# CPCLAB-UNIPI/MPC-code

Hardware: AMD Instinct MI355X
Metric: closed-loop MPC steps/sec over batch, LMPC-CSTR N=50 (higher is better)
Workload: dtype f64

## Files before the change

### __graft_entry__.py

```python
import os
import sys

ROOT = os.path.dirname(os.path.abspath(__file__))
if ROOT not in sys.path:
    sys.path.insert(0, ROOT)

WV_DIRECTION_EXTRA_SETS = ((1, 1, 1, 1, 1, 0, 0), (4, 1, 1, 1, 4, 0, 0), (4, 2, 2, 2, 4, 0, 0), (8, 2, 2, 2, 8, 0, 0))
WV_VGPR_FORM_SETS = ((1, 1, 1, 1, 1, 0, 0), (2, 1, 1, 1, 2, 0, 0), (2, 1, 1, 1, 2, 0, 1), (3, 2, 3, 3, 3, 0, 0), (4, 1, 1, 1, 4, 0, 0), (4, 2, 2, 2, 4, 0, 0))


def build() -> None:
    import mpc_code_amd
    from concurrent.futures import ThreadPoolExecutor
    from mpc_code_amd import capi, nlcodegen
    sys.path.insert(0, os.path.join(ROOT, "oracle"))
    import oracle_c
    import enmpc_oracle_c
    import nmpc_oracle_c
    jobs = [lambda: capi.build_library(verbose=True), oracle_c.build, enmpc_oracle_c.build, nmpc_oracle_c.build]
    for dims in ((3, 2, 3, 3, 3, 1, 0), (5, 2, 2, 2, 5, 0, 0), (3, 2, 3, 3, 3, 0, 0, 1, 1), (3, 2, 3, 3, 3, 0, 2, 1, 1), (6, 2, 8, 0, 6, 0, 0, 1, 1)):
        jobs.append(lambda dims=dims: capi.build_library(dims=dims))
    for dims in WV_DIRECTION_EXTRA_SETS:
        jobs.append(lambda dims=dims: capi.build_library(dims=dims))
    for dims in WV_VGPR_FORM_SETS:
        jobs.append(lambda dims=dims: capi.build_library(dims=dims, extra_flags=(capi.WV_GENERIC_TILES_FLAG,)))
    for ex, dims in (("cstr_nlplant_lmpc.py", (3, 2, 2, 2, 3, 1, 0)), ("cstr_xp_nlplant_lmpc.py", (4, 2, 2, 2, 3, 1, 1))):
        jobs.append(lambda ex=ex, dims=dims: capi.build_library(dims=dims, plant_header=nlcodegen.emit_plant_header(mpc_code_amd.load_problem(mpc_code_amd.example_path(ex)))))
    for ex in ("cstr_nmpc.py", "quadtank_nmpc_dis.py", "reactor_nmpc.py", "cstr_nmpc_rows.py"):
        jobs.append(lambda ex=ex: nlcodegen.build_nmpc_library(mpc_code_amd.load_problem(mpc_code_amd.example_path(ex))))
    from mpc_code_amd import econcodegen
    jobs.append(lambda: econcodegen.build_enmpc_library(mpc_code_amd.load_problem(mpc_code_amd.example_path("reactor_enmpc.py"))))
    jobs.append(lambda: econcodegen.build_enmpc_library(mpc_code_amd.load_problem(mpc_code_amd.example_path("reactor_enmpc_ekf.py"))))
    jobs.append(lambda: econcodegen.build_enmpc_library(mpc_code_amd.load_problem(mpc_code_amd.example_path("reactor_enmpc.py"), overrides={"wmin": [-1.0] * 4, "wmax": [1.0] * 4})))
    jobs.append(lambda: econcodegen.build_enmpc_library(mpc_code_amd.load_problem(mpc_code_amd.example_path("reactor_enmpc_rows.py"))))
    jobs.append(lambda: econcodegen.build_enmpc_library(mpc_code_amd.load_problem(mpc_code_amd.example_path("reactor_enmpc.py")), extra_flags=["-DEC_SWEEP_SERIAL"]))
    import warnings
    sys.path.insert(0, os.path.join(ROOT, "tests"))
    from enmpc_cases import FUZZ_SEEDS, draw

    def fuzz_model(seed):
        with warnings.catch_warnings():
            warnings.simplefilter("ignore")
            return mpc_code_amd.load_problem(mpc_code_amd.example_path("reactor_enmpc.py"), overrides=draw(seed)[0])
    for seed in FUZZ_SEEDS:
        jobs.append(lambda seed=seed: econcodegen.build_enmpc_library(fuzz_model(seed)))
    import nmpc_family
    for member in nmpc_family.MEMBERS:
        jobs.append(lambda member=member: nlcodegen.build_nmpc_library(nmpc_family.load_product(member)))
    import nmpc_lin_family
    for member in nmpc_lin_family.MEMBERS:
        jobs.append(lambda member=member: nlcodegen.build_nmpc_library(nmpc_lin_family.load_product(member)))
    jobs.append(lambda: nlcodegen.build_nmpc_library(mpc_code_amd.load_problem(mpc_code_amd.example_path("reactor_nmpc_lin.py"))))
    with ThreadPoolExecutor(max_workers=min(len(jobs), max(1, (os.cpu_count() or 2) - 1))) as pool:
        built = [f.result() for f in [pool.submit(j) for j in jobs]]
    lib = built[0]
    handle = capi.load_library(lib)
    missing = [s for s in capi.EXPORTS if not hasattr(handle, s)]
    if missing:
        raise RuntimeError(f"libmpc_amd.so lacks {missing}")
    for b in built:
        print("built", b)
    print(handle.mpc_build_info().decode())
    assert mpc_code_amd.load_problem(mpc_code_amd.example_path("cstr_lmpc.py")).nw == 253


def smoke() -> None:
    import numpy as np
    import mpc_code_amd as m
    from mpc_code_amd import capi
    sys.path.insert(0, os.path.join(ROOT, "oracle"))
    import oracle_c
    prob = m.load_problem(m.example_path("cstr_lmpc.py"))
    rng = np.random.default_rng(20250614)
    x0 = rng.uniform([-0.5, -8.0, -5.0], [0.5, 8.0, 5.0], size=(128, 3))
    nsteps = 8
    solver = capi.Solver(prob, device=0)
    solver.loop_alloc(len(x0), nsteps, capi.LOG_ALL)
    solver.loop_set_state(x0, x0)
    solver.loop_set_schedule(prob.schedules(nsteps))
    solver.loop_run(0, nsteps)
    solver.loop_sync()
    U = solver.loop_get_log("U"); st = solver.loop_get_log("STATUS_DYN")
    ref = oracle_c.OracleC(prob).closed_loop(nsteps, x0, x0)
    assert np.array_equal(st, ref["STATUS_DYN"]), "solver status differs from the oracle"
    err = float(np.abs(U - ref["U"]).max())
    assert err < 1e-6, f"u* differs from the oracle by {err}"
    ms, n = solver.last_kernel_ms()
    print(f"smoke ok: {len(x0)} instances x {nsteps} steps, max|u - u_oracle| = {err:.2e}, {ms:.2f} ms in {n} launches")
    solver.close()
    from mpc_code_amd import nmpc
    g = np.load(os.path.join(ROOT, "tests", "golden", "nmpc_cstr.npz"))
    nl = m.load_problem(m.example_path("cstr_nmpc.py"))
    r = nmpc.run_nmpc_closed_loop(nl, g["rti_x0"], g["rti_x0"], nsteps=3, max_sqp=1)
    e = float(np.max(np.abs(r["U"] - g["rti_U"][:3]) / (1.0 + np.abs(g["rti_U"][:3]))))
    assert np.array_equal(r["STATUS_DYN"], g["rti_STATUS_DYN"][:3]) and e < 1e-6, f"non-linear path differs from its oracle vectors by {e}"
    print(f"smoke ok: non-linear path, max rel |u - u_oracle| = {e:.2e}")
    from mpc_code_amd import enmpc
    g = np.load(os.path.join(ROOT, "tests", "golden", "enmpc_reactor.npz"))
    ec = m.load_problem(m.example_path("reactor_enmpc.py"))
    r = enmpc.run_enmpc_closed_loop(ec, g["ship_x0"], nsteps=3)
    e = float(np.abs(r["U"] - g["ship_U"][:3]).max())
    assert np.array_equal(r["STATUS_DYN"], g["ship_STATUS_DYN"][:3]) and np.array_equal(r["ITERS_DYN"], g["ship_ITERS_DYN"][:3]) and e < 1e-7, f"economic path differs from its oracle vectors by {e}"
    print(f"smoke ok: economic path, max |u - u_oracle| = {e:.2e}")


# ... 5 lines not shown
```

### mpc-code_amd/csrc/mpc_amd.hip

```cpp
#include "../../include/mpc_amd.h"
#include "mpc_device.hpp"
#include "mpc_lane_step.hpp"
#include "mpc_tp.hpp"
#include "mpc_wave.hpp"
#include "mpc_soft.hpp"

#include <hip/hip_runtime.h>
#include "mpc_comm.hpp"

#include <cmath>
#include <cstdint>
#include <cstdio>
#include <cstring>
#include <string>
#include <vector>

using namespace mpc;

#ifndef MPC_PART2
extern "C" const char *mpc_last_error(void) { return g_err; }
#endif

#define MPC_DIM9_(M, NX, NU, NY, ND, NXP, DU, NG, NGS, NHS, ...) M(NX, NU, NY, ND, NXP, DU, NG, NGS, NHS)
#define MPC_DIM9(M, ...) MPC_DIM9_(M, __VA_ARGS__, 0, 0, 0)
// ... 413 lines not shown
                    MPC_UNROLL for (int j = 0; j < NX; j++) v += P.Cm[i][j] * xs[j];
                    MPC_UNROLL for (int j = 0; j < ND; j++) v += P.Cd[i][j] * dh[j];
                    (a.YS + (size_t)((size_t)k * NY + i) * Bs)[bq] = v;
                }
            }
            if (a.st_dyn) { (a.st_ss + (size_t)k * Bs)[bq] = st_ss; (a.it_ss + (size_t)k * Bs)[bq] = it_ss; }
            OcpInst<NS, NU> q;
            build_inst<NX, NU, NY, ND, DU, NG>(P, xh, xs, us, dh, u, q);
            double delta = delta_est;
            MPC_UNROLL for (int i = 0; i < NX; i++) delta = dmax(delta, fabs(xs[i] - xs_prev[i]));
            MPC_UNROLL for (int i = 0; i < NU; i++) delta = dmax(delta, fabs(us[i] - us_prev[i]));
            const bool warm = a.ws_valid[bq] != 0 && delta <= kWsDelta && !P.no_warm;
            double *qd = sh.q + lane * Cfg::QN;
            MPC_UNROLL for (int i = 0; i < NS; i++) { qd[i] = q.z0[i]; qd[NS + i] = q.zr[i]; qd[2 * NS + i] = q.c[i]; qd[3 * NS + i] = q.zlo_m[i]; qd[4 * NS + i] = q.zhi_m[i]; }
            MPC_UNROLL for (int i = 0; i < NU; i++) { qd[5 * NS + i] = q.ur[i]; qd[5 * NS + NU + i] = q.us[i]; }
            qd[5 * NS + 2 * NU] = delta;
            sh.iflag[lane] = kTpValid | (q.ok0 ? kTpOk0 : 0) | (warm ? kTpWarm : 0);
            MPC_UNROLL for (int i = 0; i < NX; i++) { (a.xhat + (size_t)(i) * Bs)[bq] = xh[i]; (a.xs + (size_t)(i) * Bs)[bq] = xs[i]; }
            MPC_UNROLL for (int i = 0; i < ND; i++) (a.dhat + (size_t)(i) * Bs)[bq] = dh[i];
            MPC_UNROLL for (int i = 0; i < NU; i++) (a.us + (size_t)(i) * Bs)[bq] = us[i];
        } else if (wl) sh.iflag[lane] = 0;
        int st_dyn, it_dyn;
        MPC_TSTAMP(0);
        tp_solve<NS, NU, DU, NC, MASKED, NW, IPW>(P, sh, wsg, P.max_iter, st_dyn, it_dyn);
        if (valid && P.term_cons && st_dyn != kInfeasible) {
            const double *fin_rows = wsg + (size_t)lane * Cfg::ROWS_ST * 64, *qd = sh.q + lane * Cfg::QN;
            double v = 0.0;
            MPC_UNROLL for (int i = 0; i < NX; i++) v = dmax(v, fabs(fin_rows[(Cfg::ST_Z + i) * 64 + P.N - 1] - qd[NS + i]) * frcp(dmax(1.0, fabs(qd[NS + i]))));
            if (!(v <= P.term_tol)) st_dyn = kInfeasible;
        }
        if (valid) {
            double x[NXP], xh[NX], u[NU];
            MPC_UNROLL for (int i = 0; i < NXP; i++) x[i] = (a.x + (size_t)(i) * Bs)[bq];
            MPC_UNROLL for (int i = 0; i < NU; i++) u[i] = (a.u + (size_t)(i) * Bs)[bq];
            if (st_dyn != kInfeasible) {
                const double *fin_rows = wsg + (size_t)lane * Cfg::ROWS_ST * 64;
                MPC_UNROLL for (int i = 0; i < NU; i++) u[i] = (DU && P.in_is_du) ? fin_rows[(Cfg::ST_Z + (DU ? NX + i : 0)) * 64] : fin_rows[(Cfg::ST_U + i) * 64];
                MPC_UNROLL for (int i = 0; i < NX; i++) xh[i] = fin_rows[(Cfg::ST_Z + i) * 64];
            } else {
                double xo[NX], dh[ND > 0 ? ND : 1];
                MPC_UNROLL for (int i = 0; i < NX; i++) xo[i] = (a.xhat + (size_t)(i) * Bs)[bq];
                MPC_UNROLL for (int i = 0; i < ND; i++) dh[i] = (a.dhat + (size_t)(i) * Bs)[bq];
                MPC_UNROLL for (int i = 0; i < NX; i++) {
                    double v = P.fxc[i];
                    MPC_UNROLL for (int j = 0; j < NX; j++) v += P.Am[i][j] * xo[j];
                    MPC_UNROLL for (int j = 0; j < NU; j++) v += P.Bm[i][j] * u[j];
                    MPC_UNROLL for (int j = 0; j < ND; j++) v += P.Bd[i][j] * dh[j];
                    xh[i] = v;
                }
            }
            if (a.U) { MPC_UNROLL for (int i = 0; i < NU; i++) (a.U + (size_t)((size_t)k * NU + i) * Bs)[bq] = u[i]; }
            if (a.st_dyn) { (a.st_dyn + (size_t)k * Bs)[bq] = st_dyn; (a.it_dyn + (size_t)k * Bs)[bq] = it_dyn; }
            double xn[NXP];
            plant_next<NXP, NU>(P, x, u, a.pxp + k * NXP, a.t0 + k * a.h, a.h, xn);
            if (a.wn) { MPC_UNROLL for (int i = 0; i < NXP; i++) xn[i] += (a.wn + (size_t)((size_t)k * NXP + i) * Bs)[bq]; }
            MPC_UNROLL for (int i = 0; i < NXP; i++) (a.x + (size_t)(i) * Bs)[bq] = xn[i];
            MPC_UNROLL for (int i = 0; i < NX; i++) (a.xhat + (size_t)(i) * Bs)[bq] = xh[i];
            MPC_UNROLL for (int i = 0; i < NU; i++) (a.u + (size_t)(i) * Bs)[bq] = u[i];
            a.ws_valid[bq] = st_dyn == kSolved ? 1 : 0;
        }
        __syncthreads();
        MPC_STAMP_RESET
    }
    if (valid) {
        a.tw_valid[b] = sh.keepflag[lane];
        MPC_UNROLL for (int f = 0; f < NTW; f++) (a.tw + (size_t)f * Bs)[(unsigned)b] = twk[f];
    }
}

template <int NS, int NU, int NC, int NX, int NI, class Cfg>
__device__ __forceinline__ bool wv_term_aim(int N, double *q, int *iflag, int *aimv, int *itacc, const WvIterA<NS, NU, NC> (&X)[NI], const WvInst (&S)[NI])
{
    const int lane = threadIdx.x;
    if (lane == N - 1) {
        MPC_UNROLL for (int j = 0; j < NI; j++) {
            double c[NX], v = 0.0;
            MPC_UNROLL for (int i = 0; i < NX; i++) { const double zr = q[j * Cfg::QN + NS + i]; c[i] = a_get(X[j].z[i]) - zr; v = dmax(v, fabs(c[i]) * frcp(dmax(1.0, fabs(zr)))); }
            const int f = iflag[j];
            const bool again = (f & kWvValid) && (f & kWvOk0) && S[j].status != kInfeasible && v > 1e-11 && v <= 1e-4;
            if (again) { MPC_UNROLL for (int i = 0; i < NX; i++) q[j * Cfg::QN + Cfg::QZN + i] -= c[i]; q[j * Cfg::QN + 5 * NS + 2 * NU] = v; }
            aimv[j] = again ? 1 : 0;
        }
    }
    __syncthreads();
    int any = 0;
    MPC_UNROLL for (int j = 0; j < NI; j++) any |= aimv[j];
    any = __builtin_amdgcn_readfirstlane(any);
    if (any && lane < NI) {
        int st = S[0].status, it = S[0].iters;
        MPC_UNROLL for (int j = 1; j < NI; j++) { if (lane == j) { st = S[j].status; it = S[j].iters; } }
        const int f = iflag[lane];
        if ((f & kWvValid) && (f & kWvOk0) && st != kInfeasible) { iflag[lane] = kWvValid | kWvOk0 | kWvWarm | kWvNoShift; itacc[lane] += it; }
    }
    __syncthreads();
    return any != 0;
}

template <int NX, int NU, int NY, int ND, int NXP, bool DU, int NG, int NC, bool MASKED, int NI, int NGS = 0, int NHS = 0>
struct WvKernelCfg {
    static constexpr int NS = NX + (DU ? NU : 0) + NG, NE = NX + ND, NDD = ND > 0 ? ND : 1;
    using Cfg = WvCfg<NS, NU, NC, NI>;
    using RT = Row16Tab<NX, NU, NY, ND, NGS, NHS>;
    static constexpr int NTW = 2 * (NU - NHS) + 3 * (NX + NU + NY + NGS);
    static constexpr int K_X = 0, K_XH = NXP, K_DH = K_XH + NX, K_U = K_DH + NDD, K_XS = K_U + NU, K_US = K_XS + NX, K_P = K_US + NU,
                         K_TW = K_P + NE * NE, KEEP = K_TW + NTW;
    static constexpr int t_region(int N)
    {
        const int t = Cfg::t_doubles(N), x = Cfg::GUARD + (RT::fits ? 4 * RT::XCH : 0);
        return t > x ? t : x;
    }
    static constexpr size_t lds_bytes(int N) { return sizeof(double) * ((size_t)t_region(N) + NI * Cfg::QN + NI * Cfg::OUT + NI * KEEP + (RT::fits ? RT::DOUBLES : 0)) + sizeof(int) * 24; }
    static constexpr int ni() { return NI; }
};

template <bool NOISE, int NX, int NU, int NY, int ND, int NXP, bool DU, int NG, int NC, bool MASKED, int NI, int NGS, int NHS>
__device__ __forceinline__ void loop_wv_body(const DevProblem *__restrict__ Pp, const LoopArgs &a)
{
    using KC = WvKernelCfg<NX, NU, NY, ND, NXP, DU, NG, NC, MASKED, NI, NGS, NHS>;
    using Cfg = typename KC::Cfg;
    constexpr int NS = KC::NS, NE = KC::NE, NDD = KC::NDD, NTW = KC::NTW, KEEP = KC::KEEP;
    extern __shared__ double wv_smem[];
    const DevProblem &P0 = *Pp;
    const int LD = Cfg::ld(P0.N);
    double *const T = wv_smem + Cfg::GUARD, *const q = wv_smem + KC::t_region(P0.N), *const outv = q + NI * Cfg::QN, *const keep = outv + NI * Cfg::OUT;
    int *const iflag = (int *)(keep + NI * KEEP), *const twv = iflag + 4, *const wsv = twv + 4, *const aimv = wsv + 4, *const itacc = aimv + 4;
    using RT = typename KC::RT;
    double *const tab = (double *)(wsv + 16);
    const ConstProblem &P = *(const ConstProblem *)Pp;
    const size_t Bs = a.Bs;
    const int lane = threadIdx.x;
    const int il = lane < NI ? lane : 0;
    const int b = blockIdx.x * NI + il;
    const bool valid = lane < NI && b < a.B;
    double *const kp = keep + il * KEEP;
    if (valid) {
        MPC_UNROLL for (int i = 0; i < NXP; i++) kp[KC::K_X + i] = (a.x + (size_t)i * Bs)[b];
        MPC_UNROLL for (int i = 0; i < NX; i++) { kp[KC::K_XH + i] = (a.xhat + (size_t)i * Bs)[b]; kp[KC::K_XS + i] = (a.xs + (size_t)i * Bs)[b]; }
        MPC_UNROLL for (int i = 0; i < ND; i++) kp[KC::K_DH + i] = (a.dhat + (size_t)i * Bs)[b];
        MPC_UNROLL for (int i = 0; i < NU; i++) { kp[KC::K_U + i] = (a.u + (size_t)i * Bs)[b]; kp[KC::K_US + i] = (a.us + (size_t)i * Bs)[b]; }
        if (P.estimator == MPC_EST_KALMAN) { for (int i = 0; i < NE * NE; i++) kp[KC::K_P + i] = (a.Pk + (size_t)i * Bs)[b]; }
        for (int f = 0; f < NTW; f++) kp[KC::K_TW + f] = (a.tw + (size_t)f * Bs)[b];
        twv[lane] = a.tw_valid[b]; wsv[lane] = a.ws_valid[b];
    } else if (lane < NI) { twv[lane] = 0; wsv[lane] = 0; }
    for (int i = lane; i < NI * LD; i += 64) T[Cfg::RZ * NI * LD + i] = 0.0;
    if (lane < Cfg::GUARD) wv_smem[lane] = 0.0;
    if (RT::fits) row16_fill_tables<NX, NU, NY, ND, NGS, NHS>(P, tab, lane);
    __syncthreads();
    WvIterA<NS, NU, NC> X[NI];
    WvInst S[NI];
    MPC_UNROLL for (int j = 0; j < NI; j++) {
        const double *rows = a.ws + ((size_t)(blockIdx.x * NI + j) * Cfg::ROWS_WS) * 64;
        const bool w = __builtin_amdgcn_readfirstlane(wsv[j]) != 0;
        WvIter<NS, NU, NC> X0;
        MPC_UNROLL for (int i = 0; i < NU; i++) X0.u[i] = w ? rows[i * 64 + lane] : 0.0;
        MPC_UNROLL for (int i = 0; i < NC; i++) { X0.ll[i] = w ? rows[(NU + i) * 64 + lane] : 0.0; X0.lh[i] = w ? rows[(NU + NC + i) * 64 + lane] : 0.0; X0.sl[i] = 1.0; X0.sh[i] = 1.0; }
        MPC_UNROLL for (int i = 0; i < NS; i++) X0.z[i] = 0.0;
        X[j].put(X0);
    }
    MPC_STAMP_INIT
    int redo = 0;
    for (int k = 0; k < a.nsteps; k++) {
        unsigned bq = (unsigned)b;
        asm volatile("" : "+v"(bq));
        if (redo == 0) {
        if constexpr (RT::fits) {
            const int b16 = lane >> 4, r16 = lane & 15, b16c = b16 < NI ? b16 : 0;
            const unsigned bi = (unsigned)(blockIdx.x * NI + b16c);
            const bool inst16 = b16 < NI && (int)bi < a.B;
            double *const kq = keep + b16c * KEEP;
            if (inst16) {
                if (a.XP && r16 < NXP) (a.XP + (size_t)((size_t)k * NXP + r16) * Bs)[bi] = kq[KC::K_X + r16];
                if (a.XHAT && r16 < NX) (a.XHAT + (size_t)((size_t)k * NX + r16) * Bs)[bi] = kq[KC::K_XH + r16];
            }
            double xi_old = 0.0, xi_new = 0.0;
            if (P.estimator != MPC_EST_NONE)
                kalman_row16<NX, NY, ND, NXP, NU>(P, r16, b16 < NI, kq, KC::K_X, KC::K_XH, KC::K_P, a.pyp + k * NY, (NOISE && a.vn) ? a.vn + (size_t)k * NY * Bs + bi : nullptr, Bs, tab, T + b16c * RT::XCH, xi_old, xi_new);
            if (inst16 && a.DHAT && r16 >= NX && r16 < NE) (a.DHAT + (size_t)((size_t)k * ND + (r16 - NX)) * Bs)[bi] = xi_new;
            double delta = row16_max(r16 < NE ? fabs(xi_new - xi_old) : 0.0);
            __syncthreads();
            if (Cfg::RZ * NI * LD < 4 * RT::XCH) { for (int i = lane; i < NI * LD; i += 64) T[Cfg::RZ * NI * LD + i] = 0.0; }
            double dh[NDD], usv[NU];
            MPC_UNROLL for (int i = 0; i < ND; i++) dh[i] = kq[KC::K_DH + i];
            MPC_UNROLL for (int i = 0; i < NU; i++) usv[i] = kq[KC::K_US + i];
            int it_ss; double vrow;
            int st_ss;
            if constexpr (NOISE) {
                double uspv[NU], yspv[NY];
                MPC_UNROLL for (int i = 0; i < NU; i++) uspv[i] = a.usp[k * NU + i];
                MPC_UNROLL for (int i = 0; i < NY; i++) yspv[i] = a.ysp[k * NY + i];
                if (a.usp_b) { MPC_UNROLL for (int i = 0; i < NU; i++) uspv[i] = (a.usp_b + (size_t)((size_t)k * NU + i) * Bs)[bi]; }
                if (a.ysp_b) { MPC_UNROLL for (int i = 0; i < NY; i++) yspv[i] = (a.ysp_b + (size_t)((size_t)k * NY + i) * Bs)[bi]; }
                st_ss = target_row16<NX, NU, NY, ND, NGS, NHS>(P, r16, tab, uspv, yspv, dh, usv, kq + KC::K_TW, twv + b16c, inst16, vrow, it_ss);
            } else
                st_ss = target_row16<NX, NU, NY, ND, NGS, NHS>(P, r16, tab, a.usp + k * NU, a.ysp + k * NY, dh, usv, kq + KC::K_TW, twv + b16c, inst16, vrow, it_ss);
            const bool trow = r16 < NX + NU && b16 < NI;
            const double prev = trow ? kq[KC::K_XS + r16] : 0.0;
            const double tnew = (st_ss != kInfeasible && trow) ? vrow : prev;
            delta = dmax(delta, row16_max(fabs(tnew - prev)));
            if (trow) kq[KC::K_XS + r16] = tnew;
            if (inst16) {
                if (a.XS && r16 < NX) (a.XS + (size_t)((size_t)k * NX + r16) * Bs)[bi] = tnew;
                if (a.US && r16 >= NX && trow) (a.US + (size_t)((size_t)k * NU + (r16 - NX)) * Bs)[bi] = tnew;
                if (a.st_dyn && r16 == 0) { (a.st_ss + (size_t)k * Bs)[bi] = st_ss; (a.it_ss + (size_t)k * Bs)[bi] = it_ss; }
            }
            if (r16 == 0 && b16 < NI) outv[b16c * Cfg::OUT] = delta;
            __syncthreads();
        }
        if (valid) {
            double xh[NX], dh[NDD], u[NU], xs[NX], us[NU], delta = 0.0;
            MPC_UNROLL for (int i = 0; i < NX; i++) { xh[i] = kp[KC::K_XH + i]; xs[i] = kp[KC::K_XS + i]; }
            MPC_UNROLL for (int i = 0; i < ND; i++) dh[i] = kp[KC::K_DH + i];
            MPC_UNROLL for (int i = 0; i < NU; i++) { u[i] = kp[KC::K_U + i]; us[i] = kp[KC::K_US + i]; }
            if constexpr (RT::fits) delta = outv[lane * Cfg::OUT];
            else {
                double x[NXP];
                double xh_pred[NX], dh_prev[NDD], xs_prev[NX], us_prev[NU];
                MPC_UNROLL for (int i = 0; i < NXP; i++) x[i] = kp[KC::K_X + i];
                MPC_UNROLL for (int i = 0; i < NX; i++) { xh[i] = kp[KC::K_XH + i]; xs[i] = kp[KC::K_XS + i]; xh_pred[i] = xh[i]; xs_prev[i] = xs[i]; }
                MPC_UNROLL for (int i = 0; i < ND; i++) { dh[i] = kp[KC::K_DH + i]; dh_prev[i] = dh[i]; }
                MPC_UNROLL for (int i = 0; i < NU; i++) { u[i] = kp[KC::K_U + i]; us[i] = kp[KC::K_US + i]; us_prev[i] = us[i]; }
                if (a.XP) { MPC_UNROLL for (int i = 0; i < NXP; i++) (a.XP + (size_t)((size_t)k * NXP + i) * Bs)[bq] = x[i]; }
                if (a.XHAT) { MPC_UNROLL for (int i = 0; i < NX; i++) (a.XHAT + (size_t)((size_t)k * NX + i) * Bs)[bq] = xh[i]; }
                if (P.estimator != MPC_EST_NONE) {
                    double xi[NE], innov[NY];
                    MPC_UNROLL for (int i = 0; i < NX; i++) xi[i] = xh[i];
                    MPC_UNROLL for (int i = 0; i < ND; i++) xi[NX + i] = dh[i];
                    MPC_UNROLL for (int i = 0; i < NY; i++) {
                        double yh = P.fyc[i], yy = a.pyp[k * NY + i];
                        if (NOISE && a.vn) yy += (a.vn + (size_t)((size_t)k * NY + i) * Bs)[bq];
                        MPC_UNROLL for (int j = 0; j < NE; j++) yh += P.Ca[i][j] * xi[j];
                        MPC_UNROLL for (int j = 0; j < NXP; j++) yy += P.Cp[i][j] * x[j];
                        innov[i] = yy - yh;
                    }
                    if (P.estimator == MPC_EST_KALMAN) {
                        double Pk[NE][NE];
                        MPC_UNROLL for (int i = 0; i < NE; i++) { MPC_UNROLL for (int j = 0; j < NE; j++) Pk[i][j] = kp[KC::K_P + i * NE + j]; }
                        kalman_lane<NE, NY>(P, xi, Pk, innov);
                        MPC_UNROLL for (int i = 0; i < NE; i++) { MPC_UNROLL for (int j = 0; j < NE; j++) kp[KC::K_P + i * NE + j] = Pk[i][j]; }
                    } else {
                        MPC_UNROLL for (int i = 0; i < NE; i++) { double s = 0.0; MPC_UNROLL for (int l = 0; l < NY; l++) s += P.Kfix[i][l] * innov[l]; xi[i] += s; }
                    }
                    MPC_UNROLL for (int i = 0; i < NX; i++) xh[i] = xi[i];
                    MPC_UNROLL for (int i = 0; i < ND; i++) { double d = xi[NX + i]; if (P.has_dsat) d = dmin(dmax(d, P.dmin[i]), P.dmax[i]); dh[i] = d; }
                }
                if (a.DHAT) { MPC_UNROLL for (int i = 0; i < ND; i++) (a.DHAT + (size_t)((size_t)k * ND + i) * Bs)[bq] = dh[i]; }
                MPC_UNROLL for (int i = 0; i < NX; i++) delta = dmax(delta, fabs(xh[i] - xh_pred[i]));
                MPC_UNROLL for (int i = 0; i < ND; i++) delta = dmax(delta, fabs(dh[i] - dh_prev[i]));
                double usp[NU], ysp[NY], xs_n[NX], us_n[NU], ys_n[NY];
                MPC_UNROLL for (int i = 0; i < NU; i++) usp[i] = a.usp[k * NU + i];
                MPC_UNROLL for (int i = 0; i < NY; i++) ysp[i] = a.ysp[k * NY + i];
                if (NOISE && a.usp_b) { MPC_UNROLL for (int i = 0; i < NU; i++) usp[i] = (a.usp_b + (size_t)((size_t)k * NU + i) * Bs)[bq]; }
                if (NOISE && a.ysp_b) { MPC_UNROLL for (int i = 0; i < NY; i++) ysp[i] = (a.ysp_b + (size_t)((size_t)k * NY + i) * Bs)[bq]; }
                int it_ss;
                const int st_ss = target_lane<NX, NU, NY, ND, NGS, NHS>(P, usp, ysp, dh, us, xs_n, us_n, ys_n, it_ss, kp + KC::K_TW, 1, twv + lane);
                if (st_ss != kInfeasible) {
                    MPC_UNROLL for (int i = 0; i < NX; i++) xs[i] = xs_n[i];
                    MPC_UNROLL for (int i = 0; i < NU; i++) us[i] = us_n[i];
                }
                if (a.XS) { MPC_UNROLL for (int i = 0; i < NX; i++) (a.XS + (size_t)((size_t)k * NX + i) * Bs)[bq] = xs[i]; }
                if (a.US) { MPC_UNROLL for (int i = 0; i < NU; i++) (a.US + (size_t)((size_t)k * NU + i) * Bs)[bq] = us[i]; }
                if (a.st_dyn) { (a.st_ss + (size_t)k * Bs)[bq] = st_ss; (a.it_ss + (size_t)k * Bs)[bq] = it_ss; }
                MPC_UNROLL for (int i = 0; i < NX; i++) delta = dmax(delta, fabs(xs[i] - xs_prev[i]));
                MPC_UNROLL for (int i = 0; i < NU; i++) delta = dmax(delta, fabs(us[i] - us_prev[i]));
            }
            if (a.YS) {
                MPC_UNROLL for (int i = 0; i < NY; i++) {
                    double v = P.fyc[i];
                    MPC_UNROLL for (int j = 0; j < NX; j++) v += P.Cm[i][j] * xs[j];
                    MPC_UNROLL for (int j = 0; j < ND; j++) v += P.Cd[i][j] * dh[j];
                    (a.YS + (size_t)((size_t)k * NY + i) * Bs)[bq] = v;
                }
            }
            OcpInst<NS, NU> qi;
            build_inst<NX, NU, NY, ND, DU, NG>(P, xh, xs, us, dh, u, qi);
            const bool warm = wsv[lane] != 0 && delta <= kWsDelta && !P.no_warm;
            double *qd = q + lane * Cfg::QN;
            MPC_UNROLL for (int i = 0; i < NS; i++) { qd[i] = qi.z0[i]; qd[NS + i] = qi.zr[i]; qd[2 * NS + i] = qi.c[i]; qd[3 * NS + i] = qi.zlo_m[i]; qd[4 * NS + i] = qi.zhi_m[i]; qd[Cfg::QZN + i] = qi.zrN[i]; }
            MPC_UNROLL for (int i = 0; i < NU; i++) { qd[5 * NS + i] = qi.ur[i]; qd[5 * NS + NU + i] = qi.us[i]; }
            qd[5 * NS + 2 * NU] = delta;
            iflag[lane] = kWvValid | (qi.ok0 ? kWvOk0 : 0) | (warm ? kWvWarm : 0);
            itacc[lane] = 0;
            MPC_UNROLL for (int i = 0; i < NX; i++) { kp[KC::K_XH + i] = xh[i]; kp[KC::K_XS + i] = xs[i]; }
            MPC_UNROLL for (int i = 0; i < ND; i++) kp[KC::K_DH + i] = dh[i];
            MPC_UNROLL for (int i = 0; i < NU; i++) kp[KC::K_US + i] = us[i];
        } else if (lane < NI) iflag[lane] = 0;
        __syncthreads();
        }
        MPC_TSTAMP(0);
        wv_solve<NS, NU, DU, NC, MASKED, NI>(P, T, q, iflag, X, S, P.max_iter);
        MPC_STAMP_RESET
        if (lane == 0) {
            MPC_UNROLL for (int j = 0; j < NI; j++) {
                MPC_UNROLL for (int i = 0; i < NU; i++) outv[j * Cfg::OUT + i] = a_get(X[j].u[i]);
                MPC_UNROLL for (int i = 0; i < NS; i++) outv[j * Cfg::OUT + NU + i] = a_get(X[j].z[i]);
            }
        }
        if (P.term_cons && lane == P.N - 1) {
            MPC_UNROLL for (int j = 0; j < NI; j++) {
                double v = 0.0, c[NX];
                MPC_UNROLL for (int i = 0; i < NX; i++) { const double zr = q[j * Cfg::QN + NS + i]; c[i] = a_get(X[j].z[i]) - zr; v = dmax(v, fabs(c[i]) * frcp(dmax(1.0, fabs(zr)))); }
                outv[j * Cfg::OUT + NU + NS] = v;
                const int f = iflag[j];
                const bool again = redo < 2 && (f & kWvValid) && (f & kWvOk0) && S[j].status != kInfeasible && v > 1e-11 && v <= 1e-4;
                if (again) { MPC_UNROLL for (int i = 0; i < NX; i++) q[j * Cfg::QN + Cfg::QZN + i] -= c[i]; q[j * Cfg::QN + 5 * NS + 2 * NU] = v; }
                aimv[j] = again ? 1 : 0;
            }
        }
        __syncthreads();
        if (P.term_cons && redo < 2) {
            int any = 0;
            MPC_UNROLL for (int j = 0; j < NI; j++) any |= aimv[j];
            if (__builtin_amdgcn_readfirstlane(any)) {
                if (lane < NI) {
                    int st = S[0].status, it = S[0].iters;
                    MPC_UNROLL for (int j = 1; j < NI; j++) { if (lane == j) { st = S[j].status; it = S[j].iters; } }
                    const int f = iflag[lane];
                    if ((f & kWvValid) && (f & kWvOk0) && st != kInfeasible) { iflag[lane] = kWvValid | kWvOk0 | kWvWarm | kWvNoShift; itacc[lane] += it; }
                }
                __syncthreads();
                redo++; k--;
                continue;
            }
        }
        redo = 0;
        if (valid) {
            int st_dyn = S[0].status, it_dyn = S[0].iters;
            MPC_UNROLL for (int j = 1; j < NI; j++) { if (lane == j) { st_dyn = S[j].status; it_dyn = S[j].iters; } }
            if (P.term_cons) it_dyn += itacc[lane];
            if (P.term_cons && st_dyn != kInfeasible && !(outv[lane * Cfg::OUT + NU + NS] <= P.term_tol)) st_dyn = kInfeasible;
            double x[NXP], xh[NX], u[NU];
            MPC_UNROLL for (int i = 0; i < NXP; i++) x[i] = kp[KC::K_X + i];
            MPC_UNROLL for (int i = 0; i < NU; i++) u[i] = kp[KC::K_U + i];
            if (st_dyn != kInfeasible) {
                MPC_UNROLL for (int i = 0; i < NU; i++) u[i] = (DU && P.in_is_du) ? outv[lane * Cfg::OUT + NU + (DU ? NX + i : 0)] : outv[lane * Cfg::OUT + i];
                MPC_UNROLL for (int i = 0; i < NX; i++) xh[i] = outv[lane * Cfg::OUT + NU + i];
            } else {
                double xo[NX], dh[NDD];
                MPC_UNROLL for (int i = 0; i < NX; i++) xo[i] = kp[KC::K_XH + i];
                MPC_UNROLL for (int i = 0; i < ND; i++) dh[i] = kp[KC::K_DH + i];
                MPC_UNROLL for (int i = 0; i < NX; i++) {
                    double v = P.fxc[i];
                    MPC_UNROLL for (int j = 0; j < NX; j++) v += P.Am[i][j] * xo[j];
                    MPC_UNROLL for (int j = 0; j < NU; j++) v += P.Bm[i][j] * u[j];
                    MPC_UNROLL for (int j = 0; j < ND; j++) v += P.Bd[i][j] * dh[j];
                    xh[i] = v;
                }
            }
            if (a.U) { MPC_UNROLL for (int i = 0; i < NU; i++) (a.U + (size_t)((size_t)k * NU + i) * Bs)[bq] = u[i]; }
            if (a.st_dyn) { (a.st_dyn + (size_t)k * Bs)[bq] = st_dyn; (a.it_dyn + (size_t)k * Bs)[bq] = it_dyn; }
            {
                double xn[NXP];
                plant_next<NXP, NU>(P, x, u, a.pxp + k * NXP, a.t0 + k * a.h, a.h, xn);
                if (NOISE && a.wn) { MPC_UNROLL for (int i = 0; i < NXP; i++) xn[i] += (a.wn + (size_t)((size_t)k * NXP + i) * Bs)[bq]; }
                MPC_UNROLL for (int i = 0; i < NXP; i++) kp[KC::K_X + i] = xn[i];
            }
            MPC_UNROLL for (int i = 0; i < NX; i++) kp[KC::K_XH + i] = xh[i];
            MPC_UNROLL for (int i = 0; i < NU; i++) kp[KC::K_U + i] = u[i];
            wsv[lane] = st_dyn == kSolved ? 1 : 0;
        }
        __syncthreads();
        MPC_TSTAMP(7);
    }
    if (valid) {
        MPC_UNROLL for (int i = 0; i < NXP; i++) (a.x + (size_t)i * Bs)[b] = kp[KC::K_X + i];
        MPC_UNROLL for (int i = 0; i < NX; i++) { (a.xhat + (size_t)i * Bs)[b] = kp[KC::K_XH + i]; (a.xs + (size_t)i * Bs)[b] = kp[KC::K_XS + i]; }
        MPC_UNROLL for (int i = 0; i < ND; i++) (a.dhat + (size_t)i * Bs)[b] = kp[KC::K_DH + i];
        MPC_UNROLL for (int i = 0; i < NU; i++) { (a.u + (size_t)i * Bs)[b] = kp[KC::K_U + i]; (a.us + (size_t)i * Bs)[b] = kp[KC::K_US + i]; }
        if (P.estimator == MPC_EST_KALMAN) { for (int i = 0; i < NE * NE; i++) (a.Pk + (size_t)i * Bs)[b] = kp[KC::K_P + i]; }
        for (int f = 0; f < NTW; f++) (a.tw + (size_t)f * Bs)[b] = kp[KC::K_TW + f];
        a.tw_valid[b] = twv[lane]; a.ws_valid[b] = wsv[lane];
    }
    MPC_UNROLL for (int j = 0; j < NI; j++) {
        double *rows = a.ws + ((size_t)(blockIdx.x * NI + j) * Cfg::ROWS_WS) * 64;
        MPC_UNROLL for (int i = 0; i < NU; i++) rows[i * 64 + lane] = a_get(X[j].u[i]);
        MPC_UNROLL for (int i = 0; i < NC; i++) { rows[(NU + i) * 64 + lane] = a_get(X[j].ll[i]); rows[(NU + NC + i) * 64 + lane] = a_get(X[j].lh[i]); }
    }
}

template <int NX, int NU, int NY, int ND, int NXP, bool DU, int NG, int NC, bool MASKED, int NI, int NGS = 0, int NHS = 0>
__global__ __launch_bounds__(64, 1) void loop_kernel_wv(const DevProblem *__restrict__ Pp, LoopArgs a)
{
    loop_wv_body<false, NX, NU, NY, ND, NXP, DU, NG, NC, MASKED, NI, NGS, NHS>(Pp, a);
}

template <int NX, int NU, int NY, int ND, int NXP, bool DU, int NG, int NC, bool MASKED, int NI, int NGS = 0, int NHS = 0>
__global__ __launch_bounds__(64, 1) void loop_noisy_wv_kernel(const DevProblem *__restrict__ Pp, LoopArgs a)
{
    loop_wv_body<true, NX, NU, NY, ND, NXP, DU, NG, NC, MASKED, NI, NGS, NHS>(Pp, a);
}

struct OcpWvArgs {
    OcpArgs o;
    const double *u_guess;
    double *traj;
    double *prev;
    int32_t *valid;
    int warm_on;
};

template <int NX, int NU, int NY, int ND, bool DU, int NG, int NC, bool MASKED, int NI>
__global__ __launch_bounds__(64, 1) void ocp_kernel_wv(const DevProblem *__restrict__ Pp, OcpWvArgs w)
{
    constexpr int NS = NX + (DU ? NU : 0) + NG, NDD = ND > 0 ? ND : 1;
    using Cfg = WvCfg<NS, NU, NC, NI>;
    const OcpArgs &a = w.o;
    extern __shared__ double wv_smem[];
    const ConstProblem &P = *(const ConstProblem *)Pp;
    const int N = Pp->N, LD = Cfg::ld(N);
    double *const T = wv_smem + Cfg::GUARD, *const q = wv_smem + Cfg::t_doubles(N), *const outv = q + NI * Cfg::QN;
    int *const iflag = (int *)(outv + NI * Cfg::OUT), *const aimv = iflag + 4, *const itacc = aimv + 4;
    const size_t Bs = a.Bs;
    const int lane = threadIdx.x;
    const int il = lane < NI ? lane : 0;
    const int b = blockIdx.x * NI + il;
    const bool valid = lane < NI && b < a.B;
    for (int i = lane; i < NI * LD; i += 64) T[Cfg::RZ * NI * LD + i] = 0.0;
    if (lane < Cfg::GUARD) wv_smem[lane] = 0.0;
    if (valid) {
        double xh[NX], xs[NX], us[NU], up[NU], dh[NDD];
        MPC_UNROLL for (int i = 0; i < NX; i++) { xh[i] = a.xhat[i * Bs + b]; xs[i] = a.xs[i * Bs + b]; }
        MPC_UNROLL for (int i = 0; i < NU; i++) { us[i] = a.us[i * Bs + b]; up[i] = a.u_prev[i * Bs + b]; }
        MPC_UNROLL for (int i = 0; i < ND; i++) dh[i] = a.dhat[i * Bs + b];
        OcpInst<NS, NU> qi;
        build_inst<NX, NU, NY, ND, DU, NG>(P, xh, xs, us, dh, up, qi);
        double delta = 0.0;
        MPC_UNROLL for (int i = 0; i < NX; i++) delta = dmax(delta, dmax(fabs(xh[i] - w.prev[i * Bs + b]), fabs(xs[i] - w.prev[(NX + ND + i) * Bs + b])));
        MPC_UNROLL for (int i = 0; i < ND; i++) delta = dmax(delta, fabs(dh[i] - w.prev[(NX + i) * Bs + b]));
        MPC_UNROLL for (int i = 0; i < NU; i++) delta = dmax(delta, fabs(us[i] - w.prev[(2 * NX + ND + i) * Bs + b]));
        const bool warm = w.warm_on && w.valid[b] != 0 && delta <= kWsDelta && !P.no_warm;
        double *qd = q + lane * Cfg::QN;
        MPC_UNROLL for (int i = 0; i < NS; i++) { qd[i] = qi.z0[i]; qd[NS + i] = qi.zr[i]; qd[2 * NS + i] = qi.c[i]; qd[3 * NS + i] = qi.zlo_m[i]; qd[4 * NS + i] = qi.zhi_m[i]; qd[Cfg::QZN + i] = qi.zrN[i]; }
        MPC_UNROLL for (int i = 0; i < NU; i++) { qd[5 * NS + i] = qi.ur[i]; qd[5 * NS + NU + i] = qi.us[i]; }
        qd[5 * NS + 2 * NU] = delta;
        iflag[lane] = kWvValid | (qi.ok0 ? kWvOk0 : 0) | (warm ? kWvWarm : 0) | ((warm && w.u_guess) ? kWvKeepU : 0);
        itacc[lane] = 0;
        MPC_UNROLL for (int i = 0; i < ND; i++) w.prev[(NX + i) * Bs + b] = dh[i];
        MPC_UNROLL for (int i = 0; i < NX; i++) w.prev[(NX + ND + i) * Bs + b] = xs[i];
        MPC_UNROLL for (int i = 0; i < NU; i++) w.prev[(2 * NX + ND + i) * Bs + b] = us[i];
    } else if (lane < NI) iflag[lane] = 0;
    __syncthreads();
    WvIterA<NS, NU, NC> X[NI];
    WvInst S[NI];
    MPC_UNROLL for (int j = 0; j < NI; j++) {
        const size_t bj = (size_t)blockIdx.x * NI + j;
        const double *rows = a.ws + (bj * Cfg::ROWS_WS) * 64;
        const int fl = __builtin_amdgcn_readfirstlane(iflag[j]);
        const bool wm = (fl & kWvWarm) != 0, ku = (fl & kWvKeepU) != 0;
        WvIter<NS, NU, NC> X0;
        MPC_UNROLL for (int i = 0; i < NU; i++) X0.u[i] = wm ? (ku ? w.u_guess[(bj * NU + i) * 64 + lane] : rows[i * 64 + lane]) : 0.0;
        MPC_UNROLL for (int i = 0; i < NC; i++) { X0.ll[i] = wm ? rows[(NU + i) * 64 + lane] : 0.0; X0.lh[i] = wm ? rows[(NU + NC + i) * 64 + lane] : 0.0; X0.sl[i] = 1.0; X0.sh[i] = 1.0; }
        MPC_UNROLL for (int i = 0; i < NS; i++) X0.z[i] = 0.0;
        X[j].put(X0);
    }
    for (int pass = 0;; pass++) {
        wv_solve<NS, NU, DU, NC, MASKED, NI, ConstProblem, false, false, true>(P, T, q, iflag, X, S, P.max_iter);
        if (!P.term_cons || pass == 2 || !wv_term_aim<NS, NU, NC, NX, NI, Cfg>(N, q, iflag, aimv, itacc, X, S)) break;
    }
    MPC_UNROLL for (int j = 0; j < NI; j++) {
        const size_t bj = (size_t)blockIdx.x * NI + j;
        double *rows = a.ws + (bj * Cfg::ROWS_WS) * 64;
        WvIter<NS, NU, NC> Xf; X[j].get(Xf);
        MPC_UNROLL for (int i = 0; i < NU; i++) rows[i * 64 + lane] = Xf.u[i];
        MPC_UNROLL for (int i = 0; i < NC; i++) { rows[(NU + i) * 64 + lane] = Xf.ll[i]; rows[(NU + NC + i) * 64 + lane] = Xf.lh[i]; }
        if (w.traj) {
            MPC_UNROLL for (int i = 0; i < NU; i++) w.traj[(bj * (NU + NS) + i) * 64 + lane] = Xf.u[i];
            MPC_UNROLL for (int i = 0; i < NS; i++) w.traj[(bj * (NU + NS) + NU + i) * 64 + lane] = Xf.z[i];
        }
        if (lane == 0) {
            MPC_UNROLL for (int i = 0; i < NU; i++) outv[j * Cfg::OUT + i] = Xf.u[i];
            MPC_UNROLL for (int i = 0; i < NS; i++) outv[j * Cfg::OUT + NU + i] = Xf.z[i];
        }
        if (P.term_cons && lane == P.N - 1) {
            double v = 0.0;
            MPC_UNROLL for (int i = 0; i < NX; i++) { const double zr = q[j * Cfg::QN + NS + i]; v = dmax(v, fabs(Xf.z[i] - zr) * frcp(dmax(1.0, fabs(zr)))); }
            outv[j * Cfg::OUT + NU + NS] = v;
        }
    }
    __syncthreads();
    if (valid) {
        int st = S[0].status, it = S[0].iters; double r0 = S[0].res_s, r1 = S[0].res_p, r2 = S[0].mu;
        MPC_UNROLL for (int j = 1; j < NI; j++) { if (lane == j) { st = S[j].status; it = S[j].iters; r0 = S[j].res_s; r1 = S[j].res_p; r2 = S[j].mu; } }
        if (P.term_cons) it += itacc[lane];
        if (P.term_cons && st != kInfeasible && !(outv[lane * Cfg::OUT + NU + NS] <= P.term_tol)) st = kInfeasible;
        a.status[b] = st; a.iters[b] = it;
        a.res[0 * Bs + b] = r0; a.res[1 * Bs + b] = r1; a.res[2 * Bs + b] = r2;
        w.valid[b] = st == kSolved ? 1 : 0;
        if (st != kInfeasible) {
            MPC_UNROLL for (int i = 0; i < NU; i++) a.u_out[i * Bs + b] = (DU && P.in_is_du) ? outv[lane * Cfg::OUT + NU + (DU ? NX + i : 0)] : outv[lane * Cfg::OUT + i];
            MPC_UNROLL for (int i = 0; i < NX; i++) { const double v = outv[lane * Cfg::OUT + NU + i]; a.xnext_out[i * Bs + b] = v; w.prev[i * Bs + b] = v; }
        }
    }
}

#ifndef MPC_PART2
__global__ void pack_u_kernel(const double *__restrict__ u, double *__restrict__ dst, int B, size_t Bs, int nu)
{
    const int b = blockIdx.x * blockDim.x + threadIdx.x;
    if (b >= B) return;
    for (int i = 0; i < nu; i++) dst[(size_t)b * nu + i] = u[i * Bs + b];
}
#endif

struct Launchers {
    void (*ocp)(const DevProblem *, OcpArgs, hipStream_t);
    void (*ocp_pxy)(const DevProblem *, OcpPxyArgs, hipStream_t);
    void (*ocp_soft)(const DevProblem *, OcpSoftArgs, hipStream_t);
    int soft_fields;
    void (*loop_soft)(const DevProblem *, LoopArgs, hipStream_t);
    void (*loop_pxy)(const DevProblem *, LoopArgs, hipStream_t);
    int pxy_ws_rows, pxy_nc, pxy_lin;
    void (*target)(const DevProblem *, TargetArgs, hipStream_t);
    void (*kf)(const DevProblem *, KfArgs, hipStream_t);
    void (*loop)(const DevProblem *, LoopArgs, hipStream_t);
    int (*loop_tp)(const DevProblem *, LoopArgs, hipStream_t);
    int (*loop_wv)(const DevProblem *, LoopArgs, hipStream_t);
    int (*ocp_wv)(const DevProblem *, OcpWvArgs, int, hipStream_t);
    int wv_ns;
    size_t wv_ws_per_inst, wv_lds;
    int ws_rows, nc, tp_ni;
    int tp_max_batch;
    size_t tp_ws_per_inst, tp_ws_per_group, tp_lds;
};

static constexpr int kTpMaxBatch = 16384;

enum { kBoundsAllFinite = 1, kBoundsInputsOnly = 2, kBoundsGeneric = 0 };

template <int NX, int NU, int NY, int ND, int NXP, bool DU, int NG, int NC, bool MASKED, int NI, int NGS, int NHS>
static int launch_loop_wv(const DevProblem *p, LoopArgs a, hipStream_t s, int dev)
{
    using KC = WvKernelCfg<NX, NU, NY, ND, NXP, DU, NG, NC, MASKED, NI, NGS, NHS>;
    const bool noisy = a.vn || a.wn || a.ysp_b || a.usp_b;
    auto kern = noisy ? loop_noisy_wv_kernel<NX, NU, NY, ND, NXP, DU, NG, NC, MASKED, NI, NGS, NHS> : loop_kernel_wv<NX, NU, NY, ND, NXP, DU, NG, NC, MASKED, NI, NGS, NHS>;
    static bool attr_set[2][64] = {};
    if (!attr_set[noisy][dev]) {
        if (hipFuncSetAttribute(reinterpret_cast<const void *>(kern), hipFuncAttributeMaxDynamicSharedMemorySize, (int)KC::lds_bytes(64)) != hipSuccess) return -1;
        attr_set[noisy][dev] = true;
    }
    hipLaunchKernelGGL(kern, dim3((a.B + NI - 1) / NI), dim3(64), KC::lds_bytes(a.N), s, p, a);
    return 0;
}

template <int NX, int NU, int NY, int ND, int NXP, bool DU, int NG, int NC, bool MASKED, int NGS, int NHS>
static Launchers make_launchers_mode()
{
    Launchers l;
    l.ocp = [](const DevProblem *p, OcpArgs a, hipStream_t s) { hipLaunchKernelGGL((ocp_kernel<NX, NU, NY, ND, DU, NG, NC, MASKED>), dim3((a.B + 63) / 64), dim3(64), 0, s, p, a); };
    {
        constexpr int NSZ = NX + (DU ? NU : 0) + NG;
        l.ocp_pxy = [](const DevProblem *p, OcpPxyArgs a, hipStream_t s) { hipLaunchKernelGGL((ocp_kernel_pxy<NX, NU, NY, ND, DU, NG>), dim3((a.o.B + 63) / 64), dim3(64), 0, s, p, a); };
        if constexpr (NGS == 0 && NHS == 0)
            l.loop_pxy = [](const DevProblem *p, LoopArgs a, hipStream_t s) { hipLaunchKernelGGL((loop_kernel_pxy<NX, NU, NY, ND, NXP, DU, NG>), dim3((a.B + 63) / 64), dim3(64), 0, s, p, a); };
        else
            l.loop_pxy = nullptr;
        l.pxy_ws_rows = 2 * BlkLayout<NSZ, NU, NSZ + NU>::SLOTS; l.pxy_nc = NSZ + NU; l.pxy_lin = NSZ * (NSZ + NU + 1) + 2 * NSZ;
        l.ocp_soft = [](const DevProblem *p, OcpSoftArgs a, hipStream_t s) { hipLaunchKernelGGL((ocp_kernel_soft<NX, NU, NY, ND, DU, NG>), dim3((a.o.B + 63) / 64), dim3(64), 0, s, p, a); };
        l.soft_fields = SoftLayout<NSZ, NU, NY>::FIELDS;
        l.loop_soft = [](const DevProblem *p, LoopArgs a, hipStream_t s) { hipLaunchKernelGGL((loop_kernel_soft<NX, NU, NY, ND, NXP, DU, NG, NGS, NHS>), dim3((a.B + 63) / 64), dim3(64), 0, s, p, a); };
    }
    l.target = [](const DevProblem *p, TargetArgs a, hipStream_t s) { hipLaunchKernelGGL((target_kernel<NX, NU, NY, ND, NGS, NHS>), dim3((a.B + 63) / 64), dim3(64), 0, s, p, a); };
    l.kf = [](const DevProblem *p, KfArgs a, hipStream_t s) { hipLaunchKernelGGL((kf_kernel<NX, NY, ND>), dim3((a.B + 63) / 64), dim3(64), 0, s, p, a); };
// ... 1202 lines not shown
```

### mpc-code_amd/csrc/mpc_device.hpp

```cpp
#pragma once
#include <hip/hip_runtime.h>
#include <math.h>
#include <stdint.h>

namespace mpc {

constexpr double kMu0 = 1.0;
constexpr double kSMin = 1.0;
constexpr double kTau = 0.995;
constexpr double kTolStat = 1e-9;
constexpr double kTolStatAcc = 1e-6;
constexpr int kStallMax = 2;
constexpr double kTolFeas = 1e-9;
constexpr double kTolC = 1e-9;
constexpr double kTolMu = 1e-14;
constexpr double kMuFloor = 1e-15;
constexpr double kSFloor = 1e-11;
constexpr double kBoundRelax = 1e-8;
constexpr double kInfeasZ = 1e10;
constexpr double kWsDelta = 0.3;
constexpr double kWsKappa = 1e-2;
constexpr double kWsSMinLo = 1e-9, kWsSMinHi = 1e-6;
constexpr double kWsMuFactor = 1e4;

constexpr int kMaxN = 8, kMaxM = 4, kMaxY = 8, kMaxD = 8, kMaxV = kMaxN + kMaxM, kMaxC = kMaxN + kMaxM + kMaxY,
              kMaxE = kMaxN + kMaxD, kMaxGS = 4;

enum : int { kSolved = 0, kMaxIter = 1, kInfeasible = 2 };

struct DevProblem {
    int nx, nu, ny, nd, nxp, N, du_form, duss_form, y_bounded, estimator, max_iter, has_dsat;
    int term_cons; double term_tol, term_gcap, term_floor;
    int no_warm;
    int in_is_du, zr_us;
    double A[kMaxN][kMaxN], B[kMaxN][kMaxM], Q[kMaxN][kMaxN], M[kMaxN][kMaxM], R[kMaxM][kMaxM], Pf[kMaxN][kMaxN];
    double ulo[kMaxM], uhi[kMaxM], zlo_m[kMaxN], zhi_m[kMaxN], zlo_e[kMaxN], zhi_e[kMaxN];
    double Am[kMaxN][kMaxN], Bm[kMaxN][kMaxM], Cm[kMaxY][kMaxN], Bd[kMaxN][kMaxD], Cd[kMaxY][kMaxD], fxc[kMaxN], fyc[kMaxY];
    double Ap[kMaxN][kMaxN], Bp[kMaxN][kMaxM], Cp[kMaxY][kMaxN];
    double ymin[kMaxY], ymax[kMaxY], dmin[kMaxD], dmax[kMaxD];
    int ymap_idx[kMaxY]; double ymap_scale[kMaxY];
    int ng, yg_row[kMaxY];
    double Ep[kMaxV][kMaxN], Zn[kMaxV][kMaxM], CZx[kMaxY][kMaxM], Hr[kMaxM][kMaxM], W[kMaxC][kMaxM], tlo[kMaxC], thi[kMaxC];
    double Qss[kMaxY][kMaxY], Rss[kMaxM][kMaxM];
    double Aa[kMaxE][kMaxE], Ca[kMaxY][kMaxE], Qkf[kMaxE][kMaxE], Rkf[kMaxY][kMaxY], Kfix[kMaxE][kMaxY];
    double Apow[6][kMaxN][kMaxN];
    int soft;
    double Ws[2 * kMaxY][2 * kMaxY];
    int ng_ss, nh_ss;
    double Eh[kMaxV][kMaxM];
    double Hd_ss[kMaxM][kMaxD], h0_ss[kMaxM];
    double Gv_ss[kMaxGS][kMaxV], Gd_ss[kMaxGS][kMaxD], g0_ss[kMaxGS];
    double Wg[kMaxGS][kMaxM];
};

typedef __attribute__((address_space(4))) DevProblem ConstProblem;

#define MPC_UNROLL _Pragma("unroll")
#ifdef MPC_STAMPS
__device__ unsigned long long mpc_stamp_buf[4096 * 8];
#define MPC_STAMP(slot) do { const unsigned long long t_ = __builtin_amdgcn_s_memtime(); __builtin_amdgcn_s_waitcnt(0xC07F); \
    if (threadIdx.x == 0) mpc_stamp_buf[blockIdx.x * 8 + (slot)] += t_ - stamp_prev_; stamp_prev_ = t_; } while (0)
#define MPC_STAMP_INIT unsigned long long stamp_prev_ = __builtin_amdgcn_s_memtime();
#define MPC_STAMP_RESET stamp_prev_ = __builtin_amdgcn_s_memtime();
#else
#define MPC_STAMP(slot) do { } while (0)
#define MPC_STAMP_INIT
#define MPC_STAMP_RESET
#endif

__device__ __forceinline__ double dmax(double a, double b) { return __builtin_fmax(a, b); }
__device__ __forceinline__ double dmin(double a, double b) { return __builtin_fmin(a, b); }
__device__ __forceinline__ bool fin(double a) { return fabs(a) < 1.0e300; }
__device__ __forceinline__ double comp_measure(double s, double l)
{
    return dmin(dmin(s, l) * (1.0 / kTolC), s * l * (1.0 / kTolMu));
}

__device__ __forceinline__ double frcp(double x)
{
    double r = __builtin_amdgcn_rcp(x);
    double e = __builtin_fma(-x, r, 1.0);
    r = __builtin_fma(e, r, r);
    e = __builtin_fma(-x, r, 1.0);
    r = __builtin_fma(e, r, r);
    return r;
}
__device__ __forceinline__ double frcp_approx(double x) { return __builtin_amdgcn_rcp(x); }

__device__ __forceinline__ double vreg(double x)
{
    asm volatile("" : "+v"(x));
    return x;
}

template <int NS, int NU, int NC>
struct BlkLayout {
    static constexpr int NV = NS + NU;
    static constexpr int S = 0, L = NC, P = 2 * NC, IS = 3 * NC;
    static constexpr int U = 4 * NC, Z = U + (NU + 1) / 2, DU = Z + (NS + 1) / 2, DZ = DU + (NU + 1) / 2,
                         KFF = DZ + (NS + 1) / 2, K = KFF + (NU + 1) / 2, LI = K + (NU * NS + 1) / 2,
                         SLOTS = LI + (NU * (NU + 1) / 2 + 1) / 2;
};

typedef double v2d __attribute__((ext_vector_type(2)));
typedef __attribute__((address_space(1))) v2d gv2d;
struct BlkPtr {
    gv2d *base; int lane;
    __device__ __forceinline__ gv2d &operator[](int i) const { return base[i + lane]; }
};
struct Ws {
    gv2d *slab;
    int N, slots, lane;
    __device__ __forceinline__ BlkPtr blk(int k) const { return BlkPtr{slab + (ptrdiff_t)k * slots * 64, lane}; }
};

template <int CNT>
__device__ __forceinline__ void ld_field(const BlkPtr blk, int slot0, double (&out)[CNT])
{
    MPC_UNROLL for (int j = 0; j < (CNT + 1) / 2; j++) {
        const v2d v = blk[(slot0 + j) * 64];
        out[2 * j] = v.x;
        if (2 * j + 1 < CNT) out[2 * j + 1 < CNT ? 2 * j + 1 : 0] = v.y;
    }
}
template <int CNT>
__device__ __forceinline__ void st_field(const BlkPtr blk, int slot0, const double (&in)[CNT])
{
    MPC_UNROLL for (int j = 0; j < (CNT + 1) / 2; j++) {
        v2d v;
        v.x = in[2 * j];
        v.y = (2 * j + 1 < CNT) ? in[2 * j + 1 < CNT ? 2 * j + 1 : 0] : 0.0;
        blk[(slot0 + j) * 64] = v;
    }
}

#include "mpc_sym.hpp"

template <int NS, int NU>
struct OcpInst {
    double z0[NS], zr[NS], ur[NU], c[NS], us[NU], zlo_m[NS], zhi_m[NS];
    double zrN[NS];
    bool ok0;
};

template <int NX, int NU, int NY, int ND, bool DU, int NG, class PT>
__device__ __forceinline__ void build_inst(const PT &P, const double (&xhat)[NX], const double (&xs)[NX],
                                           const double (&us)[NU], const double *dhat, const double (&u_prev)[NU],
                                           OcpInst<NX + (DU ? NU : 0) + NG, NU> &q)
{
    constexpr int NS = NX + (DU ? NU : 0) + NG, NB = NX + (DU ? NU : 0);
    MPC_UNROLL for (int i = 0; i < NX; i++) {
        double c = P.fxc[i];
        MPC_UNROLL for (int j = 0; j < ND; j++) c += P.Bd[i][j] * dhat[j];
        q.c[i] = c; q.z0[i] = xhat[i]; q.zr[i] = xs[i];
    }
    MPC_UNROLL for (int i = 0; i < NU; i++) { q.us[i] = us[i]; q.ur[i] = DU ? 0.0 : us[i]; }
    if (DU) {
        MPC_UNROLL for (int i = 0; i < NU; i++) { q.z0[NX + i] = u_prev[i]; q.zr[NX + i] = 0.0; q.c[NX + i] = 0.0; }
// ... 732 lines not shown
```

### mpc-code_amd/csrc/mpc_nmpc.hip

```cpp
#include "../../include/mpc_nmpc.h"
#include "../../include/mpc_amd.h"

#include <hip/hip_runtime.h>
#include <hip/hip_ext.h>

#include MPC_NL_MODEL_HEADER
#include "mpc_nmpc.hpp"
#include "mpc_wave.hpp"
#include "mpc_host.hpp"

#include <cmath>
#include <algorithm>
#include <cstdio>
#include <cstring>
#include <string>
#include <type_traits>
#include <vector>

using namespace mpc;
using M = NlModel;

extern "C" const char *nmpc_last_error(void) { return g_err; }

template <class T, class = void> struct NgOf { static constexpr int value = 0; };
// ... 340 lines not shown
        MPC_UNROLL for (int i = 0; i < NX; i++) { xh_pred[i] = xi[i]; xs_prev[i] = xs[i]; }
        MPC_UNROLL for (int i = 0; i < ND; i++) dh_prev[i] = xi[NX + i];
        MPC_UNROLL for (int i = 0; i < NU; i++) us_prev[i] = us[i];
        nl_log<NXP>(a.XP, k, Bs, b, x);
        nl_log<NX>(a.XHAT, k, Bs, b, xi);
        double y[NY];
        nl_measure(a, k, b, x, u, t, y);
        nl_correct(P, a.h, xi, Pk, y, u, t);
        double *const dh = xi + NX;
        nl_log<ND>(a.DHAT, k, Bs, b, dh);
        int st_ss = kMaxIter, sqp_ss = 0;
        {
            double xs_t[NX], us_t[NU];
            MPC_UNROLL for (int i = 0; i < NX; i++) xs_t[i] = xs[i];
            MPC_UNROLL for (int i = 0; i < NU; i++) us_t[i] = us[i];
            for (int it = 0; it < 30; it++) {
                double F[NX], A[NX][NX], B[NX][NU], G[NX][NDD], yv[NY], hx[NY][NX], hd[NY][NDD];
                rk4_model_sens<M, false>(xs_t, us_t, dh, t, a.h, F, A, B, G);
                M::h(xs_t, us_t, dh, t, yv); M::h_jac(xs_t, us_t, dh, t, hx, hd);
                TargetLocal<NX, NU, NY> T;
                T.duss_form = P.duss_form; T.max_iter = P.max_iter;
                MPC_UNROLL for (int i = 0; i < NX; i++) { double c = F[i]; MPC_UNROLL for (int j = 0; j < NX; j++) c -= A[i][j] * xs_t[j]; MPC_UNROLL for (int j = 0; j < NU; j++) c -= B[i][j] * us_t[j]; T.fxc[i] = c; T.Bd[i][0] = 0.0; }
                MPC_UNROLL for (int i = 0; i < NY; i++) { double e = yv[i]; MPC_UNROLL for (int j = 0; j < NX; j++) { e -= hx[i][j] * xs_t[j]; T.Cm[i][j] = hx[i][j]; } T.fyc[i] = e; T.Cd[i][0] = 0.0; }
                MPC_UNROLL for (int i = 0; i < NY; i++) { MPC_UNROLL for (int j = 0; j < NY; j++) T.Qss[i][j] = P.Qss[i][j]; }
                MPC_UNROLL for (int i = 0; i < NU; i++) { MPC_UNROLL for (int j = 0; j < NU; j++) T.Rss[i][j] = P.Rss[i][j]; }
                MPC_UNROLL for (int r = 0; r < NX + NU + NY; r++) { T.tlo[r] = P.tlo[r]; T.thi[r] = P.thi[r]; }
                if (!target_prepare<NX, NU, NY>(A, B, T)) { st_ss = kInfeasible; break; }
                double usp[NU], ysp[NY], xs_n[NX], us_n[NU], ys_n[NY];
                MPC_UNROLL for (int i = 0; i < NU; i++) usp[i] = a.usp[k * NU + i];
                MPC_UNROLL for (int i = 0; i < NY; i++) ysp[i] = a.ysp[k * NY + i];
                if (a.usp_b) { MPC_UNROLL for (int i = 0; i < NU; i++) usp[i] = a.usp_b[(k * NU + i) * (long)Bs + b]; }
                if (a.ysp_b) { MPC_UNROLL for (int i = 0; i < NY; i++) ysp[i] = a.ysp_b[(k * NY + i) * (long)Bs + b]; }
                int itq;
                const int sq = target_lane<NX, NU, NY, 0>(T, usp, ysp, nullptr, us_prev, xs_n, us_n, ys_n, itq);
                sqp_ss = it + 1;
                if (sq != kSolved) { st_ss = sq; break; }
                double step = 0.0;
                MPC_UNROLL for (int i = 0; i < NX; i++) { step = dmax(step, fabs(xs_n[i] - xs_t[i])); xs_t[i] = xs_n[i]; }
                MPC_UNROLL for (int i = 0; i < NU; i++) { step = dmax(step, fabs(us_n[i] - us_t[i])); us_t[i] = us_n[i]; }
                if (step < 1e-10) { st_ss = kSolved; break; }
            }
            if (st_ss != kInfeasible) {
                MPC_UNROLL for (int i = 0; i < NX; i++) xs[i] = xs_t[i];
                MPC_UNROLL for (int i = 0; i < NU; i++) us[i] = us_t[i];
            }
        }
        nl_log<NX>(a.XS, k, Bs, b, xs);
        nl_log<NU>(a.US, k, Bs, b, us);
        if (a.st_dyn) { a.st_ss[(size_t)k * Bs + b] = st_ss; a.sqp_ss[(size_t)k * Bs + b] = sqp_ss; }
        OcpInst<NS, NU> q;
        const double delta = nl_ocp_data(P, xi, xs, us, u, xh_pred, dh_prev, xs_prev, us_prev, q);
        MPC_UNROLL for (int i = 0; i < NX; i++) { a.xch[(XC_XH + i) * Bs + b] = xi[i]; a.xch[(XC_XSP + i) * Bs + b] = xs_prev[i]; a.xch[(XC_XH0 + i) * Bs + b] = xh_pred[i]; }
        MPC_UNROLL for (int i = 0; i < ND; i++) a.xch[(XC_DH + i) * Bs + b] = dh[i];
        MPC_UNROLL for (int i = 0; i < NS; i++) { a.xch[(XC_ZR + i) * Bs + b] = q.zr[i]; a.xch[(XC_ZLO + i) * Bs + b] = q.zlo_m[i]; a.xch[(XC_ZHI + i) * Bs + b] = q.zhi_m[i]; }
        MPC_UNROLL for (int i = 0; i < NU; i++) { a.xch[(XC_UR + i) * Bs + b] = q.ur[i]; a.xch[(XC_USQ + i) * Bs + b] = q.us[i]; a.xch[(XC_USP + i) * Bs + b] = us_prev[i]; a.xch[(XC_UP + i) * Bs + b] = u[i]; }
        a.xch[XC_DELTA * Bs + b] = delta;
        a.xci[XI_OK0 * Bs + b] = q.ok0 ? 1 : 0;
    }
    nl_state_store(a, b, with_P, x, xi, u, xs, us, Pk);
}

constexpr int WNI = 4;
constexpr bool kWaveFits = MPC_NL_WAVE_FITS != 0;
static_assert(kWaveFits == (NS <= 4 && NU <= 2 && !DUV), "generated header and kernel disagree on the wave-autonomous kernel");
constexpr int kRowsWsWv = NU + NS + 2 * NC;
#if MPC_NL_WAVE_FITS
using WCfg = WvCfg<NS, NU, NC, WNI>;
struct NwKeep {
    static constexpr int K_X = 0, K_XI = NXP, K_U = K_XI + NE, K_XS = K_U + NU, K_US = K_XS + NX, K_XSP = K_US + NU, K_USP = K_XSP + NX, K_P = K_USP + NU,
                         K_XI0 = K_P + NE * NE, KEEP = K_XI0 + NX;
};
static size_t nmpc_wv_lds_bytes(int N) { return sizeof(double) * ((size_t)WCfg::t_doubles_ltv(N) + WNI * WCfg::QN + WNI * WCfg::OUT + WNI * NwKeep::KEEP) + sizeof(int) * 32; }

template <bool SPLIT, bool PAIR, bool WN = false>
__global__ __launch_bounds__(64, 1) __attribute__((flatten)) void nmpc_loop_kernel_wv(const DevProblem *__restrict__ Pp, NlArgs a)
{
    using Cfg = WCfg;
    using KK = NwKeep;
    constexpr int NI = WNI, NJ = PAIR ? NI / 2 : NI;
    extern __shared__ double nw_smem[];
    const DevProblem &Pg = *Pp;
    const ConstProblem &P = *(const ConstProblem *)Pp;
    const int N = Pg.N, LD = Cfg::ld(N);
    double *const T = nw_smem + Cfg::GUARD, *const q = nw_smem + Cfg::t_doubles_ltv(N), *const outv = q + NI * Cfg::QN, *const keep = outv + NI * Cfg::OUT;
    int *const iflag = (int *)(keep + NI * KK::KEEP), *const act = iflag + 4, *const shf = act + 4, *const wsv = shf + 4, *const stv = wsv + 4, *const itv = stv + 4, *const sqv = itv + 4;
    const size_t Bs = a.Bs;
    const int lane = threadIdx.x, k = PAIR ? (lane & 31) : lane, hsel = PAIR ? (lane >> 5) : 0;
    auto ji = [&](int j) -> int { return PAIR ? 2 * j + hsel : j; };
    const bool blk_on = k < N;
    const int il = lane < NI ? lane : 0;
    const int bix = blockIdx.x + a.b0 / NI;
    const int b = bix * NI + il;
    const bool valid = lane < NI && b < a.B;
    double *const kp = keep + il * KK::KEEP;
    if (valid && SPLIT) {
        MPC_UNROLL for (int i = 0; i < NX; i++) { kp[KK::K_XI + i] = a.xch[(XC_XH + i) * Bs + b]; kp[KK::K_XSP + i] = a.xch[(XC_XSP + i) * Bs + b]; kp[KK::K_XI0 + i] = a.xch[(XC_XH0 + i) * Bs + b]; }
        MPC_UNROLL for (int i = 0; i < ND; i++) kp[KK::K_XI + NX + i] = a.xch[(XC_DH + i) * Bs + b];
        MPC_UNROLL for (int i = 0; i < NU; i++) { kp[KK::K_U + i] = a.xch[(XC_UP + i) * Bs + b]; kp[KK::K_USP + i] = a.xch[(XC_USP + i) * Bs + b]; }
        wsv[lane] = a.ws_valid[b];
    } else if (valid) {
        MPC_UNROLL for (int i = 0; i < NXP; i++) kp[KK::K_X + i] = a.x[i * Bs + b];
        MPC_UNROLL for (int i = 0; i < NX; i++) { kp[KK::K_XI + i] = a.xhat[i * Bs + b]; kp[KK::K_XS + i] = a.xs[i * Bs + b]; }
        MPC_UNROLL for (int i = 0; i < ND; i++) kp[KK::K_XI + NX + i] = a.dhat[i * Bs + b];
        MPC_UNROLL for (int i = 0; i < NU; i++) { kp[KK::K_U + i] = a.u[i * Bs + b]; kp[KK::K_US + i] = a.us[i * Bs + b]; }
        for (int i = 0; i < NE * NE; i++) kp[KK::K_P + i] = a.Pk[i * Bs + b];
        wsv[lane] = a.ws_valid[b];
    } else if (lane < NI) wsv[lane] = 0;
    for (int i = lane; i < NI * LD; i += 64) T[Cfg::RZ * NI * LD + i] = 0.0;
    if (lane < Cfg::GUARD) nw_smem[lane] = 0.0;
    __syncthreads();
    WvIterA<NS, NU, NC> X[NJ];
    WvInst S[NJ];
    MPC_UNROLL for (int j = 0; j < NJ; j++) {
        const double *rows = a.ws + ((size_t)(bix * NI + ji(j)) * kRowsWsWv) * 64;
        const bool w = PAIR ? wsv[ji(j)] != 0 : __builtin_amdgcn_readfirstlane(wsv[j]) != 0;
        WvIter<NS, NU, NC> X0;
        MPC_UNROLL for (int i = 0; i < NU; i++) X0.u[i] = w ? rows[i * 64 + k] : 0.0;
        MPC_UNROLL for (int i = 0; i < NS; i++) X0.z[i] = w ? rows[(NU + i) * 64 + k] : 0.0;
        MPC_UNROLL for (int i = 0; i < NC; i++) { X0.ll[i] = w ? rows[(NU + NS + i) * 64 + k] : 0.0; X0.lh[i] = w ? rows[(NU + NS + NC + i) * 64 + k] : 0.0; X0.sl[i] = 1.0; X0.sh[i] = 1.0; }
        X[j].put(X0);
    }
    MPC_STAMP_INIT
    for (int ks = 0; ks < (SPLIT ? 1 : a.nsteps); ks++) {
        const double t = (a.k0 + ks) * a.h;
        MPC_STAMP_RESET
        if (valid && SPLIT) {
            double *qd = q + lane * Cfg::QN;
            MPC_UNROLL for (int i = 0; i < NS; i++) { qd[i] = i < NX ? a.xch[(XC_XH + (i < NX ? i : 0)) * Bs + b] : 0.0; qd[NS + i] = a.xch[(XC_ZR + i) * Bs + b]; qd[2 * NS + i] = 0.0; qd[3 * NS + i] = a.xch[(XC_ZLO + i) * Bs + b]; qd[4 * NS + i] = a.xch[(XC_ZHI + i) * Bs + b]; qd[Cfg::QZN + i] = qd[NS + i]; }
            MPC_UNROLL for (int i = 0; i < NU; i++) { qd[5 * NS + i] = a.xch[(XC_UR + i) * Bs + b]; qd[5 * NS + NU + i] = a.xch[(XC_USQ + i) * Bs + b]; }
            const double delta = a.xch[XC_DELTA * Bs + b];
            qd[5 * NS + 2 * NU] = delta;
            const bool ok0 = a.xci[XI_OK0 * Bs + b] != 0, have = wsv[lane] != 0, warm = have && delta <= kWsDelta;
            iflag[lane] = kWvValid | (ok0 ? kWvOk0 : 0) | (warm ? kWvWarm : 0);
            act[lane] = ok0 ? 1 : 0; shf[lane] = have ? 1 : 0;
            stv[lane] = ok0 ? kMaxIter : kInfeasible; itv[lane] = 0; sqv[lane] = 0;
        } else if (valid) {
            double x[NXP], xi[NE], u[NU], xs[NX], us[NU], Pk[NE][NE];
            MPC_UNROLL for (int i = 0; i < NXP; i++) x[i] = kp[KK::K_X + i];
            MPC_UNROLL for (int i = 0; i < NE; i++) xi[i] = kp[KK::K_XI + i];
            MPC_UNROLL for (int i = 0; i < NU; i++) { u[i] = kp[KK::K_U + i]; us[i] = kp[KK::K_US + i]; }
            MPC_UNROLL for (int i = 0; i < NX; i++) xs[i] = kp[KK::K_XS + i];
            MPC_UNROLL for (int i = 0; i < NE; i++) { MPC_UNROLL for (int jj = 0; jj < NE; jj++) Pk[i][jj] = kp[KK::K_P + i * NE + jj]; }
            double xh_pred[NX], dh_prev[NDD], xs_prev[NX], us_prev[NU];
            MPC_UNROLL for (int i = 0; i < NX; i++) { xh_pred[i] = xi[i]; xs_prev[i] = xs[i]; }
            MPC_UNROLL for (int i = 0; i < ND; i++) dh_prev[i] = xi[NX + i];
            MPC_UNROLL for (int i = 0; i < NU; i++) us_prev[i] = us[i];
            if (a.XP) { MPC_UNROLL for (int i = 0; i < NXP; i++) a.XP[((size_t)ks * NXP + i) * Bs + b] = x[i]; }
            if (a.XHAT) { MPC_UNROLL for (int i = 0; i < NX; i++) a.XHAT[((size_t)ks * NX + i) * Bs + b] = xi[i]; }
            double y[NY];
            M::hp(x, u, t, y);
            MPC_UNROLL for (int i = 0; i < NY; i++) y[i] += a.pyp[ks * NY + i];
            if (a.vn) { MPC_UNROLL for (int i = 0; i < NY; i++) y[i] += a.vn[((size_t)ks * NY + i) * Bs + b]; }
            if (Pg.estimator == MPC_EST_FIXED_GAIN) {
                double yh[NY];
                M::h(xi, u, xi + NX, t, yh);
                MPC_UNROLL for (int i = 0; i < NE; i++) { double sacc = 0.0; MPC_UNROLL for (int l = 0; l < NY; l++) sacc += Pg.Kfix[i][l] * (y[l] - yh[l]); xi[i] += sacc; }
            } else ekf_lane<M, true>(Pg, xi, Pk, y, u, t, a.h);
            if (Pg.has_dsat) { MPC_UNROLL for (int i = 0; i < ND; i++) xi[NX + i] = dmin(dmax(xi[NX + i], Pg.dmin[i]), Pg.dmax[i]); }
            double *const dh = xi + NX;
            if (a.DHAT) { MPC_UNROLL for (int i = 0; i < ND; i++) a.DHAT[((size_t)ks * ND + i) * Bs + b] = dh[i]; }
            int st_ss = kMaxIter, sqp_ss = 0;
            {
                double xs_t[NX], us_t[NU];
                MPC_UNROLL for (int i = 0; i < NX; i++) xs_t[i] = xs[i];
                MPC_UNROLL for (int i = 0; i < NU; i++) us_t[i] = us[i];
                for (int it = 0; it < 30; it++) {
                    double F[NX], A[NX][NX], B[NX][NU], G[NX][NDD], yv[NY], hx[NY][NX], hd[NY][NDD];
                    rk4_model_sens_inl<M, false>(xs_t, us_t, dh, t, a.h, F, A, B, G);
                    M::h(xs_t, us_t, dh, t, yv); M::h_jac(xs_t, us_t, dh, t, hx, hd);
                    TargetLocal<NX, NU, NY> TT;
                    TT.duss_form = Pg.duss_form; TT.max_iter = Pg.max_iter;
                    MPC_UNROLL for (int i = 0; i < NX; i++) { double c = F[i]; MPC_UNROLL for (int jj = 0; jj < NX; jj++) c -= A[i][jj] * xs_t[jj]; MPC_UNROLL for (int jj = 0; jj < NU; jj++) c -= B[i][jj] * us_t[jj]; TT.fxc[i] = c; TT.Bd[i][0] = 0.0; }
                    MPC_UNROLL for (int i = 0; i < NY; i++) { double e = yv[i]; MPC_UNROLL for (int jj = 0; jj < NX; jj++) { e -= hx[i][jj] * xs_t[jj]; TT.Cm[i][jj] = hx[i][jj]; } TT.fyc[i] = e; TT.Cd[i][0] = 0.0; }
                    MPC_UNROLL for (int i = 0; i < NY; i++) { MPC_UNROLL for (int jj = 0; jj < NY; jj++) TT.Qss[i][jj] = Pg.Qss[i][jj]; }
                    MPC_UNROLL for (int i = 0; i < NU; i++) { MPC_UNROLL for (int jj = 0; jj < NU; jj++) TT.Rss[i][jj] = Pg.Rss[i][jj]; }
                    MPC_UNROLL for (int r = 0; r < NX + NU + NY; r++) { TT.tlo[r] = Pg.tlo[r]; TT.thi[r] = Pg.thi[r]; }
                    if (!target_prepare<NX, NU, NY>(A, B, TT)) { st_ss = kInfeasible; break; }
                    double usp[NU], ysp[NY], xs_n[NX], us_n[NU], ys_n[NY];
                    MPC_UNROLL for (int i = 0; i < NU; i++) usp[i] = a.usp[ks * NU + i];
                    MPC_UNROLL for (int i = 0; i < NY; i++) ysp[i] = a.ysp[ks * NY + i];
                    if constexpr (WN) {
                        if (a.usp_b) { MPC_UNROLL for (int i = 0; i < NU; i++) usp[i] = a.usp_b[((size_t)ks * NU + i) * Bs + b]; }
                        if (a.ysp_b) { MPC_UNROLL for (int i = 0; i < NY; i++) ysp[i] = a.ysp_b[((size_t)ks * NY + i) * Bs + b]; }
                    }
                    int itq;
                    const int sq = target_lane<NX, NU, NY, 0>(TT, usp, ysp, nullptr, us_prev, xs_n, us_n, ys_n, itq);
                    sqp_ss = it + 1;
                    if (sq != kSolved) { st_ss = sq; break; }
                    double step = 0.0;
                    MPC_UNROLL for (int i = 0; i < NX; i++) { step = dmax(step, fabs(xs_n[i] - xs_t[i])); xs_t[i] = xs_n[i]; }
                    MPC_UNROLL for (int i = 0; i < NU; i++) { step = dmax(step, fabs(us_n[i] - us_t[i])); us_t[i] = us_n[i]; }
                    if (step < 1e-10) { st_ss = kSolved; break; }
// ... 735 lines not shown
```

### mpc-code_amd/csrc/mpc_tp.hpp

```cpp
#pragma once
#include "mpc_device.hpp"

#ifdef MPC_STAMPS
#define MPC_TSTAMP(slot) do { const unsigned long long t_ = __builtin_amdgcn_s_memtime(); __builtin_amdgcn_s_waitcnt(0xC07F); \
    if (threadIdx.x == 0 && threadIdx.y == 0) mpc_stamp_buf[(blockIdx.x & 4095) * 8 + (slot)] += t_ - stamp_prev_; stamp_prev_ = t_; } while (0)
#else
#define MPC_TSTAMP(slot) do { } while (0)
#endif
#ifdef MPC_STAMPS_FINE
#define MPC_TSTAMP_IT(slot) MPC_TSTAMP(3)
#define MPC_TSTAMP_FINE(slot) MPC_TSTAMP(slot)
#else
#define MPC_TSTAMP_IT(slot) MPC_TSTAMP(slot)
#define MPC_TSTAMP_FINE(slot) do { } while (0)
#endif

namespace mpc {

template <int NS, int NU, int NC, int NW, int IPW, int XKEEP = 0>
struct TpCfg {
    static constexpr int NI = NW * IPW;
    static constexpr int NV = NS + NU, NKF = NU * NS, NLI = NU * (NU + 1) / 2;
    static constexpr int RA = 0, RA_SZ = (NC > NKF + NLI ? NC : NKF + NLI);
    static constexpr int RG = RA_SZ, RK = RG + NV, ROWS = RK + NU;
    static constexpr int LD = 65;
    static constexpr int T_DOUBLES = ROWS * NI * LD;
    static constexpr int QN = 5 * NS + 2 * NU + 1;
    static constexpr int ST_SL = 0, ST_SH = NC, ST_LL = 2 * NC, ST_LH = 3 * NC, ST_DV = 4 * NC, ST_U = 5 * NC, ST_Z = 5 * NC + NU, ROWS_ST = 5 * NC + NV;
    static constexpr int KEEP_MAX = 2 * NU + 3 * (NS + NU + 8) + XKEEP;
    static constexpr size_t lds_bytes() { return sizeof(double) * (T_DOUBLES + NI * QN + NI * 4 + NI * KEEP_MAX) + sizeof(int) * (4 * NI + 4); }
};

template <int CTRL, int ROW_MASK>
__device__ __forceinline__ double dpp_move(double old, double v)
{
    constexpr bool every_lane_has_a_source = ROW_MASK == 0xF && ((CTRL >= 0 && CTRL <= 0xFF) || CTRL == 0x140 || CTRL == 0x141);
    union { double d; int i[2]; } a, o, r; a.d = v; o.d = old;
    if constexpr (every_lane_has_a_source) {
        r.i[0] = __builtin_amdgcn_update_dpp(a.i[0], a.i[0], CTRL, 0xF, 0xF, true);
        r.i[1] = __builtin_amdgcn_update_dpp(a.i[1], a.i[1], CTRL, 0xF, 0xF, true);
    } else {
        r.i[0] = __builtin_amdgcn_update_dpp(o.i[0], a.i[0], CTRL, ROW_MASK, 0xF, false);
        r.i[1] = __builtin_amdgcn_update_dpp(o.i[1], a.i[1], CTRL, ROW_MASK, 0xF, false);
    }
    return r.d;
}
__device__ __forceinline__ double wave_up1(double old, double v) { return dpp_move<0x138, 0xF>(old, v); }
__device__ __forceinline__ double wave_dn1(double old, double v) { return dpp_move<0x130, 0xF>(old, v); }
__device__ __forceinline__ double lane63(double v)
{
    union { double d; int i[2]; } x; x.d = v;
    x.i[0] = __builtin_amdgcn_readlane(x.i[0], 63); x.i[1] = __builtin_amdgcn_readlane(x.i[1], 63);
    return x.d;
}
__device__ __forceinline__ double wave_sum(double v)
{
    v += dpp_move<0xB1, 0xF>(0.0, v);
    v += dpp_move<0x4E, 0xF>(0.0, v);
    v += dpp_move<0x141, 0xF>(0.0, v);
    v += dpp_move<0x140, 0xF>(0.0, v);
    v += dpp_move<0x142, 0xA>(0.0, v);
    v += dpp_move<0x143, 0xC>(0.0, v);
    return lane63(v);
}
__device__ __forceinline__ double wave_max(double v)
{
    v = dmax(v, dpp_move<0xB1, 0xF>(v, v));
    v = dmax(v, dpp_move<0x4E, 0xF>(v, v));
    v = dmax(v, dpp_move<0x141, 0xF>(v, v));
    v = dmax(v, dpp_move<0x140, 0xF>(v, v));
    v = dmax(v, dpp_move<0x142, 0xA>(v, v));
    v = dmax(v, dpp_move<0x143, 0xC>(v, v));
    return lane63(v);
}
__device__ __forceinline__ double lane_of(double v, int l)
{
    union { double d; int i[2]; } x; x.d = v;
    x.i[0] = __builtin_amdgcn_readlane(x.i[0], l); x.i[1] = __builtin_amdgcn_readlane(x.i[1], l);
    return x.d;
}
__device__ __forceinline__ double half_sum(double v)
{
    v += dpp_move<0xB1, 0xF>(0.0, v);
    v += dpp_move<0x4E, 0xF>(0.0, v);
    v += dpp_move<0x141, 0xF>(0.0, v);
    v += dpp_move<0x140, 0xF>(0.0, v);
    v += dpp_move<0x142, 0xA>(0.0, v);
    const double lo = lane_of(v, 31), hi = lane_of(v, 63);
    return (threadIdx.x & 32) ? hi : lo;
}
__device__ __forceinline__ double half_max(double v)
{
    v = dmax(v, dpp_move<0xB1, 0xF>(v, v));
    v = dmax(v, dpp_move<0x4E, 0xF>(v, v));
    v = dmax(v, dpp_move<0x141, 0xF>(v, v));
    v = dmax(v, dpp_move<0x140, 0xF>(v, v));
    v = dmax(v, dpp_move<0x142, 0xA>(v, v));
    const double lo = lane_of(v, 31), hi = lane_of(v, 63);
    return (threadIdx.x & 32) ? hi : lo;
}
__device__ __forceinline__ double uni(double v)
{
    union { double d; int i[2]; } x; x.d = v;
    x.i[0] = __builtin_amdgcn_readfirstlane(x.i[0]); x.i[1] = __builtin_amdgcn_readfirstlane(x.i[1]);
    return x.d;
}

template <int NS, int NU, int NC, int NW, int IPW, int XKEEP = 0>
struct TpShared {
    using Cfg = TpCfg<NS, NU, NC, NW, IPW, XKEEP>;
    static constexpr int NI = Cfg::NI;
    double *T, *q, *red, *keep; int *flag, *iflag, *iters, *keepflag, *misc;
    __device__ explicit TpShared(double *base)
    {
        T = base; q = T + Cfg::T_DOUBLES; red = q + NI * Cfg::QN; keep = red + NI * 4;
        flag = (int *)(keep + NI * Cfg::KEEP_MAX); iflag = flag + NI; iters = iflag + NI; keepflag = iters + NI; misc = keepflag + NI;
    }
    __device__ __forceinline__ double &t(int row, int inst, int k) const
    {
        double *g = T + (((row >> 3) * 8 * NI + inst) * Cfg::LD + k);
        return g[(row & 7) * NI * Cfg::LD];
    }
};

enum : int { kTpOk0 = 1, kTpWarm = 2, kTpValid = 4 };

template <int NS, int NU, bool HASM, int NC, bool MASKED, int NW, int IPW, int XKEEP = 0>
__device__ void tp_solve(const DevProblem &P, const TpShared<NS, NU, NC, NW, IPW, XKEEP> &sh, double *__restrict__ wsg,
                         int max_iter, int &status_o, int &iters_o)
{
    using Cfg = TpCfg<NS, NU, NC, NW, IPW>;
    constexpr int NV = Cfg::NV, NKF = Cfg::NKF, NLI = Cfg::NLI, RA = Cfg::RA, RG = Cfg::RG, RK = Cfg::RK, NI = Cfg::NI;
    const int lane = threadIdx.x, w = __builtin_amdgcn_readfirstlane(threadIdx.y), N = P.N;
    const bool worker = w == 0;
    const bool wl = worker && lane < NI;
    MPC_STAMP_INIT
    __syncthreads();

    const int k = lane;
    const bool blk_on = k < N, last = k == N - 1;
    struct Inst {
        double qz0[NS], qzr[NS], qur[NU];
        double mu, mu_sum, sm, inv_ncon, gscale;
        int stall;
        bool on, warm;
    };
    struct Iter { double sl[NC], sh[NC], ll[NC], lh[NC], u[NU], z[NS], lo[NC], hi[NC]; bool fl[NC], fh[NC]; };
    auto bounds = [&](int wi, Iter &X) {
        const double *qd = sh.q + wi * Cfg::QN;
        MPC_UNROLL for (int i = 0; i < NC; i++) {
            const double zlm = i >= NU ? qd[3 * NS + (i >= NU ? i - NU : 0)] : 0.0, zhm = i >= NU ? qd[4 * NS + (i >= NU ? i - NU : 0)] : 0.0;
            const double lm = i < NU ? P.ulo[i < NU ? i : 0] : zlm, hm = i < NU ? P.uhi[i < NU ? i : 0] : zhm;
            const double le = i < NU ? P.ulo[i < NU ? i : 0] : P.zlo_e[i >= NU ? i - NU : 0], he = i < NU ? P.uhi[i < NU ? i : 0] : P.zhi_e[i >= NU ? i - NU : 0];
            const double lo = last ? le : lm, hi = last ? he : hm;
            X.fl[i] = MASKED ? fin(lo) : true; X.fh[i] = MASKED ? fin(hi) : true;
            X.lo[i] = X.fl[i] ? lo : 0.0; X.hi[i] = X.fh[i] ? hi : 0.0;
        }
    };
    Inst I[IPW];
    unsigned ku = (unsigned)k;
    unsigned lq = (unsigned)lane;
    auto fresh = [&]() { asm volatile("" : "+v"(ku), "+v"(lq)); };
    fresh();
    auto rowp = [&](int wi, int r) -> double * { return wsg + ((size_t)wi * Cfg::ROWS_ST + r) * 64; };
    auto load_iter = [&](int wi, Iter &X) {
        MPC_UNROLL for (int i = 0; i < NC; i++) { X.sl[i] = rowp(wi, Cfg::ST_SL + i)[ku]; X.sh[i] = rowp(wi, Cfg::ST_SH + i)[ku]; X.ll[i] = rowp(wi, Cfg::ST_LL + i)[ku]; X.lh[i] = rowp(wi, Cfg::ST_LH + i)[ku]; }
        MPC_UNROLL for (int i = 0; i < NU; i++) X.u[i] = rowp(wi, Cfg::ST_U + i)[ku];
        MPC_UNROLL for (int i = 0; i < NS; i++) X.z[i] = rowp(wi, Cfg::ST_Z + i)[ku];
        bounds(wi, X);
    };
    auto store_iter = [&](int wi, const Iter &X) {
        MPC_UNROLL for (int i = 0; i < NC; i++) { rowp(wi, Cfg::ST_SL + i)[ku] = X.sl[i]; rowp(wi, Cfg::ST_SH + i)[ku] = X.sh[i]; rowp(wi, Cfg::ST_LL + i)[ku] = X.ll[i]; rowp(wi, Cfg::ST_LH + i)[ku] = X.lh[i]; }
        MPC_UNROLL for (int i = 0; i < NU; i++) rowp(wi, Cfg::ST_U + i)[ku] = X.u[i];
        MPC_UNROLL for (int i = 0; i < NS; i++) rowp(wi, Cfg::ST_Z + i)[ku] = X.z[i];
    };
    double Qk[NS][NS], Rk[NU][NU], Mk[NS][NU];
    MPC_UNROLL for (int i = 0; i < NS; i++) {
        MPC_UNROLL for (int j = 0; j <= i; j++) { const double t = vreg(last ? P.Pf[i][j] : P.Q[i][j]); Qk[i][j] = t; Qk[j][i] = t; }
        MPC_UNROLL for (int j = 0; j < NU; j++) Mk[i][j] = HASM ? vreg(P.M[i][j]) : 0.0;
    }
// ... 485 lines not shown
```

### mpc-code_amd/csrc/mpc_wave.hpp

```cpp
#pragma once
#include "mpc_device.hpp"
#include "mpc_tp.hpp"

namespace mpc {

#ifdef MPC_WV_GENERIC_TILES
constexpr bool kWvGenericTiles = true;
#else
constexpr bool kWvGenericTiles = false;
#endif

template <int NS, int NU, int NC, int NI_>
struct WvCfg {
    static constexpr int NI = NI_;
    static constexpr int NV = NS + NU, NKF = NU * NS, NLI = NU * (NU + 1) / 2;
    static constexpr int RA = 0, RA_SZ = (NC > NKF + NLI ? NC : NKF + NLI);
    static constexpr int RG = RA_SZ, RK = RG + NV, RZ = RK + NU, ROWS = RZ + 1;
    __host__ __device__ static constexpr int ld(int N) { return (N + 1) | 1; }
    static constexpr int GUARD = 8;
    __host__ __device__ static constexpr int t_doubles(int N) { return GUARD + ROWS * NI * ld(N); }
    static constexpr int RL_A = ROWS, RL_B = RL_A + NS * NS, RL_C = RL_B + NS * NU, ROWS_LTV = RL_C + NS;
    __host__ __device__ static constexpr int t_doubles_ltv(int N) { return GUARD + ROWS_LTV * NI * ld(N); }
    static constexpr int QZN = 5 * NS + 2 * NU + 1;
    static constexpr int QN = QZN + NS;
    static constexpr int ROWS_WS = NU + 2 * NC;
    static constexpr int OUT = NU + NS + 1;
    __host__ __device__ static constexpr size_t lds_doubles(int keep_per_inst, int N) { return (size_t)t_doubles(N) + NI * QN + NI * OUT + NI * keep_per_inst; }
};

template <int V>
struct WvInt { static constexpr int value = V; };

template <int NS, int NU, int NC>
struct WvIter { double sl[NC], sh[NC], ll[NC], lh[NC], u[NU], z[NS]; };

struct AReg2 { int lo, hi; };
__device__ __forceinline__ void a_put(AReg2 &r, double v)
{
    union { double d; int i[2]; } u; u.d = v;
    asm("v_accvgpr_write_b32 %0, %1" : "=a"(r.lo) : "v"(u.i[0]));
    asm("v_accvgpr_write_b32 %0, %1" : "=a"(r.hi) : "v"(u.i[1]));
}
__device__ __forceinline__ double a_get(const AReg2 &r)
{
    union { double d; int i[2]; } u;
    asm("v_accvgpr_read_b32 %0, %1" : "=v"(u.i[0]) : "a"(r.lo));
    asm("v_accvgpr_read_b32 %0, %1" : "=v"(u.i[1]) : "a"(r.hi));
    return u.d;
}
template <int NS, int NU, int NC>
struct WvIterA {
    AReg2 sl[NC], sh[NC], ll[NC], lh[NC], u[NU], z[NS];
    __device__ __forceinline__ void get(WvIter<NS, NU, NC> &X) const
    {
        MPC_UNROLL for (int i = 0; i < NC; i++) { X.sl[i] = a_get(sl[i]); X.sh[i] = a_get(sh[i]); X.ll[i] = a_get(ll[i]); X.lh[i] = a_get(lh[i]); }
        MPC_UNROLL for (int i = 0; i < NU; i++) X.u[i] = a_get(u[i]);
        MPC_UNROLL for (int i = 0; i < NS; i++) X.z[i] = a_get(z[i]);
    }
    __device__ __forceinline__ void put(const WvIter<NS, NU, NC> &X)
    {
        MPC_UNROLL for (int i = 0; i < NC; i++) { a_put(sl[i], X.sl[i]); a_put(sh[i], X.sh[i]); a_put(ll[i], X.ll[i]); a_put(lh[i], X.lh[i]); }
        MPC_UNROLL for (int i = 0; i < NU; i++) a_put(u[i], X.u[i]);
        MPC_UNROLL for (int i = 0; i < NS; i++) a_put(z[i], X.z[i]);
    }
};

struct WvInst { double mu, mu_sum, sm, inv_ncon, gscale, res_s, res_p; int stall, iters, status; bool on, warm, keep_u; };

enum : int { kWvOk0 = 1, kWvWarm = 2, kWvValid = 4, kWvKeepU = 8, kWvNoShift = 16 };

__device__ __forceinline__ double row16_sum(double v)
{
    v += dpp_move<0xB1, 0xF>(0.0, v);
    v += dpp_move<0x4E, 0xF>(0.0, v);
    v += dpp_move<0x141, 0xF>(0.0, v);
    v += dpp_move<0x140, 0xF>(0.0, v);
    return v;
}
__device__ __forceinline__ double row16_max(double v)
{
    v = dmax(v, dpp_move<0xB1, 0xF>(v, v));
    v = dmax(v, dpp_move<0x4E, 0xF>(v, v));
    v = dmax(v, dpp_move<0x141, 0xF>(v, v));
    v = dmax(v, dpp_move<0x140, 0xF>(v, v));
    return v;
}

template <int NS, int NU, bool HASM, int NC, bool MASKED, int NI, class PT, bool LTV = false, bool PAIR = false, bool RES_P = false>
__device__ __forceinline__ void wv_solve(const PT &P, double *T, const double *q, const int *iflag,
                                         WvIterA<NS, NU, NC> (&X)[PAIR ? NI / 2 : NI], WvInst (&S)[PAIR ? NI / 2 : NI], int max_iter)
{
    static_assert(!LTV || (NS <= 4 && !HASM), "time-varying stage matrices: one 4 x 4 tile per state matrix, no cross term");
    using Cfg = WvCfg<NS, NU, NC, NI>;
    using Iter = WvIter<NS, NU, NC>;
    constexpr int NV = Cfg::NV, NKF = Cfg::NKF, NLI = Cfg::NLI, RA = Cfg::RA, RG = Cfg::RG, RK = Cfg::RK;
    static_assert(NS <= 8 && NU <= 2 && NI >= 1 && NI <= 4, "stage state <= 8 (2 x 2 tiles of 4 x 4), nu <= 2 (closed-form inverse of Lambda); at most four instances per product");
    static_assert(!PAIR || NI % 2 == 0, "pairs of instances");
    constexpr int NJ = PAIR ? NI / 2 : NI;
    const int lane = threadIdx.x, N = P.N, LD = Cfg::ld(N);
    const int k = PAIR ? (lane & 31) : lane;
    const int hsel = PAIR ? (lane >> 5) : 0;
    auto ji = [&](int j) -> int { return PAIR ? 2 * j + hsel : j; };
    const bool blk_on = k < N, last = k == N - 1;
    auto tk = [&](int row, int j) -> double & { return T[(row * NI + ji(j)) * LD + k]; };
    auto un = [](double v) -> double { return PAIR ? v : uni(v); };
    auto rsum = [](double v) -> double { return PAIR ? half_sum(v) : wave_sum(v); };
    auto rmax = [](double v) -> double { return PAIR ? half_max(v) : wave_max(v); };
    MPC_STAMP_INIT

    auto launder = [](const PT &Pin) -> const PT & { const PT *pp = &Pin; asm volatile("" : "+s"(pp)); return *pp; };
    struct Bnd { double lo[NC], hi[NC]; bool fl[NC], fh[NC]; };
    auto bounds = [&](const PT &Pl, int j, Bnd &Bd) {
        const double *qd = q + ji(j) * Cfg::QN;
        MPC_UNROLL for (int i = 0; i < NC; i++) {
            const double zlm = i >= NU ? qd[3 * NS + (i >= NU ? i - NU : 0)] : 0.0, zhm = i >= NU ? qd[4 * NS + (i >= NU ? i - NU : 0)] : 0.0;
            const double lm = i < NU ? Pl.ulo[i < NU ? i : 0] : zlm, hm = i < NU ? Pl.uhi[i < NU ? i : 0] : zhm;
            const double le = i < NU ? Pl.ulo[i < NU ? i : 0] : Pl.zlo_e[i >= NU ? i - NU : 0], he = i < NU ? Pl.uhi[i < NU ? i : 0] : Pl.zhi_e[i >= NU ? i - NU : 0];
            const double lo = last ? le : lm, hi = last ? he : hm;
            Bd.fl[i] = MASKED ? fin(lo) : true; Bd.fh[i] = MASKED ? fin(hi) : true;
            Bd.lo[i] = Bd.fl[i] ? lo : 0.0; Bd.hi[i] = Bd.fh[i] ? hi : 0.0;
        }
    };
    auto gradient = [&](const PT &Pl, int j, const Iter &Xj, double (&gu)[NU], double (&gz)[NS]) {
        const double *qd = q + ji(j) * Cfg::QN;
        double dz1[NS], du[NU];
        const double *qz = qd + (last ? Cfg::QZN : NS);
        MPC_UNROLL for (int i = 0; i < NS; i++) dz1[i] = Xj.z[i] - qz[i];
        MPC_UNROLL for (int i = 0; i < NU; i++) du[i] = Xj.u[i] - qd[5 * NS + i];
        MPC_UNROLL for (int i = 0; i < NS; i++) {
            double a = (NU + i < NC) ? Xj.lh[NU + i < NC ? NU + i : 0] - Xj.ll[NU + i < NC ? NU + i : 0] : 0.0;
            MPC_UNROLL for (int l = 0; l < NS; l++) a += (last ? Pl.Pf[i][l] : Pl.Q[i][l]) * dz1[l];
            gz[i] = a;
        }
        MPC_UNROLL for (int i = 0; i < NU; i++) {
            double a = Xj.lh[i] - Xj.ll[i];
            MPC_UNROLL for (int l = 0; l < NU; l++) a += Pl.R[i][l] * du[l];
            gu[i] = a;
        }
        if (HASM) {
            double un[NU], zp[NS];
            MPC_UNROLL for (int i = 0; i < NU; i++) un[i] = wave_dn1(du[i], du[i]);
            MPC_UNROLL for (int i = 0; i < NS; i++) { const double t = wave_up1(dz1[i], dz1[i]); zp[i] = k > 0 ? t : qd[i] - qd[NS + i]; }
            if (!last) { MPC_UNROLL for (int i = 0; i < NS; i++) { MPC_UNROLL for (int l = 0; l < NU; l++) gz[i] += Pl.M[i][l] * un[l]; } }
            MPC_UNROLL for (int i = 0; i < NU; i++) { MPC_UNROLL for (int l = 0; l < NS; l++) gu[i] += Pl.M[l][i] * zp[l]; }
        }
    };
    auto phase_a = [&](const PT &Pl, int j, WvInst &Sj, const Iter &Xj, int it) {
        Bnd Bd; bounds(Pl, j, Bd);
        double mu_p = 0.0, resp_p = 0.0, cres_p = 0.0, lmax_p = 0.0, hb[NC];
        MPC_UNROLL for (int i = 0; i < NC; i++) {
            const double v = i < NU ? Xj.u[i < NU ? i : 0] : Xj.z[i >= NU ? i - NU : 0];
            const double rh = Bd.fh[i] ? v + Xj.sh[i] - Bd.hi[i] : 0.0, rl = Bd.fl[i] ? v - Xj.sl[i] - Bd.lo[i] : 0.0;
            const double isl = frcp(Xj.sl[i]), ish = frcp(Xj.sh[i]);
            mu_p += Xj.sl[i] * Xj.ll[i] + Xj.sh[i] * Xj.lh[i];
            if (blk_on) tk(RA + i, j) = Xj.ll[i] * isl + Xj.lh[i] * ish;
            hb[i] = Xj.lh[i] * (rh * ish - 1.0) + Xj.ll[i] * (rl * isl + 1.0);
            resp_p = dmax(resp_p, dmax(fabs(rl), fabs(rh)));
            cres_p = dmax(cres_p, dmax(comp_measure(Xj.sl[i], Xj.ll[i]), comp_measure(Xj.sh[i], Xj.lh[i])));
            lmax_p = dmax(lmax_p, dmax(Xj.ll[i], Xj.lh[i]));
        }
        double gu[NU], gz[NS], pi[NS];
        gradient(Pl, j, Xj, gu, gz);
        if (blk_on) {
            MPC_UNROLL for (int i = 0; i < NU; i++) tk(RG + i, j) = gu[i] + hb[i];
            MPC_UNROLL for (int i = 0; i < NS; i++) tk(RG + NU + i, j) = gz[i] + (NU + i < NC ? hb[NU + i < NC ? NU + i : 0] : 0.0);
        }
        MPC_UNROLL for (int i = 0; i < NS; i++) pi[i] = blk_on ? gz[i] : 0.0;
        Sj.mu_sum = rsum(blk_on ? mu_p : 0.0);
        double resp_m = blk_on ? resp_p : 0.0, cres_m = blk_on ? cres_p : 0.0, lmax_m = blk_on ? lmax_p : 0.0;
        if constexpr (!PAIR) { resp_m = vreg(resp_m); cres_m = vreg(cres_m); lmax_m = vreg(lmax_m); }
        double res_p = 0.0, cres = 0.0, lmax = 0.0;
        bool ok_cp;
        if constexpr (PAIR) {
            res_p = rmax(resp_m); cres = rmax(cres_m); lmax = rmax(lmax_m);
            ok_cp = (cres <= 1.0) && (res_p <= kTolFeas);
        } else ok_cp = !__any((cres_m > 1.0 || resp_m > kTolFeas) ? 1 : 0);
        double rs_p = 0.0;
        if (LTV) {
            if (it == 0 || ok_cp) {
                double An[NS][NS], g0[NS];
                const int kn = k + 1 < N ? k + 1 : (N > 0 ? N - 1 : 0);
                const bool upd = k + 1 < N;
                MPC_UNROLL for (int i = 0; i < NS; i++) { g0[i] = pi[i]; MPC_UNROLL for (int l = 0; l < NS; l++) { const double v = T[((Cfg::RL_A + i * NS + l) * NI + ji(j)) * LD + kn]; An[i][l] = upd ? v : 0.0; } }
                for (int s = N - 2; s >= 0; s--) {
                    double t[NS];
                    MPC_UNROLL for (int i = 0; i < NS; i++) { const double v = wave_dn1(pi[i], pi[i]); t[i] = (PAIR && !upd) ? 0.0 : v; }
                    MPC_UNROLL for (int i = 0; i < NS; i++) { double a = g0[i]; MPC_UNROLL for (int l = 0; l < NS; l++) a += An[l][i] * t[l]; pi[i] = a; }
                }
                MPC_UNROLL for (int i = 0; i < NU; i++) {
                    double a = gu[i];
                    MPC_UNROLL for (int l = 0; l < NS; l++) a += (blk_on ? tk(Cfg::RL_B + l * NU + i, j) : 0.0) * pi[l];
                    rs_p = dmax(rs_p, fabs(a));
                }
            }
        } else if (it == 0 || ok_cp) {
            MPC_UNROLL for (int e = 0; e < 6; e++) {
                const int d = 1 << e;
                if (d < N) {
                    double t[NS];
                    MPC_UNROLL for (int i = 0; i < NS; i++) { const double v = e == 0 ? wave_dn1(pi[i], pi[i]) : __shfl_down(pi[i], d, 64); t[i] = (k + d < N) ? v : 0.0; }
                    MPC_UNROLL for (int i = 0; i < NS; i++) { double a = pi[i]; MPC_UNROLL for (int l = 0; l < NS; l++) a += Pl.Apow[e][l][i] * t[l]; pi[i] = a; }
                }
            }
            MPC_UNROLL for (int i = 0; i < NU; i++) { double a = gu[i]; MPC_UNROLL for (int l = 0; l < NS; l++) a += Pl.B[l][i] * pi[l]; rs_p = dmax(rs_p, fabs(a)); }
        }
        double res_s = Sj.res_s;
        if (it == 0 || ok_cp) res_s = rmax(blk_on ? rs_p : 0.0);
        Sj.mu = Sj.mu_sum * Sj.inv_ncon; Sj.res_s = res_s;
        if constexpr (PAIR) Sj.res_p = res_p;
        else if constexpr (RES_P) Sj.res_p = wave_max(resp_m);
        if (it == 0) Sj.gscale = dmax(1.0, P.term_cons ? dmin(res_s, P.term_gcap) : res_s);
        Sj.stall = ok_cp ? Sj.stall + 1 : 0;
        bool lm_big;
        if constexpr (PAIR) lm_big = lmax > kInfeasZ * Sj.gscale;
        else lm_big = __any(lmax_m > kInfeasZ * Sj.gscale ? 1 : 0) != 0;
        int verdict = -1;
        if (ok_cp && (res_s <= kTolStat * Sj.gscale + P.term_floor || (Sj.stall > kStallMax && res_s <= kTolStatAcc * Sj.gscale + P.term_floor))) verdict = kSolved;
        else if (lm_big || !(fabs(Sj.mu) < 1.0e300)) verdict = kInfeasible;
        else if (it == max_iter) verdict = kMaxIter;
        if (verdict >= 0) { Sj.on = false; Sj.status = verdict; Sj.iters = it; }
    };

    MPC_UNROLL for (int j = 0; j < NJ; j++) {
        WvInst &Sj = S[j];
        Iter Xj;
        const PT &Pl = P;
        const double *qd = q + ji(j) * Cfg::QN;
        const int myflag = PAIR ? iflag[ji(j)] : __builtin_amdgcn_readfirstlane(iflag[j]);
        Sj.on = (myflag & kWvValid) && (myflag & kWvOk0);
        Sj.warm = (myflag & kWvWarm) != 0;
        Sj.mu = 0.0; Sj.mu_sum = 0.0; Sj.sm = 0.0; Sj.gscale = 1.0; Sj.stall = 0; Sj.iters = 0; Sj.res_s = 0.0; Sj.res_p = 0.0;
        Sj.keep_u = (myflag & kWvKeepU) != 0;
        Sj.status = ((myflag & kWvValid) && !(myflag & kWvOk0)) ? kInfeasible : kMaxIter;
        double ncon = 0.0;
        MPC_UNROLL for (int i = 0; i < NC; i++) {
            const double zlm = i >= NU ? un(qd[3 * NS + (i >= NU ? i - NU : 0)]) : 0.0, zhm = i >= NU ? un(qd[4 * NS + (i >= NU ? i - NU : 0)]) : 0.0;
            const double lm = i < NU ? Pl.ulo[i < NU ? i : 0] : zlm, hm = i < NU ? Pl.uhi[i < NU ? i : 0] : zhm;
            const double le = i < NU ? Pl.ulo[i < NU ? i : 0] : Pl.zlo_e[i >= NU ? i - NU : 0], he = i < NU ? Pl.uhi[i < NU ? i : 0] : Pl.zhi_e[i >= NU ? i - NU : 0];
            const bool flm = MASKED ? fin(lm) : true, fhm = MASKED ? fin(hm) : true, fle = MASKED ? fin(le) : true, fhe = MASKED ? fin(he) : true;
            ncon += (double)(N - 1) * ((flm ? 1 : 0) + (fhm ? 1 : 0)) + (fle ? 1 : 0) + (fhe ? 1 : 0);
        }
        Sj.inv_ncon = 1.0 / dmax(ncon, 1.0);
// ... 19 lines not shown
                    if (f_lo && f_hi) push = 0.1 * (uhi - ulo);
                    else push = 0.1 * dmax(1.0, fabs(f_lo ? ulo : (f_hi ? uhi : 0.0)));
                    v = us;
                    if (f_lo) v = dmax(v, ulo + push);
                    if (f_hi) v = dmin(v, uhi - push);
                }
                Xj.u[i] = v;
            }
            MPC_UNROLL for (int i = 0; i < NC; i++) {
                if (Sj.warm) {
                    const double tl = wave_dn1(Xj.ll[i], Xj.ll[i]), th = wave_dn1(Xj.lh[i], Xj.lh[i]);
                    ll0[i] = rep ? Xj.ll[i] : tl; lh0[i] = rep ? Xj.lh[i] : th;
                } else { ll0[i] = 0.0; lh0[i] = 0.0; }
            }
            if (LTV) {
                double Ak[NS][NS], bk[NS], xk[NS];
                MPC_UNROLL for (int i = 0; i < NS; i++) {
                    double a = blk_on ? tk(Cfg::RL_C + i, j) : 0.0;
                    MPC_UNROLL for (int l = 0; l < NU; l++) a += (blk_on ? tk(Cfg::RL_B + i * NU + l, j) : 0.0) * Xj.u[l];
                    bk[i] = a;
                    MPC_UNROLL for (int l = 0; l < NS; l++) Ak[i][l] = blk_on ? tk(Cfg::RL_A + i * NS + l, j) : 0.0;
                }
                MPC_UNROLL for (int i = 0; i < NS; i++) { double a = bk[i]; MPC_UNROLL for (int l = 0; l < NS; l++) a += Ak[i][l] * qd[l]; xk[i] = k == 0 ? a : 0.0; }
                double x00[NS];
                MPC_UNROLL for (int i = 0; i < NS; i++) x00[i] = xk[i];
                if (k == 0 || !blk_on) { MPC_UNROLL for (int i = 0; i < NS; i++) { bk[i] = x00[i]; MPC_UNROLL for (int l = 0; l < NS; l++) Ak[i][l] = 0.0; } }
                for (int s = 1; s < N; s++) {
                    double t[NS];
                    MPC_UNROLL for (int i = 0; i < NS; i++) { const double v = wave_up1(xk[i], xk[i]); t[i] = (PAIR && (k == 0 || !blk_on)) ? 0.0 : v; }
                    MPC_UNROLL for (int i = 0; i < NS; i++) { double a = bk[i]; MPC_UNROLL for (int l = 0; l < NS; l++) a += Ak[i][l] * t[l]; xk[i] = a; }
                }
                MPC_UNROLL for (int i = 0; i < NS; i++) Xj.z[i] = xk[i];
            } else {
                double xk[NS];
                MPC_UNROLL for (int i = 0; i < NS; i++) {
                    double a = qd[2 * NS + i];
                    MPC_UNROLL for (int l = 0; l < NU; l++) a += Pl.B[i][l] * Xj.u[l];
                    if (k == 0) { MPC_UNROLL for (int l = 0; l < NS; l++) a += Pl.A[i][l] * qd[l]; }
                    xk[i] = blk_on ? a : 0.0;
                }
                MPC_UNROLL for (int e = 0; e < 6; e++) {
                    const int d = 1 << e;
                    if (d < N) {
                        double t[NS];
                        MPC_UNROLL for (int i = 0; i < NS; i++) { const double v = e == 0 ? wave_up1(xk[i], xk[i]) : __shfl_up(xk[i], d, 64); t[i] = k >= d ? v : 0.0; }
                        MPC_UNROLL for (int i = 0; i < NS; i++) { double a = xk[i]; MPC_UNROLL for (int l = 0; l < NS; l++) a += Pl.Apow[e][i][l] * t[l]; xk[i] = a; }
                    }
                }
                MPC_UNROLL for (int i = 0; i < NS; i++) Xj.z[i] = xk[i];
            }
            Bnd Bd; bounds(Pl, j, Bd);
            const double ws_delta = un(qd[5 * NS + 2 * NU]);
            const double ws_smin = dmin(dmax(kWsKappa * ws_delta, kWsSMinLo), kWsSMinHi), ws_mu = kWsMuFactor * ws_smin * ws_smin;
            const double smin = Sj.warm ? ws_smin : kSMin;
            MPC_UNROLL for (int i = 0; i < NC; i++) {
                const double v = i < NU ? Xj.u[i < NU ? i : 0] : Xj.z[i >= NU ? i - NU : 0];
                Xj.sl[i] = Bd.fl[i] ? dmax(v - Bd.lo[i], smin) : 1.0; Xj.sh[i] = Bd.fh[i] ? dmax(Bd.hi[i] - v, smin) : 1.0;
                const double isl = frcp(Xj.sl[i]), ish = frcp(Xj.sh[i]);
                const double llo = Sj.warm ? dmax(ll0[i], ws_mu * isl) : kMu0 * isl, lhi = Sj.warm ? dmax(lh0[i], ws_mu * ish) : kMu0 * ish;
                Xj.ll[i] = Bd.fl[i] ? llo : 0.0; Xj.lh[i] = Bd.fh[i] ? lhi : 0.0;
            }
            X[j].put(Xj);
            phase_a(Pl, j, Sj, Xj, 0);
        }
        __builtin_amdgcn_sched_barrier(0);
    }

    MPC_TSTAMP(1);
    auto mm = [](double a, double b, double c) { return __builtin_amdgcn_mfma_f64_4x4x4f64(a, b, c, 0, 0, 0); };
    constexpr int RZ = Cfg::RZ;
    constexpr int SB = (NS + 3) / 4;
    constexpr bool VF = SB == 1 && !HASM && !kWvGenericTiles;
#define MPC_MM "v_mfma_f64_4x4x4_4b_f64 "
#define MPC_WV_RD(dst, addr) "ds_read_b64 %[" #dst "], %[" #addr "] offset:%[off]\n\t"
#define MPC_WV_NORD(dst, addr) "s_nop 0\n\t"
    auto wv_lds_addr = [](const double *p) { return (unsigned)(unsigned long long)p; };
    struct TileCtx {
        int tr, tc; bool live;
        double *Tt, *trash;
        double Ar[SB][SB], Atr[SB][SB], Br[SB], Btr[SB];
        double *p_hu, *p_hz[SB], *p_kf, *p_k[SB], *p_kt[SB], *p_li;
        const double *p_a, *p_at, *p_b, *p_bt;
    };
    auto tile_ctx = [&](const PT &Pl) {
        int lo = threadIdx.x;
        asm volatile("" : "+v"(lo));
        TileCtx c;
        c.tr = lo >> 4; c.tc = lo & 3;
        const int tbq = (lo >> 2) & 3;
        c.live = tbq < NI;
        const int tb = c.live ? tbq : 0;
        const int tr = c.tr, tc = c.tc;
        c.Tt = T + tb * LD; c.trash = T - Cfg::GUARD;
        auto trow = [&](int row) -> double * { return c.Tt + (c.live ? row : RZ) * (NI * LD); };
        MPC_UNROLL for (int i = 0; i < SB; i++) {
            const int ri = 4 * i + tr, ci = 4 * i + tc;
            MPC_UNROLL for (int j = 0; j < SB; j++) {
                const int cj = 4 * j + tc, rj = 4 * j + tr;
                c.Ar[i][j] = (ri < NS && cj < NS) ? Pl.A[ri < NS ? ri : 0][cj < NS ? cj : 0] : 0.0;
                c.Atr[i][j] = (ri < NS && cj < NS) ? Pl.A[cj < NS ? cj : 0][ri < NS ? ri : 0] : 0.0;
                (void)rj;
            }
            c.Br[i] = (ri < NS && tc < NU) ? Pl.B[ri < NS ? ri : 0][tc < NU ? tc : 0] : 0.0;
            c.Btr[i] = (tr < NU && ci < NS) ? Pl.B[ci < NS ? ci : 0][tr < NU ? tr : 0] : 0.0;
            c.p_hz[i] = trow(ri < NS ? RG + NU + ri : RZ);
            c.p_k[i] = trow((tr < NU && ci < NS) ? RA + tr * NS + ci : RZ);
            c.p_kt[i] = trow((ri < NS && tc < NU) ? RA + tc * NS + ri : RZ);
        }
        c.p_hu = trow(tr < NU ? RG + tr : RZ); c.p_kf = trow(tr < NU ? RK + tr : RZ);
        if (LTV) {
            c.p_a = trow((tr < NS && tc < NS) ? Cfg::RL_A + tr * NS + tc : RZ); c.p_at = trow((tr < NS && tc < NS) ? Cfg::RL_A + tc * NS + tr : RZ);
            c.p_b = trow((tr < NS && tc < NU) ? Cfg::RL_B + tr * NU + tc : RZ); c.p_bt = trow((tr < NU && tc < NS) ? Cfg::RL_B + tc * NU + tr : RZ);
        }
        const int li_i = tr > tc ? tr : tc, li_j = tr > tc ? tc : tr;
        c.p_li = trow((tr < NU && tc < NU) ? RA + NKF + li_i * (li_i + 1) / 2 + li_j : RZ);
        return c;
    };
    double pd_min = 1.0;
    constexpr int PD = SB == 1 ? 4 : 2;

    auto tile_factor = [&]() {
        const PT &Pl = launder(P);
        const TileCtx c = tile_ctx(Pl);
        const int tr = c.tr, tc = c.tc; const bool live = c.live;
        double *const trash = c.trash;
        auto trow = [&](int row) -> double * { return c.Tt + (live ? row : RZ) * (NI * LD); };
        const bool in_uu = tr < NU && tc < NU;
        const double Rr = in_uu ? Pl.R[tr][tc] : 0.0;
        double Qr[SB][SB], Mtr[SB], BE0[SB], BE1[SB];
        MPC_UNROLL for (int i = 0; i < SB; i++) {
            const int ri = 4 * i + tr, ci = 4 * i + tc;
            MPC_UNROLL for (int j = 0; j < SB; j++) { const int cj = 4 * j + tc; Qr[i][j] = (ri < NS && cj < NS) ? Pl.Q[ri < NS ? ri : 0][cj < NS ? cj : 0] : 0.0; }
            Mtr[i] = (HASM && tr < NU && ci < NS) ? Pl.M[ci < NS ? ci : 0][tr < NU ? tr : 0] : 0.0;
            BE0[i] = ri < NS ? Pl.B[ri < NS ? ri : 0][0] : 0.0; BE1[i] = (NU > 1 && ri < NS) ? Pl.B[ri < NS ? ri : 0][NU > 1 ? 1 : 0] : 0.0;
        }
        const double RE0 = tc < NU ? Pl.R[0][tc] : 0.0, RE1 = (NU > 1 && tc < NU) ? Pl.R[NU > 1 ? 1 : 0][tc] : 0.0;
        const double Ir = tr == tc ? 1.0 : 0.0;
        const double *q_sz[SB];
        MPC_UNROLL for (int i = 0; i < SB; i++) { const int ri = 4 * i + tr; q_sz[i] = trow((tr == tc && ri < NS && NU + ri < NC) ? RA + NU + ri : RZ) + (N - 1); }
        const double *q_su = trow((tr == tc && tr < NU) ? RA + tr : RZ) + (N - 1);
        const double *q_s0 = trow(tc == 0 ? RA : RZ) + (N - 1), *q_s1 = trow((NU > 1 && tc == 1) ? RA + 1 : RZ) + (N - 1);
        const double *q_hu = c.p_hu + (N - 1);
        const double *q_hz[SB];
        MPC_UNROLL for (int i = 0; i < SB; i++) q_hz[i] = c.p_hz[i] + (N - 1);
        const int ri2 = tr & 1;
        const double c_a = (NU > 1 && tc == 1 && ri2 == 1) ? -1.0 : 0.0, c_d = (NU > 1 && tc == 0 && ri2 == 0) ? -1.0 : 0.0;
        const double c_o = (NU > 1 && tc < 2 && ri2 != tc) ? 1.0 : 0.0, c_1 = (NU == 1 && tc == 0) ? -1.0 : 0.0;
        const double w_top = tr < NU ? 1.0 : 0.0;
        const double k_a = c_a * w_top, k_d = c_d * w_top, k_o = c_o * w_top, k_1 = c_1 * w_top;
        const bool st_l = tr >= 2 && tc < NU && tc <= tr - 2 && tr - 2 < NU, st_f3 = NS < 4 && tr < NU && tc == 3;
        double *q_st[SB]; int stp[SB];
        MPC_UNROLL for (int j = 0; j < SB; j++) {
            const int cj = 4 * j + tc;
            const bool st_k = tr < NU && cj < NS;
            const bool any = live && (st_k || (j == 0 && (st_l || st_f3)));
            q_st[j] = any ? trow(st_k ? RA + tr * NS + cj : (st_l ? RA + NKF + (tr - 2) * (tr - 1) / 2 + tc : RK + (tr < NU ? tr : 0))) + (N - 1) : trash + PD;
            stp[j] = any ? PD : 0;
        }
        const bool sel_k0 = tr < NU && tc < NS;
        const bool st_f = live && NS >= 4 && tr < NU && tc == 0;
        double *q_sf = st_f ? c.p_kf + (N - 1) : trash + PD;
        const int stpf = st_f ? PD : 0;
        double Pm[SB][SB], PC[SB];
        MPC_UNROLL for (int i = 0; i < SB; i++) {
            const int ri = 4 * i + tr;
            MPC_UNROLL for (int j = 0; j < SB; j++) { const int cj = 4 * j + tc; Pm[i][j] = (ri < NS && cj < NS) ? Pl.Pf[ri < NS ? ri : 0][cj < NS ? cj : 0] : 0.0; }
            PC[i] = 0.0;
        }
        constexpr int NF = 2 * SB + 4 + (LTV ? 3 : 0);
        double f[PD][NF];
        const double *q_a = LTV ? c.p_a + (N - 1) : nullptr, *q_b = LTV ? c.p_b + (N - 1) : nullptr, *q_bt = LTV ? c.p_bt + (N - 1) : nullptr;
        auto fetch = [&](int d, int off) {
            MPC_UNROLL for (int i = 0; i < SB; i++) { f[d][i] = q_sz[i][off]; f[d][SB + 4 + i] = q_hz[i][off]; }
            f[d][SB] = q_su[off]; f[d][SB + 1] = q_s0[off]; f[d][SB + 2] = NU > 1 ? q_s1[off] : 0.0; f[d][SB + 3] = q_hu[off];
            if (LTV) { f[d][NF - 3] = q_a[off]; f[d][NF - 2] = q_b[off]; f[d][NF - 1] = q_bt[off]; }
        };
        MPC_UNROLL for (int d = 0; d < PD; d++) fetch(d, -d);
        if constexpr (VF && !LTV) {
            unsigned a_sz = wv_lds_addr(q_sz[0]) - 64, a_su = wv_lds_addr(q_su) - 64, a_s0 = wv_lds_addr(q_s0) - 64, a_s1 = wv_lds_addr(q_s1) - 64;
            unsigned a_hu = wv_lds_addr(q_hu) - 64, a_hz = wv_lds_addr(q_hz[0]) - 64;
            const double Br0 = c.Br[0], Btr0 = c.Btr[0], Ar0 = c.Ar[0][0], BE00 = BE0[0], BE10 = BE1[0], Qr0 = Qr[0][0];
            double Pm0 = Pm[0][0], PC0 = 0.0;
            auto step = [&](auto D, auto MORE) {
                constexpr int d = decltype(D)::value, dp = (d + PD - 1) % PD;
                constexpr bool more = decltype(MORE)::value;
                Pm0 += f[d][0];
                const double X0i = RE0 + f[d][2], X1i = RE1 + f[d][3], PV0 = f[d][5] + PC0, Rs = Rr + f[d][1];
                double PB, BtP, PA, psv, X0, X1, Psi;
#define MPC_FAC_STMT1(RD) \
                "s_nop 1\n\t" \
                MPC_MM "%[pb], %[pm], %[br], 0\n\t" \
                MPC_MM "%[btp], %[br], %[pm], 0\n\t" \
                MPC_MM "%[pa], %[pm], %[ar], 0\n\t" \
                MPC_MM "%[psv], %[br], %[pv], %[hu]\n\t" \
                RD(sz, asz) RD(su, asu) RD(s0, as0) \
                MPC_MM "%[x0], %[be0], %[pb], %[x0i]\n\t" \
                MPC_MM "%[x1], %[be1], %[pb], %[x1i]\n\t" \
                RD(s1, as1) \
                MPC_MM "%[psi], %[br], %[pa], 0\n\t" \
                RD(hz, ahz) \
                "s_nop 4" \
                : [pb] "=&v"(PB), [btp] "=&v"(BtP), [pa] "=&v"(PA), [psv] "=&v"(psv), [x0] "=&v"(X0), [x1] "=&v"(X1), [psi] "=&v"(Psi), \
                  [sz] "+v"(f[d][0]), [su] "+v"(f[d][1]), [s0] "+v"(f[d][2]), [s1] "+v"(f[d][3]), [hz] "+v"(f[d][5]) \
                : [pm] "v"(Pm0), [br] "v"(Br0), [ar] "v"(Ar0), [pv] "v"(PV0), [hu] "v"(f[d][4]), [be0] "v"(BE00), [be1] "v"(BE10), [x0i] "v"(X0i), [x1i] "v"(X1i), \
                  [asz] "v"(a_sz), [asu] "v"(a_su), [as0] "v"(a_s0), [as1] "v"(a_s1), [ahz] "v"(a_hz), [off] "i"((PD - d) * 8) : "memory"
                if constexpr (more) asm volatile(MPC_FAC_STMT1(MPC_WV_RD));
                else asm volatile(MPC_FAC_STMT1(MPC_WV_NORD));
#undef MPC_FAC_STMT1
                const double a = dpp_move<0x00, 0xF>(X0, X0);
                double adjm, adjk, det;
                if (NU == 1) { det = a; adjm = c_1; adjk = k_1; pd_min = dmin(pd_min, a); }
                else {
                    const double off = dpp_move<0x55, 0xF>(X0, X0), dd = dpp_move<0x55, 0xF>(X1, X1);
                    det = __builtin_fma(a, dd, -(off * off));
                    adjk = __builtin_fma(k_d, dd, __builtin_fma(k_a, a, k_o * off));
                    adjm = __builtin_fma(c_d, dd, __builtin_fma(c_a, a, c_o * off));
                    pd_min = dmin(pd_min, dmin(a, det));
                }
                double Kk0;
                asm volatile("s_waitcnt lgkmcnt(0)\n\ts_nop 0\n\t" MPC_MM "%[kk], %[adjk], %[psi], 0"
                             : [kk] "=v"(Kk0), "+v"(det), "+v"(f[d][0]), "+v"(f[d][1]), "+v"(f[d][2]), "+v"(f[d][3]), "+v"(f[d][5]), "+v"(f[dp][4])
                             : [adjk] "v"(adjk), [psi] "v"(Psi) : "memory");
                const double rdet = frcp(det);
                asm("s_nop 1" : "+v"(Kk0) : "v"(rdet));
                Kk0 *= rdet;
                const double mL = adjm * rdet, mLi = adjk * rdet;
                double RK0, Acl0, Tm0, a2, KFF, acc, acc2, PCn;
#define MPC_FAC_STMT3(RD) \
                "s_nop 1\n\t" \
                MPC_MM "%[rk], %[rs], %[kk], 0\n\t" \
                MPC_MM "%[acl], %[btr], %[kk], %[ar]\n\t" \
                MPC_MM "%[tm], %[btp], %[kk], %[pa]\n\t" \
                MPC_MM "%[a2], %[kk], %[hu], 0\n\t" \
                RD(hu, ahu) \
                MPC_MM "%[kff], %[mli], %[psv], 0\n\t" \
                "s_nop 1\n\t" \
                MPC_MM "%[acc], %[kk], %[rk], %[q]\n\t" \
                MPC_MM "%[acc2], %[acl], %[tm], 0\n\t" \
                MPC_MM "%[pcn], %[acl], %[pv], %[a2]\n\t" \
                "s_nop 5" \
                : [rk] "=&v"(RK0), [acl] "=&v"(Acl0), [tm] "=&v"(Tm0), [a2] "=&v"(a2), [kff] "=&v"(KFF), [acc] "=&v"(acc), [acc2] "=&v"(acc2), [pcn] "=&v"(PCn), [hu] "+v"(f[d][4]) \
                : [rs] "v"(Rs), [kk] "v"(Kk0), [btr] "v"(Btr0), [ar] "v"(Ar0), [btp] "v"(BtP), [pa] "v"(PA), [mli] "v"(mLi), [psv] "v"(psv), [q] "v"(Qr0), [pv] "v"(PV0), \
                  [ahu] "v"(a_hu), [off] "i"((PD - d) * 8) : "memory"
                if constexpr (more) asm volatile(MPC_FAC_STMT3(MPC_WV_RD));
                else asm volatile(MPC_FAC_STMT3(MPC_WV_NORD));
#undef MPC_FAC_STMT3
                q_st[0][-d] = sel_k0 ? Kk0 : (st_l ? mL : KFF);
                if (NS >= 4) q_sf[-d] = KFF;
                Pm0 = acc + acc2;
// ... 307 lines not shown
            MPC_MM "%[du], %[kt], %[dz], %[kf]\n\t" \
            RD(kf, akf) \
            RD(kt, akt) \
            MPC_MM "%[acltn], %[k1], %[btr], %[atr]\n\t" \
            MPC_MM "%[a0n], %[btr], %[kf1], 0\n\t" \
            "s_waitcnt lgkmcnt(" W ")\n\t" \
            "s_nop 1" \
            : [dzn] "=&v"(DZn), [du] "=&v"(DUv), [acltn] "=&v"(AcltN), [a0n] "=&v"(a0N), [kf] "+v"(f[d][0]), [k] "+v"(f[d][1]), [kt] "+v"(f[d][2]), \
              "+v"(f[dp][0]), "+v"(f[dp][1]), "+v"(f[dp][2]) \
            : [aclt] "v"(Aclt), [a0] "v"(a0), [dz] "v"(DZ0), [kf1] "v"(f[dn][0]), [k1] "v"(f[dn][1]), [btr] "v"(Btr0), [atr] "v"(Atr0), \
              [akf] "v"(a_kf), [ak] "v"(a_k), [akt] "v"(a_kt), [off] "i"((PD + d) * 8) : "memory"
            auto step = [&](auto D, auto MORE) {
                constexpr int d = decltype(D)::value, dn = (d + 1) % PD, dp = (d + PD - 1) % PD;
                double DZn, DUv, AcltN, a0N;
                if constexpr (decltype(MORE)::value) asm volatile(MPC_FWD_STMT(MPC_WV_RD, "3"));
                else asm volatile(MPC_FWD_STMT(MPC_WV_NORD, "0"));
                q_st[0][d] = st_u ? DUv : DZn;
                DZ0 = DZn; Aclt = AcltN; a0 = a0N;
            };
#undef MPC_FWD_STMT
            const int G = N / PD, rem = N - G * PD;
            for (int g = 0; g < G; g++) {
                step(WvInt<0>{}, WvInt<1>{}); step(WvInt<1>{}, WvInt<1>{}); step(WvInt<2>{}, WvInt<1>{}); step(WvInt<3>{}, WvInt<1>{});
                a_kf += PD * 8; a_k += PD * 8; a_kt += PD * 8; q_st[0] += stp[0];
            }
            if (0 < rem) step(WvInt<0>{}, WvInt<0>{});
            if (1 < rem) step(WvInt<1>{}, WvInt<0>{});
            if (2 < rem) step(WvInt<2>{}, WvInt<0>{});
            asm volatile("s_waitcnt lgkmcnt(0)\n\ts_nop 5"
                         : "+v"(f[0][0]), "+v"(f[0][1]), "+v"(f[0][2]), "+v"(f[1][0]), "+v"(f[1][1]), "+v"(f[1][2]), "+v"(f[2][0]), "+v"(f[2][1]), "+v"(f[2][2]),
                           "+v"(f[3][0]), "+v"(f[3][1]), "+v"(f[3][2]), "+v"(Aclt), "+v"(a0));
            return;
        }
        auto block = [&](int d, bool more) {
            const double KFF = f[d][0];
            double Kk[SB], KkT[SB];
            MPC_UNROLL for (int i = 0; i < SB; i++) { Kk[i] = f[d][1 + i]; KkT[i] = f[d][1 + SB + i]; }
            double Atrl[SB][SB], Btrl[SB];
            MPC_UNROLL for (int i = 0; i < SB; i++) { Btrl[i] = c.Btr[i]; MPC_UNROLL for (int jj = 0; jj < SB; jj++) Atrl[i][jj] = c.Atr[i][jj]; }
            if (LTV) { Atrl[0][0] = f[d][NF - 2]; Btrl[0] = f[d][NF - 1]; }
            if (more) fetch(d, PD + d);
            if constexpr (VF) {
                double Aclt, a0, DUv, DZn0;
                asm("s_nop 1\n\t"
                    MPC_MM "%0, %4, %5, %6\n\t"
                    MPC_MM "%1, %5, %7, 0\n\t"
                    MPC_MM "%2, %8, %9, %7\n\t"
                    "s_nop 3\n\t"
                    MPC_MM "%3, %0, %9, %1\n\t"
                    "s_nop 5"
                    : "=&v"(Aclt), "=&v"(a0), "=&v"(DUv), "=&v"(DZn0)
                    : "v"(Kk[0]), "v"(Btrl[0]), "v"(Atrl[0][0]), "v"(KFF), "v"(KkT[0]), "v"(DZ[0]));
                q_st[0][d] = st_u ? DUv : DZn0;
                DZ[0] = DZn0;
                return;
            }
            double DU = KFF;
            MPC_UNROLL for (int j = 0; j < SB; j++) DU = mm(KkT[j], DZ[j], DU);
            double DZn[SB];
            MPC_UNROLL for (int i = 0; i < SB; i++) {
                double a = mm(Btrl[i], KFF, 0.0);
                MPC_UNROLL for (int j = 0; j < SB; j++) a = mm(mm(Kk[j], Btrl[i], Atrl[j][i]), DZ[j], a);
                DZn[i] = a;
            }
            q_st[0][d] = st_u ? DU : DZn[0];
            MPC_UNROLL for (int i = 1; i < SB; i++) q_st[i][d] = DZn[i];
            MPC_UNROLL for (int i = 0; i < SB; i++) DZ[i] = DZn[i];
        };
        const int G = N / PD, rem = N - G * PD;
        for (int g = 0; g < G; g++) {
            MPC_UNROLL for (int d = 0; d < PD; d++) block(d, true);
            MPC_UNROLL for (int i = 0; i < SB; i++) { q_k[i] += PD; q_kt[i] += PD; q_st[i] += stp[i]; }
            q_kf += PD;
            if (LTV) { q_at += PD; q_bt += PD; }
        }
        MPC_UNROLL for (int d = 0; d < PD - 1; d++) { if (d < rem) block(d, false); }
    };

    AReg2 dvp[NJ][NC];
    for (int it = 0;; it++) {
        bool any_on = false;
        MPC_UNROLL for (int j = 0; j < NJ; j++) any_on = any_on || (PAIR ? __any(S[j].on) != 0 : S[j].on);
        if (!any_on) break;
        __syncthreads();
        pd_min = 1.0;
        tile_factor();
        __syncthreads();
        MPC_TSTAMP(2);
        tile_forward();
        __syncthreads();
        MPC_TSTAMP(3);
        {
            const unsigned long long bad = __ballot(((lane >> 2) & 3) < NI && !(pd_min > 0.0));
            MPC_UNROLL for (int j = 0; j < NJ; j++) {
                if (S[j].on && (bad & (0x000F000F000F000FULL << (4 * ji(j))))) { S[j].on = false; S[j].status = kInfeasible; S[j].iters = it; }
            }
        }
        MPC_UNROLL for (int j = 0; j < NJ; j++) {
            WvInst &Sj = S[j];
            if (Sj.on) {
                Iter Xj; X[j].get(Xj);
                const PT &Pl = P;
                Bnd Bd; bounds(Pl, j, Bd);
                double maff_p = 1.0, s1_p = 0.0, s2_p = 0.0, pl[NC], ph[NC], dvj[NC];
                MPC_UNROLL for (int i = 0; i < NC; i++) { dvj[i] = tk(RG + i, j); a_put(dvp[j][i], dvj[i]); }
                MPC_UNROLL for (int i = 0; i < NC; i++) {
                    const double v = i < NU ? Xj.u[i < NU ? i : 0] : Xj.z[i >= NU ? i - NU : 0];
                    const double isl = frcp(Xj.sl[i]), ish = frcp(Xj.sh[i]);
                    const double rh = Bd.fh[i] ? v + Xj.sh[i] - Bd.hi[i] : 0.0, rl = Bd.fl[i] ? v - Xj.sl[i] - Bd.lo[i] : 0.0;
                    const double dsh = Bd.fh[i] ? -rh - dvj[i] : 0.0, dsl = Bd.fl[i] ? rl + dvj[i] : 0.0;
                    const double qh = dsh * ish, ql = dsl * isl;
                    const double dlh = Bd.fh[i] ? -Xj.lh[i] - Xj.lh[i] * qh : 0.0, dll = Bd.fl[i] ? -Xj.ll[i] - Xj.ll[i] * ql : 0.0;
                    maff_p = dmax(maff_p, dmax(-ql, -qh));
                    if (Bd.fl[i]) maff_p = dmax(maff_p, 1.0 + ql);
                    if (Bd.fh[i]) maff_p = dmax(maff_p, 1.0 + qh);
                    s1_p += Xj.sl[i] * dll + Xj.ll[i] * dsl + Xj.sh[i] * dlh + Xj.lh[i] * dsh;
                    s2_p += dsl * dll + dsh * dlh;
                    pl[i] = dsl * dll; ph[i] = dsh * dlh;
                }
                const double m_aff = rmax(blk_on ? maff_p : 1.0), s1 = rsum(blk_on ? s1_p : 0.0), s2 = rsum(blk_on ? s2_p : 0.0);
                const double a_aff = frcp(m_aff);
                const double mu_aff = (Sj.mu_sum + a_aff * s1 + a_aff * a_aff * s2) * Sj.inv_ncon;
                const double rat = Sj.mu > 0.0 ? mu_aff * frcp(Sj.mu) : 0.0;
                Sj.sm = dmax(rat * rat * rat * Sj.mu, kMuFloor);
                double gu[NU], gz[NS], hc[NV];
                gradient(Pl, j, Xj, gu, gz);
                MPC_UNROLL for (int i = NC; i < NV; i++) hc[i] = 0.0;
                MPC_UNROLL for (int i = 0; i < NC; i++) {
                    const double v = i < NU ? Xj.u[i < NU ? i : 0] : Xj.z[i >= NU ? i - NU : 0];
                    const double isl = frcp(Xj.sl[i]), ish = frcp(Xj.sh[i]);
                    const double rh = Bd.fh[i] ? v + Xj.sh[i] - Bd.hi[i] : 0.0, rl = Bd.fl[i] ? v - Xj.sl[i] - Bd.lo[i] : 0.0;
                    const double rch = Bd.fh[i] ? Xj.sh[i] * Xj.lh[i] - dmax(Sj.sm, Xj.lh[i] * kSFloor) + ph[i] : 0.0;
                    const double rcl = Bd.fl[i] ? Xj.sl[i] * Xj.ll[i] - dmax(Sj.sm, Xj.ll[i] * kSFloor) + pl[i] : 0.0;
                    hc[i] = (-rch + Xj.lh[i] * rh) * ish + (rcl + Xj.ll[i] * rl) * isl;
                }
                if (blk_on) {
                    MPC_UNROLL for (int i = 0; i < NU; i++) tk(RG + i, j) = gu[i] + hc[i];
                    MPC_UNROLL for (int i = 0; i < NS; i++) tk(RG + NU + i, j) = gz[i] + hc[NU + i];
                }
            }
            __builtin_amdgcn_sched_barrier(0);
        }
        __syncthreads();
        MPC_TSTAMP(4);
        tile_rhs();
        __syncthreads();
        MPC_TSTAMP(5);
        tile_forward();
        __syncthreads();
        MPC_TSTAMP(3);
        MPC_UNROLL for (int j = 0; j < NJ; j++) {
            WvInst &Sj = S[j];
            if (Sj.on) {
                Iter Xj; X[j].get(Xj);
                const PT &Pl = P;
                Bnd Bd; bounds(Pl, j, Bd);
                double dvzj[NV], dvj[NC];
                MPC_UNROLL for (int i = 0; i < NC; i++) dvj[i] = a_get(dvp[j][i]);
                MPC_UNROLL for (int i = 0; i < NV; i++) dvzj[i] = tk(RG + i, j);
                double mcc_p = kTau;
                double dsl[NC], dsh[NC], dll[NC], dlh[NC];
                MPC_UNROLL for (int i = 0; i < NC; i++) {
                    const double v = i < NU ? Xj.u[i < NU ? i : 0] : Xj.z[i >= NU ? i - NU : 0];
                    const double isl = frcp(Xj.sl[i]), ish = frcp(Xj.sh[i]);
                    const double rh = Bd.fh[i] ? v + Xj.sh[i] - Bd.hi[i] : 0.0, rl = Bd.fl[i] ? v - Xj.sl[i] - Bd.lo[i] : 0.0;
                    const double ash = Bd.fh[i] ? -rh - dvj[i] : 0.0, asl = Bd.fl[i] ? rl + dvj[i] : 0.0;
                    const double alh = Bd.fh[i] ? -Xj.lh[i] - Xj.lh[i] * (ash * ish) : 0.0, all_ = Bd.fl[i] ? -Xj.ll[i] - Xj.ll[i] * (asl * isl) : 0.0;
                    const double rch = Bd.fh[i] ? Xj.sh[i] * Xj.lh[i] - dmax(Sj.sm, Xj.lh[i] * kSFloor) + ash * alh : 0.0;
                    const double rcl = Bd.fl[i] ? Xj.sl[i] * Xj.ll[i] - dmax(Sj.sm, Xj.ll[i] * kSFloor) + asl * all_ : 0.0;
                    dsh[i] = Bd.fh[i] ? -rh - dvzj[i] : 0.0; dsl[i] = Bd.fl[i] ? rl + dvzj[i] : 0.0;
                    dlh[i] = Bd.fh[i] ? (-rch - Xj.lh[i] * dsh[i]) * ish : 0.0; dll[i] = Bd.fl[i] ? (-rcl - Xj.ll[i] * dsl[i]) * isl : 0.0;
                    mcc_p = dmax(mcc_p, dmax(-dsl[i] * isl, -dsh[i] * ish));
                    if (Bd.fl[i]) mcc_p = dmax(mcc_p, -dll[i] * frcp_approx(Xj.ll[i]));
                    if (Bd.fh[i]) mcc_p = dmax(mcc_p, -dlh[i] * frcp_approx(Xj.lh[i]));
                }
                const double m_cc = rmax(blk_on ? mcc_p : kTau);
                const double alpha = m_cc <= kTau ? 1.0 : kTau * frcp(m_cc);
                MPC_UNROLL for (int i = 0; i < NC; i++) { Xj.sl[i] += alpha * dsl[i]; Xj.sh[i] += alpha * dsh[i]; Xj.ll[i] += alpha * dll[i]; Xj.lh[i] += alpha * dlh[i]; }
                MPC_UNROLL for (int i = 0; i < NU; i++) Xj.u[i] += alpha * dvzj[i];
                MPC_UNROLL for (int i = 0; i < NS; i++) Xj.z[i] += alpha * dvzj[NU + i];
                X[j].put(Xj);
                phase_a(Pl, j, Sj, Xj, it + 1);
            }
            __builtin_amdgcn_sched_barrier(0);
        }
        MPC_TSTAMP(6);
    }
}
#undef MPC_MM
#undef MPC_WV_RD
#undef MPC_WV_NORD



template <int NX, int NU, int NY, int ND, int NGS = 0, int NHS = 0>
struct Row16Tab {
    static constexpr int NE = NX + ND, NR = NU - NHS, NCT = NX + NU + NY + NGS;
    static constexpr int E_A = 0, E_Q = NE, E_K = 2 * NE, E_DMIN = 2 * NE + NY, E_DMAX = E_DMIN + 1, ESZ = E_DMAX + 1;
    static constexpr int T_W = 0, T_LO = NR, T_HI = NR + 1, TSZ = NR + 2;
    static constexpr int DOUBLES = NE * ESZ + NCT * TSZ;
#ifdef MPC_ROW16_OFF
    static constexpr bool fits = false;
#else
    static constexpr bool fits = NE <= 16 && NCT <= 16;
#endif
    static constexpr int XCH = NE * NY + NE * NE;
};

template <int NX, int NU, int NY, int ND, int NGS = 0, int NHS = 0, class PT>
__device__ __forceinline__ void row16_fill_tables(const PT &P, double *tab, int lane)
{
    using RT = Row16Tab<NX, NU, NY, ND, NGS, NHS>;
    constexpr int NE = RT::NE;
    if (lane < NE) {
        double *e = tab + lane * RT::ESZ;
        for (int j = 0; j < NE; j++) { e[RT::E_A + j] = P.Aa[lane][j]; e[RT::E_Q + j] = P.Qkf[lane][j]; }
        for (int j = 0; j < NY; j++) e[RT::E_K + j] = P.Kfix[lane][j];
        e[RT::E_DMIN] = lane >= NX ? P.dmin[lane - NX] : 0.0; e[RT::E_DMAX] = lane >= NX ? P.dmax[lane - NX] : 0.0;
    }
    if (lane < RT::NCT) {
        double *t = tab + NE * RT::ESZ + lane * RT::TSZ;
        constexpr int NVY = NX + NU + NY;
        if (NGS == 0 || lane < NVY) {
            for (int c = 0; c < RT::NR; c++) t[RT::T_W + c] = P.W[lane][c];
            t[RT::T_LO] = P.tlo[lane]; t[RT::T_HI] = P.thi[lane];
        } else if constexpr (NGS > 0) {
            for (int c = 0; c < RT::NR; c++) t[RT::T_W + c] = P.Wg[lane - NVY][c];
            t[RT::T_LO] = -INFINITY; t[RT::T_HI] = 0.0;
        }
    }
}

template <int NX, int NY, int ND, int NXP, int NU, class PT>
__device__ __forceinline__ void kalman_row16(const PT &P, int r, bool slot_on, double *kp, int x_off, int xi_off, int p_off, const double *pyp_k,
                                             const double *vn_k, size_t Bs, const double *tab, double *xch, double &xi_old, double &xi_new)
{
    using RT = Row16Tab<NX, NU, NY, ND>;
    constexpr int NE = RT::NE;
    const bool row = r < NE && slot_on;
    const int rr = r < NE ? r : 0;
    const double *e = tab + rr * RT::ESZ;
    double xi[NE], innov[NY];
    MPC_UNROLL for (int i = 0; i < NE; i++) xi[i] = kp[xi_off + i];
    MPC_UNROLL for (int i = 0; i < NY; i++) {
        double yh = P.fyc[i], yy = pyp_k[i];
        if (vn_k) yy += vn_k[i * Bs];
        MPC_UNROLL for (int j = 0; j < NE; j++) yh += P.Ca[i][j] * xi[j];
        MPC_UNROLL for (int j = 0; j < NXP; j++) yy += P.Cp[i][j] * kp[x_off + j];
        innov[i] = yy - yh;
    }
    xi_old = kp[xi_off + rr];
    double Kr[NY];
    if (P.estimator == MPC_EST_KALMAN) {
        double Pr[NE], PCt[NY];
        MPC_UNROLL for (int j = 0; j < NE; j++) Pr[j] = kp[p_off + rr * NE + j];
        MPC_UNROLL for (int j = 0; j < NY; j++) { double a = 0.0; MPC_UNROLL for (int l = 0; l < NE; l++) a += Pr[l] * P.Ca[j][l]; PCt[j] = a; }
        if (row) { MPC_UNROLL for (int j = 0; j < NY; j++) xch[r * NY + j] = PCt[j]; }
        __syncthreads();
        double all[NE][NY], S[NY][NY];
        MPC_UNROLL for (int l = 0; l < NE; l++) { MPC_UNROLL for (int j = 0; j < NY; j++) all[l][j] = xch[l * NY + j]; }
        MPC_UNROLL for (int i = 0; i < NY; i++) { MPC_UNROLL for (int j = 0; j < NY; j++) { double a = P.Rkf[i][j]; MPC_UNROLL for (int l = 0; l < NE; l++) a += P.Ca[i][l] * all[l][j]; S[i][j] = a; } }
        MPC_UNROLL for (int i = 0; i < NY; i++) { MPC_UNROLL for (int j = 0; j < i; j++) { const double a = 0.5 * (S[i][j] + S[j][i]); S[i][j] = a; S[j][i] = a; } }
        sym_inverse<NY>(S);
        MPC_UNROLL for (int j = 0; j < NY; j++) { double a = 0.0; MPC_UNROLL for (int l = 0; l < NY; l++) a += PCt[l] * S[l][j]; Kr[j] = a; }
        double Pc[NE], U[NE];
        MPC_UNROLL for (int j = 0; j < NE; j++) { double a = Pr[j]; MPC_UNROLL for (int m = 0; m < NY; m++) a -= Kr[m] * all[j][m]; Pc[j] = a; }
        MPC_UNROLL for (int j = 0; j < NE; j++) { double a = 0.0; MPC_UNROLL for (int l = 0; l < NE; l++) a += Pc[l] * P.Aa[j][l]; U[j] = a; }
        double *xu = xch + NE * NY;
        if (row) { MPC_UNROLL for (int j = 0; j < NE; j++) xu[r * NE + j] = U[j]; }
        __syncthreads();
        double Pn[NE];
        MPC_UNROLL for (int j = 0; j < NE; j++) Pn[j] = e[RT::E_Q + j];
        MPC_UNROLL for (int l = 0; l < NE; l++) { const double al = e[RT::E_A + l]; MPC_UNROLL for (int j = 0; j < NE; j++) Pn[j] += al * xu[l * NE + j]; }
        if (row) { MPC_UNROLL for (int j = 0; j < NE; j++) kp[p_off + r * NE + j] = Pn[j]; }
    } else {
        MPC_UNROLL for (int j = 0; j < NY; j++) Kr[j] = e[RT::E_K + j];
    }
    double v = xi_old;
    MPC_UNROLL for (int l = 0; l < NY; l++) v += Kr[l] * innov[l];
    if (P.has_dsat && r >= NX) v = dmin(dmax(v, e[RT::E_DMIN]), e[RT::E_DMAX]);
    xi_new = v;
    __syncthreads();
    if (row) kp[xi_off + r] = v;
}

template <int NX, int NU, int NY, int ND, int NGS = 0, int NHS = 0, class PT>
__device__ __forceinline__ int target_row16(const PT &P, int r, const double *tab, const double *usp, const double *ysp, const double *dh,
                                            const double *us_prev, double *tw, int *twv, bool inst_on, double &v_out, int &iters)
{
    using RT = Row16Tab<NX, NU, NY, ND, NGS, NHS>;
    constexpr int NV = NX + NU, NC = RT::NCT, NR = RT::NR, NE = RT::NE;
    const bool row = r < NC;
    const int rr = row ? r : 0;
    const double *t = tab + NE * RT::ESZ + rr * RT::TSZ;
    double Wr[NR];
    MPC_UNROLL for (int c = 0; c < NR; c++) Wr[c] = row ? t[RT::T_W + c] : 0.0;
    const double tlo = t[RT::T_LO], thi = t[RT::T_HI];
    const bool fl = row && fin(tlo), fh = row && fin(thi);
    const double lo = fl ? tlo : 0.0, hi = fh ? thi : 0.0;
    double cx[NX], e[NY], vp[NV], yp[NY], gr[NR], y[NR];
    MPC_UNROLL for (int i = 0; i < NX; i++) { double a = P.fxc[i]; MPC_UNROLL for (int j = 0; j < ND; j++) a += P.Bd[i][j] * dh[j]; cx[i] = a; }
    MPC_UNROLL for (int i = 0; i < NY; i++) { double a = P.fyc[i]; MPC_UNROLL for (int j = 0; j < ND; j++) a += P.Cd[i][j] * dh[j]; e[i] = a; }
    MPC_UNROLL for (int q = 0; q < NV; q++) { double a = 0.0; MPC_UNROLL for (int j = 0; j < NX; j++) a -= P.Ep[q][j] * cx[j]; vp[q] = a; }
    if constexpr (NHS > 0) {
        double ch[NHS];
        MPC_UNROLL for (int h = 0; h < NHS; h++) { double a = P.h0_ss[h]; MPC_UNROLL for (int j = 0; j < ND; j++) a += P.Hd_ss[h][j] * dh[j]; ch[h] = a; }
        MPC_UNROLL for (int q = 0; q < NV; q++) { double a = vp[q]; MPC_UNROLL for (int h = 0; h < NHS; h++) a -= P.Eh[q][h] * ch[h]; vp[q] = a; }
    }
    MPC_UNROLL for (int i = 0; i < NY; i++) { double a = e[i]; MPC_UNROLL for (int j = 0; j < NX; j++) a += P.Cm[i][j] * vp[j]; yp[i] = a; }
    MPC_UNROLL for (int c = 0; c < NR; c++) {
        double a = 0.0;
        MPC_UNROLL for (int i = 0; i < NY; i++) { double qi = 0.0; MPC_UNROLL for (int j = 0; j < NY; j++) qi += P.Qss[i][j] * (yp[j] - ysp[j]); a += qi * P.CZx[i][c]; }
        MPC_UNROLL for (int i = 0; i < NU; i++) {
            double ri = 0.0;
            MPC_UNROLL for (int j = 0; j < NU; j++) ri += P.Rss[i][j] * (vp[NX + j] - (P.duss_form ? us_prev[j] : usp[j]));
            a += ri * P.Zn[NX + i][c];
        }
        gr[c] = a;
    }
    double w0 = 0.0;
    MPC_UNROLL for (int q = 0; q < NV; q++) w0 = r == q ? vp[q] : w0;
    MPC_UNROLL for (int i = 0; i < NY; i++) w0 = r == NV + i ? yp[i] : w0;
    if constexpr (NGS > 0) {
        MPC_UNROLL for (int g = 0; g < NGS; g++) {
            double a = P.g0_ss[g];
            MPC_UNROLL for (int j = 0; j < ND; j++) a += P.Gd_ss[g][j] * dh[j];
            MPC_UNROLL for (int j = 0; j < NV; j++) a += P.Gv_ss[g][j] * vp[j];
            w0 = r == NV + NY + g ? a : w0;
        }
    }
    const double ncon = row16_sum((fl ? 1.0 : 0.0) + (fh ? 1.0 : 0.0));
    const double inv_ncon = 1.0 / dmax(ncon, 1.0);
    {
        double Hi[NR][NR];
        MPC_UNROLL for (int i = 0; i < NR; i++) { MPC_UNROLL for (int j = 0; j < NR; j++) Hi[i][j] = P.Hr[i][j]; }
        sym_inverse<NR>(Hi);
        MPC_UNROLL for (int i = 0; i < NR; i++) { double a = 0.0; MPC_UNROLL for (int j = 0; j < NR; j++) a += Hi[i][j] * gr[j]; y[i] = -a; }
    }
    double s_lo, s_hi, l_lo, l_hi;
    {
        double v = w0; MPC_UNROLL for (int c = 0; c < NR; c++) v += Wr[c] * y[c];
        s_lo = fl ? dmax(v - lo, kSMin) : 1.0; s_hi = fh ? dmax(hi - v, kSMin) : 1.0;
        l_lo = fl ? kMu0 * frcp(s_lo) : 0.0; l_hi = fh ? kMu0 * frcp(s_hi) : 0.0;
    }
    if (*twv != 0) {
        double dl = row ? fabs(w0 - tw[2 * NR + 2 * NC + rr]) : 0.0;
        MPC_UNROLL for (int c = 0; c < NR; c++) dl = dmax(dl, fabs(gr[c] - tw[NR + 2 * NC + c]));
        const double delta = row16_max(dl);
        if (delta <= kWsDelta) {
            const double smin = dmin(dmax(kWsKappa * delta, kWsSMinLo), kWsSMinHi), wmu = kWsMuFactor * smin * smin;
            MPC_UNROLL for (int c = 0; c < NR; c++) y[c] = tw[c];
            double v = w0; MPC_UNROLL for (int c = 0; c < NR; c++) v += Wr[c] * y[c];
            s_lo = fl ? dmax(v - lo, smin) : 1.0; s_hi = fh ? dmax(hi - v, smin) : 1.0;
            l_lo = fl ? dmax(tw[NR + rr], wmu * frcp(s_lo)) : 0.0; l_hi = fh ? dmax(tw[NR + NC + rr], wmu * frcp(s_hi)) : 0.0;
        }
    }
    double gscale = 1.0; int stall = 0, status = kMaxIter;
    MPC_UNROLL for (int c = 0; c < NR; c++) gscale = dmax(gscale, fabs(gr[c]));
    bool on = inst_on;
    iters = 0;
    for (int it = 0;; it++) {
        if (!__any(on ? 1 : 0)) break;
        double v = w0; MPC_UNROLL for (int c = 0; c < NR; c++) v += Wr[c] * y[c];
        const double r_lo = fl ? v - s_lo - lo : 0.0, r_hi = fh ? v + s_hi - hi : 0.0;
        const double is_lo = frcp(s_lo), is_hi = frcp(s_hi);
        const double sig = l_lo * is_lo + l_hi * is_hi;
        const double mu = row16_sum(s_lo * l_lo + s_hi * l_hi) * inv_ncon;
        const double res_p = row16_max(dmax(fabs(r_lo), fabs(r_hi)));
        const double cres = row16_max(dmax(comp_measure(s_lo, l_lo), comp_measure(s_hi, l_hi)));
        const double lmax = row16_max(dmax(l_lo, l_hi));
        double grad[NR], res_s = 0.0;
        MPC_UNROLL for (int c = 0; c < NR; c++) {
            double a = gr[c]; MPC_UNROLL for (int j = 0; j < NR; j++) a += P.Hr[c][j] * y[j];
            a += row16_sum((l_hi - l_lo) * Wr[c]);
            grad[c] = a; res_s = dmax(res_s, fabs(a));
        }
        if (on) {
            iters = it;
            const bool ok_cp = (cres <= 1.0) && (res_p <= kTolFeas);
            stall = ok_cp ? stall + 1 : 0;
            if (ok_cp && (res_s <= kTolStat * gscale || (stall > kStallMax && res_s <= kTolStatAcc * gscale))) { status = kSolved; on = false; }
            else if (lmax > kInfeasZ * gscale || !(fabs(mu) < 1.0e300)) { status = kInfeasible; on = false; }
            else if (it == P.max_iter) { status = kMaxIter; on = false; }
        }
        double Ht[NR][NR];
        MPC_UNROLL for (int i = 0; i < NR; i++) { MPC_UNROLL for (int j = 0; j <= i; j++) { const double a = P.Hr[i][j] + row16_sum(sig * Wr[i] * Wr[j]); Ht[i][j] = a; Ht[j][i] = a; } }
        const bool pd = sym_inverse<NR>(Ht);
        if (on && !pd) { status = kInfeasible; on = false; }
        double dy[NR], ds_lo = 0.0, ds_hi = 0.0, dl_lo = 0.0, dl_hi = 0.0, sm = 0.0, alpha = 1.0;
        MPC_UNROLL for (int pass = 0; pass < 2; pass++) {
            double rc_lo, rc_hi, rhs[NR];
            if (pass == 0) { rc_lo = fl ? s_lo * l_lo : 0.0; rc_hi = fh ? s_hi * l_hi : 0.0; }
            else {
                rc_lo = fl ? s_lo * l_lo - dmax(sm, l_lo * kSFloor) + ds_lo * dl_lo : 0.0;
                rc_hi = fh ? s_hi * l_hi - dmax(sm, l_hi * kSFloor) + ds_hi * dl_hi : 0.0;
            }
            const double h = (-rc_hi + l_hi * r_hi) * is_hi + (rc_lo + l_lo * r_lo) * is_lo;
            MPC_UNROLL for (int c = 0; c < NR; c++) rhs[c] = grad[c] + row16_sum(h * Wr[c]);
            MPC_UNROLL for (int i = 0; i < NR; i++) { double a = 0.0; MPC_UNROLL for (int j = 0; j < NR; j++) a += Ht[i][j] * rhs[j]; dy[i] = -a; }
            double dv = 0.0; MPC_UNROLL for (int c = 0; c < NR; c++) dv += Wr[c] * dy[c];
            ds_hi = fh ? -r_hi - dv : 0.0; ds_lo = fl ? r_lo + dv : 0.0;
            dl_hi = fh ? (-rc_hi - l_hi * ds_hi) * is_hi : 0.0;
            dl_lo = fl ? (-rc_lo - l_lo * ds_lo) * is_lo : 0.0;
            double m = dmax(pass == 0 ? 1.0 : kTau, dmax(-ds_lo * is_lo, -ds_hi * is_hi));
            if (fl) m = dmax(m, -dl_lo * frcp_approx(l_lo));
            if (fh) m = dmax(m, -dl_hi * frcp_approx(l_hi));
            m = row16_max(m);
            if (pass == 0) {
                const double amax = frcp(m);
                const double s1 = row16_sum((s_lo + amax * ds_lo) * (l_lo + amax * dl_lo) + (s_hi + amax * ds_hi) * (l_hi + amax * dl_hi));
                const double mu_aff = s1 * inv_ncon, rat = mu > 0.0 ? mu_aff * frcp(mu) : 0.0;
                sm = dmax(rat * rat * rat * mu, kMuFloor);
            } else alpha = m <= kTau ? 1.0 : kTau * frcp(m);
        }
        if (on) {
            MPC_UNROLL for (int c = 0; c < NR; c++) y[c] += alpha * dy[c];
            s_lo += alpha * ds_lo; s_hi += alpha * ds_hi; l_lo += alpha * dl_lo; l_hi += alpha * dl_hi;
        }
    }
    {
        double v = w0; MPC_UNROLL for (int c = 0; c < NR; c++) v += Wr[c] * y[c];
        v_out = v;
    }
    if (inst_on) {
        if (row) { tw[NR + r] = l_lo; tw[NR + NC + r] = l_hi; tw[2 * NR + 2 * NC + r] = w0; }
        if (r == 0) { MPC_UNROLL for (int c = 0; c < NR; c++) { tw[c] = y[c]; tw[NR + 2 * NC + c] = gr[c]; } *twv = status == kSolved ? 1 : 0; }
    }
    return status;
}

}
```

Before: 35.80 million.

## Replace block barriers with wave LDS waits and stage model tiles in LDS

```diff
diff --git a/__graft_entry__.py b/__graft_entry__.py
--- a/__graft_entry__.py
+++ b/__graft_entry__.py
@@ -6,6 +6,7 @@
     sys.path.insert(0, ROOT)
 
 WV_DIRECTION_EXTRA_SETS = ((1, 1, 1, 1, 1, 0, 0), (4, 1, 1, 1, 4, 0, 0), (4, 2, 2, 2, 4, 0, 0), (8, 2, 2, 2, 8, 0, 0))
+WV_STEP_STALLS_EXTRA_SETS = ((1, 2, 1, 1, 1, 0, 0),)
 WV_VGPR_FORM_SETS = ((1, 1, 1, 1, 1, 0, 0), (2, 1, 1, 1, 2, 0, 0), (2, 1, 1, 1, 2, 0, 1), (3, 2, 3, 3, 3, 0, 0), (4, 1, 1, 1, 4, 0, 0), (4, 2, 2, 2, 4, 0, 0))
 
 
@@ -21,6 +22,8 @@
     for dims in ((3, 2, 3, 3, 3, 1, 0), (5, 2, 2, 2, 5, 0, 0), (3, 2, 3, 3, 3, 0, 0, 1, 1), (3, 2, 3, 3, 3, 0, 2, 1, 1), (6, 2, 8, 0, 6, 0, 0, 1, 1)):
         jobs.append(lambda dims=dims: capi.build_library(dims=dims))
     for dims in WV_DIRECTION_EXTRA_SETS:
+        jobs.append(lambda dims=dims: capi.build_library(dims=dims))
+    for dims in WV_STEP_STALLS_EXTRA_SETS:
         jobs.append(lambda dims=dims: capi.build_library(dims=dims))
     for dims in WV_VGPR_FORM_SETS:
         jobs.append(lambda dims=dims: capi.build_library(dims=dims, extra_flags=(capi.WV_GENERIC_TILES_FLAG,)))
diff --git a/mpc-code_amd/csrc/mpc_amd.hip b/mpc-code_amd/csrc/mpc_amd.hip
--- a/mpc-code_amd/csrc/mpc_amd.hip
+++ b/mpc-code_amd/csrc/mpc_amd.hip
@@ -519,7 +519,7 @@
             aimv[j] = again ? 1 : 0;
         }
     }
-    __syncthreads();
+    wave_lds_sync();
     int any = 0;
     MPC_UNROLL for (int j = 0; j < NI; j++) any |= aimv[j];
     any = __builtin_amdgcn_readfirstlane(any);
@@ -529,7 +529,7 @@
         const int f = iflag[lane];
         if ((f & kWvValid) && (f & kWvOk0) && st != kInfeasible) { iflag[lane] = kWvValid | kWvOk0 | kWvWarm | kWvNoShift; itacc[lane] += it; }
     }
-    __syncthreads();
+    wave_lds_sync();
     return any != 0;
 }
 
@@ -543,7 +543,7 @@
                          K_TW = K_P + NE * NE, KEEP = K_TW + NTW;
     static constexpr int t_region(int N)
     {
-        const int t = Cfg::t_doubles(N), x = Cfg::GUARD + (RT::fits ? 4 * RT::XCH : 0);
+        const int t = Cfg::t_doubles(N), x = Cfg::T_OFF + (RT::fits ? 4 * RT::XCH : 0);
         return t > x ? t : x;
     }
     static constexpr size_t lds_bytes(int N) { return sizeof(double) * ((size_t)t_region(N) + NI * Cfg::QN + NI * Cfg::OUT + NI * KEEP + (RT::fits ? RT::DOUBLES : 0)) + sizeof(int) * 24; }
@@ -559,7 +559,7 @@
     extern __shared__ double wv_smem[];
     const DevProblem &P0 = *Pp;
     const int LD = Cfg::ld(P0.N);
-    double *const T = wv_smem + Cfg::GUARD, *const q = wv_smem + KC::t_region(P0.N), *const outv = q + NI * Cfg::QN, *const keep = outv + NI * Cfg::OUT;
+    double *const T = wv_smem + Cfg::T_OFF, *const q = wv_smem + KC::t_region(P0.N), *const outv = q + NI * Cfg::QN, *const keep = outv + NI * Cfg::OUT;
     int *const iflag = (int *)(keep + NI * KEEP), *const twv = iflag + 4, *const wsv = twv + 4, *const aimv = wsv + 4, *const itacc = aimv + 4;
     using RT = typename KC::RT;
     double *const tab = (double *)(wsv + 16);
@@ -580,9 +580,10 @@
         twv[lane] = a.tw_valid[b]; wsv[lane] = a.ws_valid[b];
     } else if (lane < NI) { twv[lane] = 0; wsv[lane] = 0; }
     for (int i = lane; i < NI * LD; i += 64) T[Cfg::RZ * NI * LD + i] = 0.0;
-    if (lane < Cfg::GUARD) wv_smem[lane] = 0.0;
+    if (lane < Cfg::GUARD) wv_smem[Cfg::TCN + lane] = 0.0;
+    wv_fill_tile_consts<NS, NU, DU, NC, NI>(P, wv_smem, lane);
     if (RT::fits) row16_fill_tables<NX, NU, NY, ND, NGS, NHS>(P, tab, lane);
-    __syncthreads();
+    wave_lds_sync();
     WvIterA<NS, NU, NC> X[NI];
     WvInst S[NI];
     MPC_UNROLL for (int j = 0; j < NI; j++) {
@@ -602,7 +603,8 @@
         if (redo == 0) {
         if constexpr (RT::fits) {
             const int b16 = lane >> 4, r16 = lane & 15, b16c = b16 < NI ? b16 : 0;
-            const unsigned bi = (unsigned)(blockIdx.x * NI + b16c);
+            unsigned bi = (unsigned)(blockIdx.x * NI + b16c);
+            asm volatile("" : "+v"(bi));
             const bool inst16 = b16 < NI && (int)bi < a.B;
             double *const kq = keep + b16c * KEEP;
             if (inst16) {
@@ -614,7 +616,7 @@
                 kalman_row16<NX, NY, ND, NXP, NU>(P, r16, b16 < NI, kq, KC::K_X, KC::K_XH, KC::K_P, a.pyp + k * NY, (NOISE && a.vn) ? a.vn + (size_t)k * NY * Bs + bi : nullptr, Bs, tab, T + b16c * RT::XCH, xi_old, xi_new);
             if (inst16 && a.DHAT && r16 >= NX && r16 < NE) (a.DHAT + (size_t)((size_t)k * ND + (r16 - NX)) * Bs)[bi] = xi_new;
             double delta = row16_max(r16 < NE ? fabs(xi_new - xi_old) : 0.0);
-            __syncthreads();
+            wave_lds_sync();
             if (Cfg::RZ * NI * LD < 4 * RT::XCH) { for (int i = lane; i < NI * LD; i += 64) T[Cfg::RZ * NI * LD + i] = 0.0; }
             double dh[NDD], usv[NU];
             MPC_UNROLL for (int i = 0; i < ND; i++) dh[i] = kq[KC::K_DH + i];
@@ -641,7 +643,7 @@
                 if (a.st_dyn && r16 == 0) { (a.st_ss + (size_t)k * Bs)[bi] = st_ss; (a.it_ss + (size_t)k * Bs)[bi] = it_ss; }
             }
             if (r16 == 0 && b16 < NI) outv[b16c * Cfg::OUT] = delta;
-            __syncthreads();
+            wave_lds_sync();
         }
         if (valid) {
             double xh[NX], dh[NDD], u[NU], xs[NX], us[NU], delta = 0.0;
@@ -721,7 +723,7 @@
             MPC_UNROLL for (int i = 0; i < ND; i++) kp[KC::K_DH + i] = dh[i];
             MPC_UNROLL for (int i = 0; i < NU; i++) kp[KC::K_US + i] = us[i];
         } else if (lane < NI) iflag[lane] = 0;
-        __syncthreads();
+        wave_lds_sync();
         }
         MPC_TSTAMP(0);
         wv_solve<NS, NU, DU, NC, MASKED, NI>(P, T, q, iflag, X, S, P.max_iter);
@@ -743,7 +745,7 @@
                 aimv[j] = again ? 1 : 0;
             }
         }
-        __syncthreads();
+        wave_lds_sync();
         if (P.term_cons && redo < 2) {
             int any = 0;
             MPC_UNROLL for (int j = 0; j < NI; j++) any |= aimv[j];
@@ -754,7 +756,7 @@
                     const int f = iflag[lane];
                     if ((f & kWvValid) && (f & kWvOk0) && st != kInfeasible) { iflag[lane] = kWvValid | kWvOk0 | kWvWarm | kWvNoShift; itacc[lane] += it; }
                 }
-                __syncthreads();
+                wave_lds_sync();
                 redo++; k--;
                 continue;
             }
@@ -795,7 +797,7 @@
             MPC_UNROLL for (int i = 0; i < NU; i++) kp[KC::K_U + i] = u[i];
             wsv[lane] = st_dyn == kSolved ? 1 : 0;
         }
-        __syncthreads();
+        wave_lds_sync();
         MPC_TSTAMP(7);
     }
     if (valid) {
@@ -844,7 +846,7 @@
     extern __shared__ double wv_smem[];
     const ConstProblem &P = *(const ConstProblem *)Pp;
     const int N = Pp->N, LD = Cfg::ld(N);
-    double *const T = wv_smem + Cfg::GUARD, *const q = wv_smem + Cfg::t_doubles(N), *const outv = q + NI * Cfg::QN;
+    double *const T = wv_smem + Cfg::T_OFF, *const q = wv_smem + Cfg::t_doubles(N), *const outv = q + NI * Cfg::QN;
     int *const iflag = (int *)(outv + NI * Cfg::OUT), *const aimv = iflag + 4, *const itacc = aimv + 4;
     const size_t Bs = a.Bs;
     const int lane = threadIdx.x;
@@ -852,7 +854,8 @@
     const int b = blockIdx.x * NI + il;
     const bool valid = lane < NI && b < a.B;
     for (int i = lane; i < NI * LD; i += 64) T[Cfg::RZ * NI * LD + i] = 0.0;
-    if (lane < Cfg::GUARD) wv_smem[lane] = 0.0;
+    if (lane < Cfg::GUARD) wv_smem[Cfg::TCN + lane] = 0.0;
+    wv_fill_tile_consts<NS, NU, DU, NC, NI>(P, wv_smem, lane);
     if (valid) {
         double xh[NX], xs[NX], us[NU], up[NU], dh[NDD];
         MPC_UNROLL for (int i = 0; i < NX; i++) { xh[i] = a.xhat[i * Bs + b]; xs[i] = a.xs[i * Bs + b]; }
@@ -875,7 +878,7 @@
         MPC_UNROLL for (int i = 0; i < NX; i++) w.prev[(NX + ND + i) * Bs + b] = xs[i];
         MPC_UNROLL for (int i = 0; i < NU; i++) w.prev[(2 * NX + ND + i) * Bs + b] = us[i];
     } else if (lane < NI) iflag[lane] = 0;
-    __syncthreads();
+    wave_lds_sync();
     WvIterA<NS, NU, NC> X[NI];
     WvInst S[NI];
     MPC_UNROLL for (int j = 0; j < NI; j++) {
@@ -913,7 +916,7 @@
             outv[j * Cfg::OUT + NU + NS] = v;
         }
     }
-    __syncthreads();
+    wave_lds_sync();
     if (valid) {
         int st = S[0].status, it = S[0].iters; double r0 = S[0].res_s, r1 = S[0].res_p, r2 = S[0].mu;
         MPC_UNROLL for (int j = 1; j < NI; j++) { if (lane == j) { st = S[j].status; it = S[j].iters; r0 = S[j].res_s; r1 = S[j].res_p; r2 = S[j].mu; } }
diff --git a/mpc-code_amd/csrc/mpc_device.hpp b/mpc-code_amd/csrc/mpc_device.hpp
--- a/mpc-code_amd/csrc/mpc_device.hpp
+++ b/mpc-code_amd/csrc/mpc_device.hpp
@@ -70,10 +70,31 @@
 
 __device__ __forceinline__ double dmax(double a, double b) { return __builtin_fmax(a, b); }
 __device__ __forceinline__ double dmin(double a, double b) { return __builtin_fmin(a, b); }
+__device__ __forceinline__ double dmax_vv(double a, double b)
+{
+    double r;
+    asm("v_max_f64 %0, %1, %2" : "=v"(r) : "v"(a), "v"(b));
+    return r;
+}
+__device__ __forceinline__ double dmin_vv(double a, double b)
+{
+    double r;
+    asm("v_min_f64 %0, %1, %2" : "=v"(r) : "v"(a), "v"(b));
+    return r;
+}
+__device__ __forceinline__ void wave_lds_sync()
+{
+    asm volatile("s_waitcnt lgkmcnt(0)" ::: "memory");
+}
 __device__ __forceinline__ bool fin(double a) { return fabs(a) < 1.0e300; }
 __device__ __forceinline__ double comp_measure(double s, double l)
 {
     return dmin(dmin(s, l) * (1.0 / kTolC), s * l * (1.0 / kTolMu));
+}
+
+__device__ __forceinline__ double comp_measure_vv(double s, double l)
+{
+    return dmin(dmin_vv(s, l) * (1.0 / kTolC), s * l * (1.0 / kTolMu));
 }
 
 __device__ __forceinline__ double frcp(double x)
diff --git a/mpc-code_amd/csrc/mpc_nmpc.hip b/mpc-code_amd/csrc/mpc_nmpc.hip
--- a/mpc-code_amd/csrc/mpc_nmpc.hip
+++ b/mpc-code_amd/csrc/mpc_nmpc.hip
@@ -446,7 +446,7 @@
     const DevProblem &Pg = *Pp;
     const ConstProblem &P = *(const ConstProblem *)Pp;
     const int N = Pg.N, LD = Cfg::ld(N);
-    double *const T = nw_smem + Cfg::GUARD, *const q = nw_smem + Cfg::t_doubles_ltv(N), *const outv = q + NI * Cfg::QN, *const keep = outv + NI * Cfg::OUT;
+    double *const T = nw_smem + Cfg::T_OFF, *const q = nw_smem + Cfg::t_doubles_ltv(N), *const outv = q + NI * Cfg::QN, *const keep = outv + NI * Cfg::OUT;
     int *const iflag = (int *)(keep + NI * KK::KEEP), *const act = iflag + 4, *const shf = act + 4, *const wsv = shf + 4, *const stv = wsv + 4, *const itv = stv + 4, *const sqv = itv + 4;
     const size_t Bs = a.Bs;
     const int lane = threadIdx.x, k = PAIR ? (lane & 31) : lane, hsel = PAIR ? (lane >> 5) : 0;
@@ -471,7 +471,8 @@
         wsv[lane] = a.ws_valid[b];
     } else if (lane < NI) wsv[lane] = 0;
     for (int i = lane; i < NI * LD; i += 64) T[Cfg::RZ * NI * LD + i] = 0.0;
-    if (lane < Cfg::GUARD) nw_smem[lane] = 0.0;
+    if (lane < Cfg::GUARD) nw_smem[Cfg::TCN + lane] = 0.0;
+    wv_fill_tile_consts<NS, NU, false, NC, NI>(P, nw_smem, lane);
     __syncthreads();
     WvIterA<NS, NU, NC> X[NJ];
     WvInst S[NJ];
diff --git a/mpc-code_amd/csrc/mpc_tp.hpp b/mpc-code_amd/csrc/mpc_tp.hpp
--- a/mpc-code_amd/csrc/mpc_tp.hpp
+++ b/mpc-code_amd/csrc/mpc_tp.hpp
@@ -65,12 +65,12 @@
 }
 __device__ __forceinline__ double wave_max(double v)
 {
-    v = dmax(v, dpp_move<0xB1, 0xF>(v, v));
-    v = dmax(v, dpp_move<0x4E, 0xF>(v, v));
-    v = dmax(v, dpp_move<0x141, 0xF>(v, v));
-    v = dmax(v, dpp_move<0x140, 0xF>(v, v));
-    v = dmax(v, dpp_move<0x142, 0xA>(v, v));
-    v = dmax(v, dpp_move<0x143, 0xC>(v, v));
+    v = dmax_vv(v, dpp_move<0xB1, 0xF>(v, v));
+    v = dmax_vv(v, dpp_move<0x4E, 0xF>(v, v));
+    v = dmax_vv(v, dpp_move<0x141, 0xF>(v, v));
+    v = dmax_vv(v, dpp_move<0x140, 0xF>(v, v));
+    v = dmax_vv(v, dpp_move<0x142, 0xA>(v, v));
+    v = dmax_vv(v, dpp_move<0x143, 0xC>(v, v));
     return lane63(v);
 }
 __device__ __forceinline__ double lane_of(double v, int l)
@@ -91,11 +91,11 @@
 }
 __device__ __forceinline__ double half_max(double v)
 {
-    v = dmax(v, dpp_move<0xB1, 0xF>(v, v));
-    v = dmax(v, dpp_move<0x4E, 0xF>(v, v));
-    v = dmax(v, dpp_move<0x141, 0xF>(v, v));
-    v = dmax(v, dpp_move<0x140, 0xF>(v, v));
-    v = dmax(v, dpp_move<0x142, 0xA>(v, v));
+    v = dmax_vv(v, dpp_move<0xB1, 0xF>(v, v));
+    v = dmax_vv(v, dpp_move<0x4E, 0xF>(v, v));
+    v = dmax_vv(v, dpp_move<0x141, 0xF>(v, v));
+    v = dmax_vv(v, dpp_move<0x140, 0xF>(v, v));
+    v = dmax_vv(v, dpp_move<0x142, 0xA>(v, v));
     const double lo = lane_of(v, 31), hi = lane_of(v, 63);
     return (threadIdx.x & 32) ? hi : lo;
 }
diff --git a/mpc-code_amd/csrc/mpc_wave.hpp b/mpc-code_amd/csrc/mpc_wave.hpp
--- a/mpc-code_amd/csrc/mpc_wave.hpp
+++ b/mpc-code_amd/csrc/mpc_wave.hpp
@@ -18,9 +18,12 @@
     static constexpr int RG = RA_SZ, RK = RG + NV, RZ = RK + NU, ROWS = RZ + 1;
     __host__ __device__ static constexpr int ld(int N) { return (N + 1) | 1; }
     static constexpr int GUARD = 8;
-    __host__ __device__ static constexpr int t_doubles(int N) { return GUARD + ROWS * NI * ld(N); }
+    static constexpr bool TILE_TAB = NS <= 4;
+    static constexpr int TC_A = 0, TC_Q = 16, TC_P = 32, TC_B = 48, TC_M = 64, TC_R = 80, TCN = TILE_TAB ? 96 : 0;
+    static constexpr int T_OFF = TCN + GUARD;
+    __host__ __device__ static constexpr int t_doubles(int N) { return T_OFF + ROWS * NI * ld(N); }
     static constexpr int RL_A = ROWS, RL_B = RL_A + NS * NS, RL_C = RL_B + NS * NU, ROWS_LTV = RL_C + NS;
-    __host__ __device__ static constexpr int t_doubles_ltv(int N) { return GUARD + ROWS_LTV * NI * ld(N); }
+    __host__ __device__ static constexpr int t_doubles_ltv(int N) { return T_OFF + ROWS_LTV * NI * ld(N); }
     static constexpr int QZN = 5 * NS + 2 * NU + 1;
     static constexpr int QN = QZN + NS;
     static constexpr int ROWS_WS = NU + 2 * NC;
@@ -69,6 +72,21 @@
 
 enum : int { kWvOk0 = 1, kWvWarm = 2, kWvValid = 4, kWvKeepU = 8, kWvNoShift = 16 };
 
+template <int NS, int NU, bool HASM, int NC, int NI, class PT>
+__device__ __forceinline__ void wv_fill_tile_consts(const PT &P, double *tc, int lane)
+{
+    using Cfg = WvCfg<NS, NU, NC, NI>;
+    if constexpr (Cfg::TILE_TAB) {
+        for (int e = lane; e < Cfg::TCN; e += 64) tc[e] = 0.0;
+        const int r = (lane >> 2) & 3, c = lane & 3;
+        if (lane < 16) {
+            if (r < NS && c < NS) { tc[Cfg::TC_A + lane] = P.A[r][c]; tc[Cfg::TC_Q + lane] = P.Q[r][c]; tc[Cfg::TC_P + lane] = P.Pf[r][c]; }
+            if (r < NS && c < NU) { tc[Cfg::TC_B + lane] = P.B[r][c]; if (HASM) tc[Cfg::TC_M + lane] = P.M[r][c]; }
+            if (r < NU && c < NU) tc[Cfg::TC_R + lane] = P.R[r][c];
+        }
+    }
+}
+
 __device__ __forceinline__ double row16_sum(double v)
 {
     v += dpp_move<0xB1, 0xF>(0.0, v);
@@ -79,10 +97,10 @@
 }
 __device__ __forceinline__ double row16_max(double v)
 {
-    v = dmax(v, dpp_move<0xB1, 0xF>(v, v));
-    v = dmax(v, dpp_move<0x4E, 0xF>(v, v));
-    v = dmax(v, dpp_move<0x141, 0xF>(v, v));
-    v = dmax(v, dpp_move<0x140, 0xF>(v, v));
+    v = dmax_vv(v, dpp_move<0xB1, 0xF>(v, v));
+    v = dmax_vv(v, dpp_move<0x4E, 0xF>(v, v));
+    v = dmax_vv(v, dpp_move<0x141, 0xF>(v, v));
+    v = dmax_vv(v, dpp_move<0x140, 0xF>(v, v));
     return v;
 }
 
@@ -129,7 +147,7 @@
         MPC_UNROLL for (int i = 0; i < NU; i++) du[i] = Xj.u[i] - qd[5 * NS + i];
         MPC_UNROLL for (int i = 0; i < NS; i++) {
             double a = (NU + i < NC) ? Xj.lh[NU + i < NC ? NU + i : 0] - Xj.ll[NU + i < NC ? NU + i : 0] : 0.0;
-            MPC_UNROLL for (int l = 0; l < NS; l++) a += (last ? Pl.Pf[i][l] : Pl.Q[i][l]) * dz1[l];
+            MPC_UNROLL for (int l = 0; l < NS; l++) { const double wq = Pl.Q[i][l], wp = Pl.Pf[i][l]; a += (last ? wp : wq) * dz1[l]; }
             gz[i] = a;
         }
         MPC_UNROLL for (int i = 0; i < NU; i++) {
@@ -156,8 +174,8 @@
             if (blk_on) tk(RA + i, j) = Xj.ll[i] * isl + Xj.lh[i] * ish;
             hb[i] = Xj.lh[i] * (rh * ish - 1.0) + Xj.ll[i] * (rl * isl + 1.0);
             resp_p = dmax(resp_p, dmax(fabs(rl), fabs(rh)));
-            cres_p = dmax(cres_p, dmax(comp_measure(Xj.sl[i], Xj.ll[i]), comp_measure(Xj.sh[i], Xj.lh[i])));
-            lmax_p = dmax(lmax_p, dmax(Xj.ll[i], Xj.lh[i]));
+            cres_p = dmax(cres_p, dmax(comp_measure_vv(Xj.sl[i], Xj.ll[i]), comp_measure_vv(Xj.sh[i], Xj.lh[i])));
+            lmax_p = dmax(lmax_p, dmax_vv(Xj.ll[i], Xj.lh[i]));
         }
         double gu[NU], gz[NS], pi[NS];
         gradient(Pl, j, Xj, gu, gz);
@@ -343,6 +361,17 @@
         double *p_hu, *p_hz[SB], *p_kf, *p_k[SB], *p_kt[SB], *p_li;
         const double *p_a, *p_at, *p_b, *p_bt;
     };
+    const double *const tcs = T - Cfg::T_OFF;
+    auto tile_el = [&](int tab, const auto &M, int nr, int nc, int r, int c) -> double {
+        if constexpr (Cfg::TILE_TAB) return tcs[tab + 4 * r + c];
+        else return (r < nr && c < nc) ? M[r < nr ? r : 0][c < nc ? c : 0] : 0.0;
+    };
+    auto el_a = [&](const PT &Pl, int r, int c) -> double { return tile_el(Cfg::TC_A, Pl.A, NS, NS, r, c); };
+    auto el_q = [&](const PT &Pl, int r, int c) -> double { return tile_el(Cfg::TC_Q, Pl.Q, NS, NS, r, c); };
+    auto el_p = [&](const PT &Pl, int r, int c) -> double { return tile_el(Cfg::TC_P, Pl.Pf, NS, NS, r, c); };
+    auto el_b = [&](const PT &Pl, int r, int c) -> double { return tile_el(Cfg::TC_B, Pl.B, NS, NU, r, c); };
+    auto el_m = [&](const PT &Pl, int r, int c) -> double { return tile_el(Cfg::TC_M, Pl.M, NS, NU, r, c); };
+    auto el_r = [&](const PT &Pl, int r, int c) -> double { return tile_el(Cfg::TC_R, Pl.R, NU, NU, r, c); };
     auto tile_ctx = [&](const PT &Pl) {
         int lo = threadIdx.x;
         asm volatile("" : "+v"(lo));
@@ -356,14 +385,8 @@
         auto trow = [&](int row) -> double * { return c.Tt + (c.live ? row : RZ) * (NI * LD); };
         MPC_UNROLL for (int i = 0; i < SB; i++) {
             const int ri = 4 * i + tr, ci = 4 * i + tc;
-            MPC_UNROLL for (int j = 0; j < SB; j++) {
-                const int cj = 4 * j + tc, rj = 4 * j + tr;
-                c.Ar[i][j] = (ri < NS && cj < NS) ? Pl.A[ri < NS ? ri : 0][cj < NS ? cj : 0] : 0.0;
-                c.Atr[i][j] = (ri < NS && cj < NS) ? Pl.A[cj < NS ? cj : 0][ri < NS ? ri : 0] : 0.0;
-                (void)rj;
-            }
-            c.Br[i] = (ri < NS && tc < NU) ? Pl.B[ri < NS ? ri : 0][tc < NU ? tc : 0] : 0.0;
-            c.Btr[i] = (tr < NU && ci < NS) ? Pl.B[ci < NS ? ci : 0][tr < NU ? tr : 0] : 0.0;
+            MPC_UNROLL for (int j = 0; j < SB; j++) { c.Ar[i][j] = el_a(Pl, ri, 4 * j + tc); c.Atr[i][j] = el_a(Pl, 4 * j + tc, ri); }
+            c.Br[i] = el_b(Pl, ri, tc); c.Btr[i] = el_b(Pl, ci, tr);
             c.p_hz[i] = trow(ri < NS ? RG + NU + ri : RZ);
             c.p_k[i] = trow((tr < NU && ci < NS) ? RA + tr * NS + ci : RZ);
             c.p_kt[i] = trow((ri < NS && tc < NU) ? RA + tc * NS + ri : RZ);
@@ -386,16 +409,15 @@
         const int tr = c.tr, tc = c.tc; const bool live = c.live;
         double *const trash = c.trash;
         auto trow = [&](int row) -> double * { return c.Tt + (live ? row : RZ) * (NI * LD); };
-        const bool in_uu = tr < NU && tc < NU;
-        const double Rr = in_uu ? Pl.R[tr][tc] : 0.0;
+        const double Rr = el_r(Pl, tr, tc);
         double Qr[SB][SB], Mtr[SB], BE0[SB], BE1[SB];
         MPC_UNROLL for (int i = 0; i < SB; i++) {
             const int ri = 4 * i + tr, ci = 4 * i + tc;
-            MPC_UNROLL for (int j = 0; j < SB; j++) { const int cj = 4 * j + tc; Qr[i][j] = (ri < NS && cj < NS) ? Pl.Q[ri < NS ? ri : 0][cj < NS ? cj : 0] : 0.0; }
-            Mtr[i] = (HASM && tr < NU && ci < NS) ? Pl.M[ci < NS ? ci : 0][tr < NU ? tr : 0] : 0.0;
-            BE0[i] = ri < NS ? Pl.B[ri < NS ? ri : 0][0] : 0.0; BE1[i] = (NU > 1 && ri < NS) ? Pl.B[ri < NS ? ri : 0][NU > 1 ? 1 : 0] : 0.0;
-        }
-        const double RE0 = tc < NU ? Pl.R[0][tc] : 0.0, RE1 = (NU > 1 && tc < NU) ? Pl.R[NU > 1 ? 1 : 0][tc] : 0.0;
+            MPC_UNROLL for (int j = 0; j < SB; j++) Qr[i][j] = el_q(Pl, ri, 4 * j + tc);
+            Mtr[i] = HASM ? el_m(Pl, ci, tr) : 0.0;
+            BE0[i] = el_b(Pl, ri, 0); BE1[i] = NU > 1 ? el_b(Pl, ri, 1) : 0.0;
+        }
+        const double RE0 = el_r(Pl, 0, tc), RE1 = NU > 1 ? el_r(Pl, 1, tc) : 0.0;
         const double Ir = tr == tc ? 1.0 : 0.0;
         const double *q_sz[SB];
         MPC_UNROLL for (int i = 0; i < SB; i++) { const int ri = 4 * i + tr; q_sz[i] = trow((tr == tc && ri < NS && NU + ri < NC) ? RA + NU + ri : RZ) + (N - 1); }
@@ -424,8 +446,7 @@
         const int stpf = st_f ? PD : 0;
         double Pm[SB][SB], PC[SB];
         MPC_UNROLL for (int i = 0; i < SB; i++) {
-            const int ri = 4 * i + tr;
-            MPC_UNROLL for (int j = 0; j < SB; j++) { const int cj = 4 * j + tc; Pm[i][j] = (ri < NS && cj < NS) ? Pl.Pf[ri < NS ? ri : 0][cj < NS ? cj : 0] : 0.0; }
+            MPC_UNROLL for (int j = 0; j < SB; j++) Pm[i][j] = el_p(Pl, 4 * i + tr, 4 * j + tc);
             PC[i] = 0.0;
         }
         constexpr int NF = 2 * SB + 4 + (LTV ? 3 : 0);
@@ -899,13 +920,13 @@
         bool any_on = false;
         MPC_UNROLL for (int j = 0; j < NJ; j++) any_on = any_on || (PAIR ? __any(S[j].on) != 0 : S[j].on);
         if (!any_on) break;
-        __syncthreads();
+        wave_lds_sync();
         pd_min = 1.0;
         tile_factor();
-        __syncthreads();
+        wave_lds_sync();
         MPC_TSTAMP(2);
         tile_forward();
-        __syncthreads();
+        wave_lds_sync();
         MPC_TSTAMP(3);
         {
             const unsigned long long bad = __ballot(((lane >> 2) & 3) < NI && !(pd_min > 0.0));
@@ -958,13 +979,13 @@
             }
             __builtin_amdgcn_sched_barrier(0);
         }
-        __syncthreads();
+        wave_lds_sync();
         MPC_TSTAMP(4);
         tile_rhs();
-        __syncthreads();
+        wave_lds_sync();
         MPC_TSTAMP(5);
         tile_forward();
-        __syncthreads();
+        wave_lds_sync();
         MPC_TSTAMP(3);
         MPC_UNROLL for (int j = 0; j < NJ; j++) {
             WvInst &Sj = S[j];
@@ -1073,7 +1094,7 @@
         MPC_UNROLL for (int j = 0; j < NE; j++) Pr[j] = kp[p_off + rr * NE + j];
         MPC_UNROLL for (int j = 0; j < NY; j++) { double a = 0.0; MPC_UNROLL for (int l = 0; l < NE; l++) a += Pr[l] * P.Ca[j][l]; PCt[j] = a; }
         if (row) { MPC_UNROLL for (int j = 0; j < NY; j++) xch[r * NY + j] = PCt[j]; }
-        __syncthreads();
+        wave_lds_sync();
         double all[NE][NY], S[NY][NY];
         MPC_UNROLL for (int l = 0; l < NE; l++) { MPC_UNROLL for (int j = 0; j < NY; j++) all[l][j] = xch[l * NY + j]; }
         MPC_UNROLL for (int i = 0; i < NY; i++) { MPC_UNROLL for (int j = 0; j < NY; j++) { double a = P.Rkf[i][j]; MPC_UNROLL for (int l = 0; l < NE; l++) a += P.Ca[i][l] * all[l][j]; S[i][j] = a; } }
@@ -1085,7 +1106,7 @@
         MPC_UNROLL for (int j = 0; j < NE; j++) { double a = 0.0; MPC_UNROLL for (int l = 0; l < NE; l++) a += Pc[l] * P.Aa[j][l]; U[j] = a; }
         double *xu = xch + NE * NY;
         if (row) { MPC_UNROLL for (int j = 0; j < NE; j++) xu[r * NE + j] = U[j]; }
-        __syncthreads();
+        wave_lds_sync();
         double Pn[NE];
         MPC_UNROLL for (int j = 0; j < NE; j++) Pn[j] = e[RT::E_Q + j];
         MPC_UNROLL for (int l = 0; l < NE; l++) { const double al = e[RT::E_A + l]; MPC_UNROLL for (int j = 0; j < NE; j++) Pn[j] += al * xu[l * NE + j]; }
@@ -1097,7 +1118,7 @@
     MPC_UNROLL for (int l = 0; l < NY; l++) v += Kr[l] * innov[l];
     if (P.has_dsat && r >= NX) v = dmin(dmax(v, e[RT::E_DMIN]), e[RT::E_DMAX]);
     xi_new = v;
-    __syncthreads();
+    wave_lds_sync();
     if (row) kp[xi_off + r] = v;
 }
 
@@ -1200,6 +1221,7 @@
             else if (lmax > kInfeasZ * gscale || !(fabs(mu) < 1.0e300)) { status = kInfeasible; on = false; }
             else if (it == P.max_iter) { status = kMaxIter; on = false; }
         }
+        if (!__any(on ? 1 : 0)) break;
         double Ht[NR][NR];
         MPC_UNROLL for (int i = 0; i < NR; i++) { MPC_UNROLL for (int j = 0; j <= i; j++) { const double a = P.Hr[i][j] + row16_sum(sig * Wr[i] * Wr[j]); Ht[i][j] = a; Ht[j][i] = a; } }
         const bool pd = sym_inverse<NR>(Ht);
```

After: 37.74 million (median of 6 runs). 1.05x the previous value.
